# rlawhdrhs/Vision-Transformer-OpenCL

Hardware: AMD Instinct MI355X
Metric: images/sec ViT-B/16 224² fp32 @batch256; % MFMA roofline; top-1 match (higher is better)
Workload: dtype f32; 1 GPU; ViT-B/16 224x224 fp32 forward, batch 256 per GPU, synthetic weights and images (BASELINE.json configs[1]); batch_per_gpu=256, global_batch=256, parallelism=dp1, lanes_per_gpu=1, prune_last_layer=False, ln_fold=True, device=AMD Radeon Graphics, arch=gfx950:sramecc+:xnack-, compute_units=256, clock_mhz=2400

## Files before the change

### include/vit_hip_kernels.h

```cpp
#ifndef VIT_HIP_KERNELS_H
#define VIT_HIP_KERNELS_H

#include <stddef.h>

#ifdef __cplusplus
extern "C" {
#endif

typedef void *vithip_stream_t;
typedef void *vithip_event_t;
typedef void *vithip_graph_t;

typedef struct {
    char name[256];
    char arch[64];
    int compute_units;
    int clock_mhz;
    int wavefront;
    int lds_per_block;
    unsigned long long hbm_bytes;
} vithip_device_info;

const char *vithip_error_string(int code);
int vithip_device_count(int *count);
int vithip_set_device(int device);
int vithip_get_device_info(int device, vithip_device_info *info);
int vithip_malloc(void **ptr, size_t bytes);
int vithip_free(void *ptr);
int vithip_host_alloc(void **ptr, size_t bytes);
int vithip_host_free(void *ptr);
int vithip_memcpy_h2d(void *dst, const void *src, size_t bytes, vithip_stream_t stream);
int vithip_memcpy_d2h(void *dst, const void *src, size_t bytes, vithip_stream_t stream);
int vithip_memcpy_d2d(void *dst, const void *src, size_t bytes, vithip_stream_t stream);
int vithip_memcpy_peer(void *dst, int dst_device, const void *src, int src_device, size_t bytes, vithip_stream_t stream);
int vithip_memset(void *dst, int value, size_t bytes, vithip_stream_t stream);
int vithip_stream_create(vithip_stream_t *stream);
int vithip_stream_destroy(vithip_stream_t stream);
int vithip_stream_sync(vithip_stream_t stream);
int vithip_device_sync(void);
int vithip_event_create(vithip_event_t *event);
int vithip_event_destroy(vithip_event_t event);
int vithip_event_record(vithip_event_t event, vithip_stream_t stream);
int vithip_event_sync(vithip_event_t event);
int vithip_event_elapsed_ms(float *ms, vithip_event_t start, vithip_event_t stop);
int vithip_stream_wait_event(vithip_stream_t stream, vithip_event_t event);
int vithip_graph_begin(vithip_stream_t stream);
int vithip_graph_end(vithip_stream_t stream, vithip_graph_t *graph);
int vithip_graph_launch(vithip_graph_t graph, vithip_stream_t stream);
int vithip_graph_destroy(vithip_graph_t graph);


enum { VITHIP_EPI_BIAS = 0, VITHIP_EPI_BIAS_GELU = 1, VITHIP_EPI_BIAS_RESIDUAL = 2 };

typedef struct {
    const float *A; int lda;
    const float *W; int ldw;
    const float *bias;
    const float *residual; int ldr;
    float *C; int ldc;
    int M, N, K;
    int epilogue;
    int tile, group_m;
    void *workspace;
    int handover_test;
    const float *ln_rows, *ln_colsum;
    float *stats_out, *stats_partials;
    int arith;
} vithip_gemm_args;
int vithip_gemm_f32(vithip_stream_t stream, const vithip_gemm_args *args);
int vithip_gemm_f32_stats_in_epilogue(const vithip_gemm_args *args);
int vithip_ln_fold_weights_f32(vithip_stream_t stream, const float *W, const float *bias, const float *gamma, const float *beta,
                               float *Wf, float *colsum, float *bias_f, int N, int K);
int vithip_ln_fold_weights_f32_centered(vithip_stream_t stream, const float *W, const float *bias, const float *gamma,
                                        const float *beta, float *Wc, float *residual_colsum, float *bias_f, int N, int K);
int vithip_rowstats_f32(vithip_stream_t stream, const float *x, size_t ldx, float *rows_out, int rows, int dim);
int vithip_rowstats_finalize_f32(vithip_stream_t stream, const float *partials, int rows, int dim, float *rows_out);
size_t vithip_gemm_f32_workspace_bytes(void);
int vithip_gemm_f32_workspace_create(void **workspace);
int vithip_gemm_f32_workspace_destroy(void *workspace);
int vithip_gemm_f32_workspace_stats(void *workspace, int *taken, int *recomputed);
void *vithip_gemm_f32_workspace_device_ptr(void *workspace);
enum { VITHIP_BF16_EPI_BF16 = 0, VITHIP_BF16_EPI_BF16_GELU = 1, VITHIP_BF16_EPI_F32_RESIDUAL = 2,
       VITHIP_BF16_EPI_F32_EMBED = 3  };
typedef struct {
    const unsigned short *A; int lda;
    const unsigned short *W; int ldw;
    const float *bias;
    const float *residual; int ldr;
    void *C; int ldc;
    int M, N, K;
    int epilogue;
    int variant;
    const float *ln_rows, *ln_colsum;
    unsigned short *x16; int ldx16;
    float *row_partials;
} vithip_gemm_bf16_args;
int vithip_gemm_bf16(vithip_stream_t stream, const vithip_gemm_bf16_args *args);
int vithip_ln_fold_weights(vithip_stream_t stream, const float *W, const float *bias, const float *gamma, const float *beta,
                           unsigned short *Wf, float *colsum, float *bias_f, int N, int K);
#define VITHIP_QSCALE 0.18033688011112042f
int vithip_ln_fold_weights_scaled(vithip_stream_t stream, const float *W, const float *bias, const float *gamma, const float *beta,
                                  unsigned short *Wf, float *colsum, float *bias_f, int N, int K, int scale_rows, float scale);
int vithip_rowstats_bf16(vithip_stream_t stream, const float *x, size_t ldx, unsigned short *x16, size_t ldx16,
                         float *rows_out, int rows, int dim);
int vithip_ln_strips(int N);
int vithip_rowstats_finalize(vithip_stream_t stream, const float *partials, int strips, int rows, int dim, float *rows_out);
int vithip_gather_rows_f32(vithip_stream_t stream, const float *src, size_t src_stride, float *dst, size_t dst_stride, int rows,
                           int width);
int vithip_layernorm_f32_bf16out(vithip_stream_t stream, const float *x, size_t ldx, unsigned short *y, size_t ldy,
                                 const float *gamma, const float *beta, int rows, int dim);
int vithip_attention_bf16io(vithip_stream_t stream, const unsigned short *qkv, unsigned short *out,
                            int n_images, int tokens, int heads);
int vithip_attention_bf16io_f32math(vithip_stream_t stream, const unsigned short *qkv, unsigned short *out,
                                    int n_images, int tokens, int heads);
int vithip_attention_f32_rows(vithip_stream_t stream, const float *qkv, float *out, int n_images, int tokens, int heads,
                              int q_rows);
int vithip_attention_bf16io_rows(vithip_stream_t stream, const unsigned short *qkv, unsigned short *out, int n_images,
                                 int tokens, int heads, int q_rows);
int vithip_attention_bf16io_qscaled(vithip_stream_t stream, const unsigned short *qkv, unsigned short *out, int n_images,
                                    int tokens, int heads, int q_rows);
int vithip_patch_embed_bf16(vithip_stream_t stream, const float *images, const unsigned short *conv_w16,
                            const float *conv_b, const float *cls, const float *pos, float *x,
                            unsigned short *patches16, int n_images, int img_size, int patch_size, int in_chans,
                            int embed_dim);
int vithip_patch_embed_bf16_implicit(vithip_stream_t stream, const float *images, const unsigned short *conv_w16,
                                     const float *conv_b, const float *cls, const float *pos, float *x,
                                     int n_images, int img_size, int patch_size, int in_chans, int embed_dim);
int vithip_f32_to_bf16(vithip_stream_t stream, const float *src, unsigned short *dst, size_t count);

int vithip_patch_embed_f32(vithip_stream_t stream, const float *images, const float *conv_w,
                           const float *conv_b, const float *cls, const float *pos, float *x,
                           int n_images, int img_size, int patch_size, int in_chans, int embed_dim);

int vithip_layernorm_f32(vithip_stream_t stream, const float *x, size_t ldx, float *y, size_t ldy,
                         const float *gamma, const float *beta, int rows, int dim);

int vithip_attention_f32(vithip_stream_t stream, const float *qkv, float *out,
                         int n_images, int tokens, int heads);

int vithip_softmax_top1_f32(vithip_stream_t stream, const float *logits, int ld_logits,
                            float *probs, int ld_probs, int *top1_label, float *top1_prob,
                            int rows, int classes);

int vithip_images_u8_to_f32(vithip_stream_t stream, const unsigned char *src, float *dst, int n, int img_size, int chans,
                            const float *mean, const float *std);

#ifdef __cplusplus
}
#endif
#endif
```

### vision-transformer-opencl_amd/binding.py

```python
from __future__ import annotations

import ctypes as C
import os
from typing import Optional, Sequence

import numpy as np

from .synth import ModelConfig

HERE = os.path.dirname(os.path.abspath(__file__))
LIB_PATH = os.environ.get("VIT_HIP_LIBRARY") or os.path.join(HERE, "libvit_mi355x.so")

f32p = C.POINTER(C.c_float)
i32p = C.POINTER(C.c_int)

STAGES = ("embed", "ln", "qkv", "attn", "outproj", "fc1", "fc2", "head", "softmax")
IMAGENET_MEAN = (0.485, 0.456, 0.406)
IMAGENET_STD = (0.229, 0.224, 0.225)
EPI_BIAS, EPI_BIAS_GELU, EPI_BIAS_RESIDUAL = 0, 1, 2
ARITH_F32, ARITH_SPLIT3 = 0, 1


class VitError(RuntimeError):
    pass


class CConfig(C.Structure):
    _fields_ = [(k, C.c_int) for k in ("img_size", "patch_size", "in_chans", "num_classes",
                                       "embed_dim", "depth", "num_heads", "hidden_dim")]

    @classmethod
    def of(cls, cfg: ModelConfig) -> "CConfig":
        return cls(cfg.img_size, cfg.patch_size, cfg.in_chans, cfg.num_classes, cfg.embed_dim,
                   cfg.depth, cfg.num_heads, cfg.hidden_dim)


class CNetwork(C.Structure):
    _fields_ = [("data", f32p), ("size", C.c_size_t)]


class CImageData(C.Structure):
    _fields_ = [("n", C.c_int), ("c", C.c_int), ("h", C.c_int), ("w", C.c_int), ("data", f32p)]


class COptions(C.Structure):
    _fields_ = [("device", C.c_int), ("max_batch", C.c_int), ("profile", C.c_int), ("lanes", C.c_int),
                ("dtype", C.c_int), ("prune_last_layer", C.c_int), ("use_graph", C.c_int), ("gemm_tile", C.c_int), ("ln_fold", C.c_int),
                ("gemm_handover_test", C.c_int), ("host_first_piece", C.c_int), ("fp32_split", C.c_int)]


class CStageTimes(C.Structure):
    _fields_ = [("ms", C.c_double * len(STAGES)), ("launches", C.c_long * len(STAGES)), ("images", C.c_long)]


class CDeviceInfo(C.Structure):
    _fields_ = [("name", C.c_char * 256), ("arch", C.c_char * 64), ("compute_units", C.c_int),
                ("clock_mhz", C.c_int), ("wavefront", C.c_int), ("lds_per_block", C.c_int),
                ("hbm_bytes", C.c_ulonglong)]


class CGemmArgs(C.Structure):
    _fields_ = [("A", C.c_void_p), ("lda", C.c_int), ("W", C.c_void_p), ("ldw", C.c_int),
                ("bias", C.c_void_p), ("residual", C.c_void_p), ("ldr", C.c_int),
                ("C", C.c_void_p), ("ldc", C.c_int), ("M", C.c_int), ("N", C.c_int), ("K", C.c_int),
                ("epilogue", C.c_int), ("tile", C.c_int), ("group_m", C.c_int), ("workspace", C.c_void_p),
                ("handover_test", C.c_int), ("ln_rows", C.c_void_p), ("ln_colsum", C.c_void_p),
                ("stats_out", C.c_void_p), ("stats_partials", C.c_void_p), ("arith", C.c_int)]


_lib: Optional[C.CDLL] = None


DP_LIB_PATH = os.path.join(HERE, "libvit_mi355x_dp.so")
_dp_lib = None


def dp_lib() -> C.CDLL:
    global _dp_lib
    if _dp_lib is None:
        if not os.path.exists(DP_LIB_PATH):
            raise VitError(f"{DP_LIB_PATH} is missing: run `make -C {HERE}`")
        L = C.CDLL(DP_LIB_PATH)
        L.vit_dp_create.argtypes = [C.POINTER(C.c_void_p), C.POINTER(C.c_int), C.c_int]
        L.vit_dp_destroy.argtypes = [C.c_void_p]
        L.vit_dp_destroy.restype = None
        L.vit_dp_size.argtypes = [C.c_void_p]
        L.vit_dp_device.argtypes = [C.c_void_p, C.c_int]
        L.vit_dp_last_error.argtypes = [C.c_void_p]
        L.vit_dp_last_error.restype = C.c_char_p
        L.vit_dp_gather_top1.argtypes = [C.c_void_p, C.POINTER(C.c_void_p), C.POINTER(C.c_void_p), C.c_size_t, C.POINTER(C.c_void_p)]
        _dp_lib = L
    return _dp_lib


class DpGroup:

    def __init__(self, devices):
        self.devices = [int(d) for d in devices]
        self._h = C.c_void_p()
        arr = (C.c_int * len(self.devices))(*self.devices)
        rc = dp_lib().vit_dp_create(C.byref(self._h), arr, len(self.devices))
        if rc != 0:
            raise VitError(f"vit_dp_create({self.devices}) failed: {rc}")

    def gather_top1(self, send_ptrs, recv_ptrs, records: int, streams=None) -> None:
        n = len(self.devices)
        send = (C.c_void_p * n)(*send_ptrs)
        recv = (C.c_void_p * n)(*recv_ptrs)
        st = (C.c_void_p * n)(*streams) if streams is not None else None
        rc = dp_lib().vit_dp_gather_top1(self._h, send, recv, records, st)
        if rc != 0:
            raise VitError(f"vit_dp_gather_top1: {dp_lib().vit_dp_last_error(self._h).decode()} ({rc})")

    def close(self) -> None:
        if self._h:
            dp_lib().vit_dp_destroy(self._h)
            self._h = C.c_void_p()


def lib() -> C.CDLL:
    global _lib
    if _lib is None:
        if not os.path.exists(LIB_PATH):
            raise VitError(f"{LIB_PATH} is missing: the HIP extension has not been built "
                           "(run `python -c 'import __graft_entry__ as g; g.build()'` or `make -C "
                           f"{HERE}`); there is no CPU fallback")
        L = C.CDLL(LIB_PATH)
        L.vithip_error_string.restype = C.c_char_p
        L.vit_engine_last_error.restype = C.c_char_p
        L.vit_engine_last_error.argtypes = [C.c_void_p]
        L.vit_engine_create.argtypes = [C.POINTER(C.c_void_p), C.POINTER(CConfig), C.POINTER(COptions)]
        L.vit_engine_destroy.argtypes = [C.c_void_p]
        L.vit_engine_load_weights.argtypes = [C.c_void_p, C.POINTER(CNetwork), C.c_int]
        L.vit_engine_forward_device.argtypes = [C.c_void_p, C.c_void_p, C.c_int, C.c_void_p, C.c_void_p,
                                                C.c_void_p, C.c_void_p]
        L.vit_engine_forward_host.argtypes = [C.c_void_p, C.POINTER(f32p), C.c_int, C.POINTER(f32p)]
        L.vit_engine_forward_device_u8.argtypes = [C.c_void_p, C.c_void_p, C.c_int, f32p, f32p, C.c_void_p, C.c_void_p,
                                                   C.c_void_p, C.c_void_p]
        L.vit_engine_forward_host_u8.argtypes = [C.c_void_p, C.POINTER(C.c_void_p), C.c_int, f32p, f32p, C.POINTER(f32p)]
        L.vithip_images_u8_to_f32.argtypes = [C.c_void_p, C.c_void_p, C.c_void_p, C.c_int, C.c_int, C.c_int, f32p, f32p]
        L.vit_engine_read_logits.argtypes = [C.c_void_p, f32p, C.c_int]
        L.vit_engine_sync.argtypes = [C.c_void_p]
        L.vit_engine_get_stage_times.argtypes = [C.c_void_p, C.POINTER(CStageTimes)]
        L.vit_engine_reset_stage_times.argtypes = [C.c_void_p]
        L.vit_engine_set_profile.argtypes = [C.c_void_p, C.c_int]
        L.vit_config_weight_size.restype = C.c_size_t
        L.vit_config_weight_size.argtypes = [C.POINTER(CConfig), C.c_int]
        L.vit_config_macs_per_image.restype = C.c_ulonglong
        L.vit_config_macs_per_image.argtypes = [C.POINTER(CConfig)]
        L.vit_config_macs_per_image_pruned.restype = C.c_ulonglong
        L.vit_config_macs_per_image_pruned.argtypes = [C.POINTER(CConfig)]
        L.vit_config_b16.restype = CConfig
        L.load_image_data.restype = C.POINTER(CImageData)
        L.load_image_data.argtypes = [C.c_char_p]
        L.free_image_data.argtypes = [C.POINTER(CImageData)]
        L.load_weights.argtypes = [C.c_char_p, C.POINTER(CNetwork), C.c_int]
        L.free_weights.argtypes = [C.POINTER(CNetwork), C.c_int]
        L.vit_round_weights.argtypes = [f32p, C.c_size_t]
        L.vit_compare_results.argtypes = [C.c_char_p, C.c_char_p, C.c_int, C.c_float]
        L.vit_synth_uniform.argtypes = [C.c_ulonglong, C.c_int, C.c_size_t, C.c_float, C.c_float, f32p]
        L.vit_synth_weights.argtypes = [C.POINTER(CConfig), C.c_ulonglong, C.POINTER(CNetwork), C.c_int]
        L.vit_synth_images.restype = C.POINTER(CImageData)
        L.vit_synth_images.argtypes = [C.POINTER(CConfig), C.c_int, C.c_ulonglong]
        L.vit_argmax.argtypes = [f32p, C.c_int]
        L.ViT_hip.argtypes = [C.POINTER(CImageData), C.POINTER(CNetwork), C.POINTER(f32p)]
        L.ViT_opencl.argtypes = [C.POINTER(CImageData), C.POINTER(CNetwork), C.POINTER(f32p)]
        for fn in ("vithip_malloc", "vithip_host_alloc"):
            getattr(L, fn).argtypes = [C.POINTER(C.c_void_p), C.c_size_t]
        L.vithip_free.argtypes = [C.c_void_p]
        for fn in ("vithip_memcpy_h2d", "vithip_memcpy_d2h", "vithip_memcpy_d2d"):
            getattr(L, fn).argtypes = [C.c_void_p, C.c_void_p, C.c_size_t, C.c_void_p]
        L.vithip_gemm_f32.argtypes = [C.c_void_p, C.POINTER(CGemmArgs)]
        L.vithip_patch_embed_f32.argtypes = [C.c_void_p] + [C.c_void_p] * 6 + [C.c_int] * 5
        L.vithip_layernorm_f32.argtypes = [C.c_void_p, C.c_void_p, C.c_size_t, C.c_void_p, C.c_size_t,
                                           C.c_void_p, C.c_void_p, C.c_int, C.c_int]
        L.vithip_attention_f32.argtypes = [C.c_void_p, C.c_void_p, C.c_void_p, C.c_int, C.c_int, C.c_int]
        L.vithip_softmax_top1_f32.argtypes = [C.c_void_p, C.c_void_p, C.c_int, C.c_void_p, C.c_int, C.c_void_p,
                                              C.c_void_p, C.c_int, C.c_int]
        L.vithip_event_create.argtypes = [C.POINTER(C.c_void_p)]
        L.vithip_event_record.argtypes = [C.c_void_p, C.c_void_p]
        L.vithip_event_sync.argtypes = [C.c_void_p]
        L.vithip_event_destroy.argtypes = [C.c_void_p]
        L.vithip_event_elapsed_ms.argtypes = [C.POINTER(C.c_float), C.c_void_p, C.c_void_p]
        L.vithip_stream_sync.argtypes = [C.c_void_p]
        L.vithip_get_device_info.argtypes = [C.c_int, C.POINTER(CDeviceInfo)]
        _lib = L
    return _lib


def hip_check(rc: int, what: str = "HIP call") -> None:
    if rc != 0:
        raise VitError(f"{what}: HIP error {rc} ({lib().vithip_error_string(rc).decode()})")


def _as_f32(a) -> np.ndarray:
    return np.ascontiguousarray(a, dtype=np.float32)


def networks_from(weights: Sequence[np.ndarray]):
    arr = (CNetwork * len(weights))()
    keep = []
    for i, w in enumerate(weights):
        if w is None:
            arr[i].data = None
            arr[i].size = 0
        else:
            w = _as_f32(w)
            keep.append(w)
            arr[i].data = w.ctypes.data_as(f32p)
            arr[i].size = w.size
    return arr, keep


class DeviceArray:

    def __init__(self, shape, dtype=np.float32):
        self.shape = tuple(int(s) for s in np.atleast_1d(shape))
        self.dtype = np.dtype(dtype)
        self.nbytes = int(np.prod(self.shape)) * self.dtype.itemsize
        p = C.c_void_p()
        hip_check(lib().vithip_malloc(C.byref(p), max(self.nbytes, 16)), "vithip_malloc")
        self.ptr = p.value

    @classmethod
    def from_numpy(cls, a: np.ndarray) -> "DeviceArray":
        a = np.ascontiguousarray(a)
        d = cls(a.shape, a.dtype)
        hip_check(lib().vithip_memcpy_h2d(d.ptr, a.ctypes.data, a.nbytes, None), "h2d")
        hip_check(lib().vithip_device_sync(), "sync")
        return d

    def numpy(self) -> np.ndarray:
        out = np.empty(self.shape, self.dtype)
        hip_check(lib().vithip_device_sync(), "sync")
        hip_check(lib().vithip_memcpy_d2h(out.ctypes.data, self.ptr, self.nbytes, None), "d2h")
        hip_check(lib().vithip_device_sync(), "sync")
        return out

    def free(self) -> None:
        if self.ptr:
            lib().vithip_free(self.ptr)
            self.ptr = None

    def __del__(self):
        try:
            self.free()
        except Exception:
            pass


def gemm(A, W, bias, residual=None, epilogue=EPI_BIAS, tile: int = 0, group_m: int = 0, workspace: bool = False,
         handover_test: int = 0, stats: Optional[dict] = None, ln=None, row_stats: Optional[dict] = None,
         arith: int = ARITH_F32) -> np.ndarray:
    A, W, bias = _as_f32(A), _as_f32(W), _as_f32(bias)
    M, K = A.shape
    N = W.shape[0]
    dA, dW, db = DeviceArray.from_numpy(A), DeviceArray.from_numpy(W), DeviceArray.from_numpy(bias)
    dC = DeviceArray((M, N))
    dR = DeviceArray.from_numpy(_as_f32(residual)) if residual is not None else None
    ws = gemm_workspace() if workspace else None
    dRows = DeviceArray.from_numpy(_as_f32(ln[0])) if ln is not None else None
    dCs = DeviceArray.from_numpy(_as_f32(ln[1])) if ln is not None and ln[1] is not None else None
    dSt = DeviceArray((M, 2)) if row_stats is not None else None
    dPart = DeviceArray((max(N // 64, 1), M, 2)) if row_stats is not None and row_stats.get("scratch", True) else None
    args = CGemmArgs(dA.ptr, K, dW.ptr, K, db.ptr, dR.ptr if dR else None, N, dC.ptr, N, M, N, K, epilogue, tile, group_m, ws,
                     handover_test, dRows.ptr if dRows else None, dCs.ptr if dCs else None, dSt.ptr if dSt else None,
                     dPart.ptr if dPart else None, arith)
    if row_stats is not None:
        row_stats["in_epilogue"] = int(lib().vithip_gemm_f32_stats_in_epilogue(C.byref(args)))
    hip_check(lib().vithip_gemm_f32(None, C.byref(args)), "vithip_gemm_f32")
    out = dC.numpy()
    if row_stats is not None:
        row_stats["rows"] = dSt.numpy()
    if ws:
        if stats is not None:
            stats.update(gemm_workspace_stats(ws))
        lib().vithip_gemm_f32_workspace_destroy(C.c_void_p(ws))
    return out


def gemm_workspace() -> int:
    p = C.c_void_p()
    hip_check(lib().vithip_gemm_f32_workspace_create(C.byref(p)), "vithip_gemm_f32_workspace_create")
    return p.value


def gemm_workspace_stats(ws: int) -> dict:
    L = lib()
    hip_check(L.vithip_device_sync(), "vithip_device_sync")
    t, r = C.c_int(), C.c_int()
    L.vithip_gemm_f32_workspace_stats.argtypes = [C.c_void_p, C.POINTER(C.c_int), C.POINTER(C.c_int)]
    hip_check(L.vithip_gemm_f32_workspace_stats(ws, C.byref(t), C.byref(r)), "vithip_gemm_f32_workspace_stats")
    return {"taken": t.value, "recomputed": r.value}


def gemm_workspace_flags(ws: int, count: int = 1016) -> np.ndarray:
    L = lib()
    L.vithip_gemm_f32_workspace_device_ptr.restype = C.c_void_p
    L.vithip_gemm_f32_workspace_device_ptr.argtypes = [C.c_void_p]
    flags = np.empty(count, np.int32)
    hip_check(L.vithip_device_sync(), "sync")
    hip_check(L.vithip_memcpy_d2h(flags.ctypes.data, L.vithip_gemm_f32_workspace_device_ptr(ws), flags.nbytes, None), "d2h")
    hip_check(L.vithip_device_sync(), "sync")
    return flags


def gemm_workspace_set_flags(ws: int, values) -> None:
    L = lib()
    L.vithip_gemm_f32_workspace_device_ptr.restype = C.c_void_p
    L.vithip_gemm_f32_workspace_device_ptr.argtypes = [C.c_void_p]
    v = np.ascontiguousarray(values, np.int32)
    hip_check(L.vithip_device_sync(), "sync")
    hip_check(L.vithip_memcpy_h2d(L.vithip_gemm_f32_workspace_device_ptr(ws), v.ctypes.data, v.nbytes, None), "h2d")
    hip_check(L.vithip_device_sync(), "sync")


class CGemmBf16Args(C.Structure):
    _fields_ = [("A", C.c_void_p), ("lda", C.c_int), ("W", C.c_void_p), ("ldw", C.c_int), ("bias", C.c_void_p),
                ("residual", C.c_void_p), ("ldr", C.c_int), ("C", C.c_void_p), ("ldc", C.c_int),
                ("M", C.c_int), ("N", C.c_int), ("K", C.c_int), ("epilogue", C.c_int),
                ("variant", C.c_int),
                ("ln_rows", C.c_void_p), ("ln_colsum", C.c_void_p), ("x16", C.c_void_p), ("ldx16", C.c_int),
                ("row_partials", C.c_void_p)]


BF16_EPI_BF16, BF16_EPI_BF16_GELU, BF16_EPI_F32_RESIDUAL = 0, 1, 2


def to_bf16_bits(x: np.ndarray) -> np.ndarray:
    u = np.ascontiguousarray(x, np.float32).view(np.uint32).astype(np.uint64)
    return ((u + 0x7FFF + ((u >> 16) & 1)) >> 16).astype(np.uint16)


def from_bf16_bits(b: np.ndarray) -> np.ndarray:
    return (b.astype(np.uint32) << 16).view(np.float32)


def f32_to_bf16_device(x: np.ndarray) -> np.ndarray:
    x = _as_f32(x)
    L = lib()
    L.vithip_f32_to_bf16.argtypes = [C.c_void_p, C.c_void_p, C.c_void_p, C.c_size_t]
    dx = DeviceArray.from_numpy(x)
    dy = DeviceArray(x.shape, np.uint16)
    hip_check(L.vithip_f32_to_bf16(None, dx.ptr, dy.ptr, x.size), "vithip_f32_to_bf16")
    return dy.numpy()


def gemm_bf16(A_bits, W_bits, bias, residual=None, epilogue=BF16_EPI_BF16, variant: int = 0, ln_rows=None, ln_colsum=None,
              ln_producer: bool = False):
    L = lib()
    L.vithip_gemm_bf16.argtypes = [C.c_void_p, C.POINTER(CGemmBf16Args)]
    M, K = A_bits.shape
    N = W_bits.shape[0]
    dA, dW = DeviceArray.from_numpy(np.ascontiguousarray(A_bits, np.uint16)), DeviceArray.from_numpy(np.ascontiguousarray(W_bits, np.uint16))
    db = DeviceArray.from_numpy(_as_f32(bias))
    out_f32 = epilogue == BF16_EPI_F32_RESIDUAL
    dC = DeviceArray((M, N), np.float32 if out_f32 else np.uint16)
    dR = DeviceArray.from_numpy(_as_f32(residual)) if residual is not None else None
    dRows = DeviceArray.from_numpy(_as_f32(ln_rows)) if ln_rows is not None else None
    dCs = DeviceArray.from_numpy(_as_f32(ln_colsum)) if ln_colsum is not None else None
    strips = ln_strips(N)
    dX16 = DeviceArray((M, N), np.uint16) if ln_producer else None
    dPart = DeviceArray((strips, M, 2), np.float32) if ln_producer else None
    args = CGemmBf16Args(dA.ptr, K, dW.ptr, K, db.ptr, dR.ptr if dR else None, N, dC.ptr, N, M, N, K, epilogue,
                         variant, dRows.ptr if dRows else None, dCs.ptr if dCs else None,
                         dX16.ptr if dX16 else None, N, dPart.ptr if dPart else None)
    hip_check(L.vithip_gemm_bf16(None, C.byref(args)), "vithip_gemm_bf16")
    if ln_producer:
        return dC.numpy(), dX16.numpy(), dPart.numpy()
    return dC.numpy()


def ln_strips(N: int) -> int:
    return int(lib().vithip_ln_strips(int(N)))


def ln_fold_weights(W, bias, gamma, beta):
    W = _as_f32(W)
    N, K = W.shape
    L = lib()
    L.vithip_ln_fold_weights.argtypes = [C.c_void_p] * 8 + [C.c_int, C.c_int]
    dW, db, dg, dbe = (DeviceArray.from_numpy(_as_f32(a)) for a in (W, bias, gamma, beta))
    dWf, dcs, dbf = DeviceArray((N, K), np.uint16), DeviceArray((N,), np.float32), DeviceArray((N,), np.float32)
    hip_check(L.vithip_ln_fold_weights(None, dW.ptr, db.ptr, dg.ptr, dbe.ptr, dWf.ptr, dcs.ptr, dbf.ptr, N, K), "vithip_ln_fold_weights")
    return dWf.numpy(), dcs.numpy(), dbf.numpy()


def rowstats_bf16(x):
    x = _as_f32(x)
    rows, dim = x.shape
    L = lib()
    L.vithip_rowstats_bf16.argtypes = [C.c_void_p, C.c_void_p, C.c_size_t, C.c_void_p, C.c_size_t, C.c_void_p, C.c_int, C.c_int]
    dx, d16, dr = DeviceArray.from_numpy(x), DeviceArray((rows, dim), np.uint16), DeviceArray((rows, 2), np.float32)
    hip_check(L.vithip_rowstats_bf16(None, dx.ptr, dim, d16.ptr, dim, dr.ptr, rows, dim), "vithip_rowstats_bf16")
    return d16.numpy(), dr.numpy()


def rowstats_finalize(partials, dim: int):
    partials = _as_f32(partials)
    strips, rows, _ = partials.shape
    L = lib()
    L.vithip_rowstats_finalize.argtypes = [C.c_void_p, C.c_void_p, C.c_int, C.c_int, C.c_int, C.c_void_p]
    dp, dr = DeviceArray.from_numpy(partials), DeviceArray((rows, 2), np.float32)
    hip_check(L.vithip_rowstats_finalize(None, dp.ptr, strips, rows, dim, dr.ptr), "vithip_rowstats_finalize")
    return dr.numpy()


def layernorm_bf16out(x, gamma, beta) -> np.ndarray:
    x = _as_f32(x)
    rows, dim = x.shape
    L = lib()
    L.vithip_layernorm_f32_bf16out.argtypes = [C.c_void_p, C.c_void_p, C.c_size_t, C.c_void_p, C.c_size_t,
                                               C.c_void_p, C.c_void_p, C.c_int, C.c_int]
    dx, dg, db = DeviceArray.from_numpy(x), DeviceArray.from_numpy(_as_f32(gamma)), DeviceArray.from_numpy(_as_f32(beta))
    dy = DeviceArray((rows, dim), np.uint16)
    hip_check(L.vithip_layernorm_f32_bf16out(None, dx.ptr, dim, dy.ptr, dim, dg.ptr, db.ptr, rows, dim),
              "vithip_layernorm_f32_bf16out")
    return dy.numpy()


QSCALE = 0.18033688011112042


def attention_bf16io(qkv_bits, n_images: int, tokens: int, heads: int, f32math: bool = False, q_scaled: bool = False,
                     q_rows: Optional[int] = None) -> np.ndarray:
    D = heads * 64
    dq = DeviceArray.from_numpy(np.ascontiguousarray(qkv_bits, np.uint16))
    do = DeviceArray((n_images * tokens, D), np.uint16)
    if q_scaled:
        fn = lib().vithip_attention_bf16io_qscaled
        fn.argtypes = [C.c_void_p, C.c_void_p, C.c_void_p, C.c_int, C.c_int, C.c_int, C.c_int]
        hip_check(fn(None, dq.ptr, do.ptr, n_images, tokens, heads, q_rows or tokens), "vithip_attention_bf16io_qscaled")
        return do.numpy()
    fn = getattr(lib(), "vithip_attention_bf16io_f32math" if f32math else "vithip_attention_bf16io")
    fn.argtypes = [C.c_void_p, C.c_void_p, C.c_void_p, C.c_int, C.c_int, C.c_int]
    hip_check(fn(None, dq.ptr, do.ptr, n_images, tokens, heads), "vithip_attention_bf16io")
    return do.numpy()


def layernorm(x, gamma, beta) -> np.ndarray:
    x = _as_f32(x)
    rows, dim = x.shape
    dx, dg, db = DeviceArray.from_numpy(x), DeviceArray.from_numpy(_as_f32(gamma)), DeviceArray.from_numpy(_as_f32(beta))
    dy = DeviceArray((rows, dim))
    hip_check(lib().vithip_layernorm_f32(None, dx.ptr, dim, dy.ptr, dim, dg.ptr, db.ptr, rows, dim), "vithip_layernorm_f32")
    return dy.numpy()


def ln_fold_weights_f32(W, bias, gamma, beta):
    W, bias, gamma, beta = _as_f32(W), _as_f32(bias), _as_f32(gamma), _as_f32(beta)
    N, K = W.shape
    dW, db, dg, dbe = (DeviceArray.from_numpy(a) for a in (W, bias, gamma, beta))
    dWf, dcs, dbf = DeviceArray((N, K)), DeviceArray((N,)), DeviceArray((N,))
    lib().vithip_ln_fold_weights_f32.argtypes = [C.c_void_p] * 8 + [C.c_int, C.c_int]
    hip_check(lib().vithip_ln_fold_weights_f32(None, dW.ptr, db.ptr, dg.ptr, dbe.ptr, dWf.ptr, dcs.ptr, dbf.ptr, N, K),
              "vithip_ln_fold_weights_f32")
    return dWf.numpy(), dcs.numpy(), dbf.numpy()


def ln_fold_weights_f32_centered(W, bias, gamma, beta):
    W, bias, gamma, beta = _as_f32(W), _as_f32(bias), _as_f32(gamma), _as_f32(beta)
    N, K = W.shape
    dW, db, dg, dbe = (DeviceArray.from_numpy(a) for a in (W, bias, gamma, beta))
    dWf, dcs, dbf = DeviceArray((N, K)), DeviceArray((N,)), DeviceArray((N,))
    lib().vithip_ln_fold_weights_f32_centered.argtypes = [C.c_void_p] * 8 + [C.c_int, C.c_int]
    hip_check(lib().vithip_ln_fold_weights_f32_centered(None, dW.ptr, db.ptr, dg.ptr, dbe.ptr, dWf.ptr, dcs.ptr, dbf.ptr, N, K),
              "vithip_ln_fold_weights_f32_centered")
    return dWf.numpy(), dcs.numpy(), dbf.numpy()


def rowstats_f32(x) -> np.ndarray:
    x = _as_f32(x)
    rows, dim = x.shape
    L = lib()
    L.vithip_rowstats_f32.argtypes = [C.c_void_p, C.c_void_p, C.c_size_t, C.c_void_p, C.c_int, C.c_int]
    dx, dr = DeviceArray.from_numpy(x), DeviceArray((rows, 2))
    hip_check(L.vithip_rowstats_f32(None, dx.ptr, dim, dr.ptr, rows, dim), "vithip_rowstats_f32")
    return dr.numpy()


def attention(qkv, n_images: int, tokens: int, heads: int) -> np.ndarray:
    qkv = _as_f32(qkv)
    D = heads * 64
    assert qkv.shape == (n_images * tokens, 3 * D)
    dq = DeviceArray.from_numpy(qkv)
    do = DeviceArray((n_images * tokens, D))
    hip_check(lib().vithip_attention_f32(None, dq.ptr, do.ptr, n_images, tokens, heads), "vithip_attention_f32")
    return do.numpy()


def attention_rows(qkv, n_images: int, tokens: int, heads: int, q_rows: int, fill: float = 0.0) -> np.ndarray:
    qkv = _as_f32(qkv)
    D = heads * 64
    L = lib()
    L.vithip_attention_f32_rows.argtypes = [C.c_void_p, C.c_void_p, C.c_void_p, C.c_int, C.c_int, C.c_int, C.c_int]
    dq = DeviceArray.from_numpy(qkv)
    do = DeviceArray.from_numpy(np.full((n_images * tokens, D), fill, np.float32))
    hip_check(L.vithip_attention_f32_rows(None, dq.ptr, do.ptr, n_images, tokens, heads, q_rows), "vithip_attention_f32_rows")
    return do.numpy()


def patch_embed(cfg: ModelConfig, images, conv_w, conv_b, cls, pos) -> np.ndarray:
    images = _as_f32(images)
    n = images.shape[0]
    d = [DeviceArray.from_numpy(_as_f32(a)) for a in (images, conv_w, conv_b, cls, pos)]
    dx = DeviceArray((n * cfg.tokens, cfg.embed_dim))
    hip_check(lib().vithip_patch_embed_f32(None, d[0].ptr, d[1].ptr, d[2].ptr, d[3].ptr, d[4].ptr, dx.ptr, n,
                                           cfg.img_size, cfg.patch_size, cfg.in_chans, cfg.embed_dim),
              "vithip_patch_embed_f32")
    return dx.numpy().reshape(n, cfg.tokens, cfg.embed_dim)


def patch_embed_bf16(cfg: ModelConfig, images, conv_w, conv_b, cls, pos, implicit: bool = False) -> np.ndarray:
    images = _as_f32(images)
    n = images.shape[0]
    L = lib()
    if implicit:
        L.vithip_patch_embed_bf16_implicit.argtypes = [C.c_void_p] * 7 + [C.c_int] * 5
        d = [DeviceArray.from_numpy(_as_f32(a)) for a in (images, conv_b, cls, pos)]
        dw = DeviceArray.from_numpy(to_bf16_bits(_as_f32(conv_w).reshape(cfg.embed_dim, -1)))
        dx = DeviceArray((n * cfg.tokens, cfg.embed_dim))
        hip_check(L.vithip_patch_embed_bf16_implicit(None, d[0].ptr, dw.ptr, d[1].ptr, d[2].ptr, d[3].ptr, dx.ptr, n, cfg.img_size,
                                                     cfg.patch_size, cfg.in_chans, cfg.embed_dim), "vithip_patch_embed_bf16_implicit")
        return dx.numpy().reshape(n, cfg.tokens, cfg.embed_dim)
    L.vithip_patch_embed_bf16.argtypes = [C.c_void_p] * 8 + [C.c_int] * 5
    d = [DeviceArray.from_numpy(_as_f32(a)) for a in (images, conv_b, cls, pos)]
    dw = DeviceArray.from_numpy(to_bf16_bits(_as_f32(conv_w).reshape(cfg.embed_dim, -1)))
    dx = DeviceArray((n * cfg.tokens, cfg.embed_dim))
    dp = DeviceArray((n * cfg.patches, cfg.patch_dim), np.uint16)
    hip_check(L.vithip_patch_embed_bf16(None, d[0].ptr, dw.ptr, d[1].ptr, d[2].ptr, d[3].ptr, dx.ptr, dp.ptr, n,
                                        cfg.img_size, cfg.patch_size, cfg.in_chans, cfg.embed_dim), "vithip_patch_embed_bf16")
    return dx.numpy().reshape(n, cfg.tokens, cfg.embed_dim)


def softmax_top1(logits):
    logits = _as_f32(logits)
    rows, classes = logits.shape
    dl = DeviceArray.from_numpy(logits)
    dp = DeviceArray((rows, classes))
    dlab = DeviceArray((rows,), np.int32)
    dpr = DeviceArray((rows,))
    hip_check(lib().vithip_softmax_top1_f32(None, dl.ptr, classes, dp.ptr, classes, dlab.ptr, dpr.ptr, rows, classes),
              "vithip_softmax_top1_f32")
    return dp.numpy(), dlab.numpy(), dpr.numpy()


def _norm_consts(mean, std, chans: int):
    out = []
    for v in (mean, std):
        if v is None:
            out.append(None)
            continue
        v = np.ascontiguousarray(v, np.float32).reshape(-1)
        if v.size != chans:
            raise ValueError(f"expected {chans} normalisation constants, got {v.size}")
        out.append((C.c_float * chans)(*v.tolist()))
    return out


def images_u8_to_f32(images, mean=IMAGENET_MEAN, std=IMAGENET_STD) -> np.ndarray:
    images = np.ascontiguousarray(images, np.uint8)
    n, S, S2, chans = images.shape
    assert S == S2
    m, s = _norm_consts(mean, std, chans)
    ds, dd = DeviceArray.from_numpy(images), DeviceArray((n, chans, S, S))
    hip_check(lib().vithip_images_u8_to_f32(None, ds.ptr, dd.ptr, n, S, chans, m, s), "vithip_images_u8_to_f32")
    return dd.numpy()


def device_info(device: int = 0) -> dict:
    info = CDeviceInfo()
    hip_check(lib().vithip_get_device_info(device, C.byref(info)), "vithip_get_device_info")
    return {"name": info.name.decode(), "arch": info.arch.decode(), "compute_units": info.compute_units,
            "clock_mhz": info.clock_mhz, "wavefront": info.wavefront, "lds_per_block": info.lds_per_block,
            "hbm_bytes": int(info.hbm_bytes)}


class Engine:

    def __init__(self, cfg: ModelConfig, max_batch: int = 256, device: int = 0, profile: bool = False,
                 lanes: int = 1, dtype: str = "f32", prune_last_layer: bool = False, use_graph: bool = False,
# ... 305 lines not shown
```

### vision-transformer-opencl_amd/csrc/vit_gemm.hip

```cpp
#include <new>

#include "vit_gemm_common.hpp"
#ifdef VIT_PROBES
#include "vit_probes.h"
#endif

namespace vitgemm {
int launch_persistent(hipStream_t stream, GemmParams &p, int epilogue, int group_m, int arith = ARITH_F32);
int launch_persistent_stamped(hipStream_t stream, GemmParams &p, int epilogue, int group_m);
int launch_persistent_switchoff(hipStream_t stream, GemmParams &p, int epilogue, int group_m, int dbg);
int persistent_piece_steps(int M, int N, int K, int slots, int wgs, int kstep);
}

namespace {

using namespace vitgemm;

#ifdef VIT_PROBES
int g_gemm_tile = 0;
int g_gemm_group = 0;
unsigned long long *g_gemm_dbg = nullptr;
#endif

template <int BM, int BN, int WM, int WN, int EPI, int AMODE, int DBG = 0, int BK = 32, bool PIPE = false, int ARITH = ARITH_F32>
// ... 219 lines not shown
                }
            }
            cur ^= 1;
        }
    } else {
        load_global(0);
        store_lds(0);
        if constexpr (DBG != 0) store_lds(1);
        __syncthreads();


        if constexpr (DBG == 5) st_clk1 = __builtin_amdgcn_s_memtime();
        if constexpr (DBG >= 10) {
#pragma unroll
            for (int q = 0; q < DBG - 10; ++q) asm volatile("s_nop 0");
        }
        int cur = 0;
        for (int kt = 0; kt < nk; ++kt) {
            const bool more = kt + 1 < nk;
            if constexpr (DBG == 0 || DBG == 3 || DBG == 5) {
                if (more) load_global((kt + 1) * BK);
            }

            const float *As = As0 + cur * BM * LDS_LD + a_frag_off;
            const float *Bs = Bs0 + cur * BN * LDS_LD + b_frag_off;
#pragma unroll
            for (int c = 0; c < BK / 8; ++c) {
                f32x4 a[TM], b[TN];
#pragma unroll
                for (int i = 0; i < TM; ++i) a[i] = *reinterpret_cast<const f32x4 *>(As + i * 32 * LDS_LD + c * 8);
#pragma unroll
                for (int j = 0; j < TN; ++j) b[j] = *reinterpret_cast<const f32x4 *>(Bs + j * 32 * LDS_LD + c * 8);
#pragma unroll
                for (int s = 0; s < 4; ++s)
#pragma unroll
                    for (int i = 0; i < TM; ++i)
#pragma unroll
                        for (int j = 0; j < TN; ++j)
                            acc[i][j] = __builtin_amdgcn_mfma_f32_32x32x2f32(a[i][s], b[j][s], acc[i][j], 0, 0, 0);
            }

            if constexpr (DBG == 0 || DBG == 2 || DBG == 5) {
                if (more) store_lds(cur ^ 1);
            } else if constexpr (DBG == 3) {
#pragma unroll
                for (int i = 0; i < A_CHUNKS; ++i) asm volatile("" ::"v"(a_stage[i]));
#pragma unroll
                for (int i = 0; i < B_CHUNKS; ++i) asm volatile("" ::"v"(b_stage[i]));
            }
            if constexpr (DBG != 4) __syncthreads();
            cur ^= 1;
        }

    }

    if constexpr (DBG == 5) st_clk2 = __builtin_amdgcn_s_memtime();
    epilogue_store<BM, BN, WM, WN, EPI, AMODE>(p, acc, bias_r, m0, n0, wm, wn, r, h, fold);
    if constexpr (DBG == 5) {
        __builtin_amdgcn_s_waitcnt(0);
        const unsigned long long c3 = __builtin_amdgcn_s_memtime(), r3 = __builtin_amdgcn_s_memrealtime();
        if (tid == 0) {
            unsigned long long *d = p.dbg + (size_t)blockIdx.x * 8;
            d[0] = st_clk0; d[1] = st_clk1; d[2] = st_clk2; d[3] = c3; d[4] = st_rt0; d[5] = r3;
            d[6] = __builtin_amdgcn_s_getreg((3 << 11) | 20);
            d[7] = (unsigned long long)tile;
        }
    }
}

__global__ void cls_rows_kernel(const float *cls, const float *pos, float *x, int n_images, int tokens, int dim) {
    const int idx = blockIdx.x * blockDim.x + threadIdx.x;
    if (idx >= n_images * dim) return;
    const int im = idx / dim, d = idx - im * dim;
    x[(size_t)im * tokens * dim + d] = cls[d] + pos[d];
}

template <int BM, int BN, int WM, int WN, int AMODE, int BK = 32, bool PIPE = false, int ARITH = ARITH_F32>
int launch_tile(hipStream_t stream, GemmParams &p, int epilogue) {
    p.tiles_m = (p.M + BM - 1) / BM;
    p.tiles_n = (p.N + BN - 1) / BN;
    const dim3 grid(p.tiles_m * p.tiles_n), block(256);
    if constexpr (AMODE == A_PATCHES) {
        hipLaunchKernelGGL((gemm_f32_nt_kernel<BM, BN, WM, WN, VITHIP_EPI_BIAS, A_PATCHES, 0, BK, PIPE>), grid, block, 0, stream, p);
    } else {
        switch (epilogue) {
            case VITHIP_EPI_BIAS:
                hipLaunchKernelGGL((gemm_f32_nt_kernel<BM, BN, WM, WN, VITHIP_EPI_BIAS, A_DENSE, 0, BK, PIPE, ARITH>), grid, block, 0, stream, p);
                break;
            case VITHIP_EPI_BIAS_GELU:
                hipLaunchKernelGGL((gemm_f32_nt_kernel<BM, BN, WM, WN, VITHIP_EPI_BIAS_GELU, A_DENSE, 0, BK, PIPE, ARITH>), grid, block, 0, stream, p);
                break;
            case VITHIP_EPI_BIAS_RESIDUAL:
                hipLaunchKernelGGL((gemm_f32_nt_kernel<BM, BN, WM, WN, VITHIP_EPI_BIAS_RESIDUAL, A_DENSE, 0, BK, PIPE, ARITH>), grid, block, 0, stream, p);
                break;
            case EPI_BIAS_LN:
                hipLaunchKernelGGL((gemm_f32_nt_kernel<BM, BN, WM, WN, EPI_BIAS_LN, A_DENSE, 0, BK, PIPE, ARITH>), grid, block, 0, stream, p);
                break;
            case EPI_BIAS_GELU_LN:
                hipLaunchKernelGGL((gemm_f32_nt_kernel<BM, BN, WM, WN, EPI_BIAS_GELU_LN, A_DENSE, 0, BK, PIPE, ARITH>), grid, block, 0, stream, p);
                break;
            default:
                return static_cast<int>(hipErrorInvalidValue);
        }
    }
    return static_cast<int>(hipGetLastError());
}

#ifdef VIT_PROBES
template <int DBG, int EPI = VITHIP_EPI_BIAS, bool PIPE = false>
int launch_probe(hipStream_t stream, GemmParams &p) {
    p.tiles_m = (p.M + 127) / 128;
    p.tiles_n = (p.N + 127) / 128;
    hipLaunchKernelGGL((gemm_f32_nt_kernel<128, 128, 64, 64, EPI, A_DENSE, DBG, 32, PIPE>),
                       dim3(p.tiles_m * p.tiles_n), dim3(256), 0, stream, p);
    return static_cast<int>(hipGetLastError());
}
#endif

template <int AMODE, int ARITH = ARITH_F32>
int dispatch(hipStream_t stream, GemmParams &p, int epilogue, int tile, int group_m) {
    constexpr bool SPLIT = ARITH == ARITH_SPLIT3;
    constexpr int BK = SPLIT ? SPLIT_BK : 32;
    static_assert(!SPLIT || AMODE == A_DENSE, "the patch embedding stays on fp32 MFMA");
    const int cols128 = (p.N + 127) / 128;
    p.group_m = group_m > 0 ? group_m : (cols128 <= 8 ? 1 : 4);
#ifdef VIT_PROBES
    if (g_gemm_tile) tile = g_gemm_tile;
    if (g_gemm_group) p.group_m = g_gemm_group;
    if constexpr (AMODE == A_DENSE && !SPLIT) {
        switch (tile) {
            case 101: return launch_probe<1>(stream, p);
            case 102: return launch_probe<2>(stream, p);
            case 103: return launch_probe<3>(stream, p);
            case 104: return launch_probe<4>(stream, p);
            case 105: p.dbg = g_gemm_dbg; return g_gemm_dbg ? launch_probe<5>(stream, p) : static_cast<int>(hipErrorInvalidValue);
            case 129: p.dbg = g_gemm_dbg; return g_gemm_dbg ? vitgemm::launch_persistent_stamped(stream, p, epilogue, p.group_m) : static_cast<int>(hipErrorInvalidValue);
            case 125: p.dbg = g_gemm_dbg; return g_gemm_dbg ? launch_probe<5, VITHIP_EPI_BIAS, true>(stream, p) : static_cast<int>(hipErrorInvalidValue);
            case 126: p.dbg = g_gemm_dbg; return g_gemm_dbg ? launch_probe<5, VITHIP_EPI_BIAS_GELU, true>(stream, p) : static_cast<int>(hipErrorInvalidValue);
            case 131: case 132: case 133: case 134: case 135: case 136:
                return vitgemm::launch_persistent_switchoff(stream, p, epilogue, p.group_m, tile - 130);
            default: break;
        }
    }
#endif
    if constexpr (AMODE == A_PATCHES) {
        const bool pipe_ok = (32 % p.patch == 0 || p.patch % 32 == 0) && (p.patch * p.patch) % 32 == 0 &&
                             (size_t)(p.M / p.patches + 1) * p.chans * p.img * p.img * 4 < 0x7fffffffull;
#ifdef VIT_PROBES
        if (tile == 1) return launch_tile<128, 128, 64, 64, A_PATCHES>(stream, p, epilogue);
        if (tile == 2) return launch_tile<256, 128, 128, 64, A_PATCHES>(stream, p, epilogue);
        if (tile == 10) return launch_tile<128, 128, 64, 64, A_PATCHES, 32, true>(stream, p, epilogue);
        if (tile == 3) return launch_tile<128, 64, 64, 32, A_PATCHES>(stream, p, epilogue);
#endif
        if (!pipe_ok) return launch_tile<128, 64, 64, 32, A_PATCHES>(stream, p, epilogue);
        return launch_tile<128, 64, 64, 32, A_PATCHES, 32, true>(stream, p, epilogue);
    }
    switch (tile) {
        case 9: return vitgemm::launch_persistent(stream, p, epilogue, p.group_m, ARITH);
        case 6: case 7: case 8: case 12:
            if constexpr (SPLIT) return static_cast<int>(hipErrorInvalidValue);
            else if (tile == 6) return launch_tile<128, 128, 64, 64, AMODE, 16, true>(stream, p, epilogue);
            else if (tile == 7) return launch_tile<256, 128, 128, 64, AMODE, 32, true>(stream, p, epilogue);
            else if (tile == 8) return launch_tile<128, 64, 64, 32, AMODE, 32, true>(stream, p, epilogue);
            else if (p.K % 128) return static_cast<int>(hipErrorInvalidValue);
            else return vitgemm::launch_gemm_f32_latency(stream, p, epilogue);
        case 10: return launch_tile<128, 128, 64, 64, AMODE, BK, true, ARITH>(stream, p, epilogue);
        case 11: return launch_tile<64, 64, 32, 32, AMODE, BK, true, ARITH>(stream, p, epilogue);
        default: {
            const long tiles = (long)((p.M + 127) / 128) * ((p.N + 127) / 128);
            if (!SPLIT && p.K % 128 == 0 && (long)((p.M + 63) / 64) * ((p.N + 63) / 64) < 160)
                return vitgemm::launch_gemm_f32_latency(stream, p, epilogue);
            if ((long)((p.M + 127) / 128) * ((p.N + 63) / 64) < 256)
                return launch_tile<64, 64, 32, 32, AMODE, BK, true, ARITH>(stream, p, epilogue);
            if (epilogue == VITHIP_EPI_BIAS_RESIDUAL) {
                if (tiles < 1024) return launch_tile<64, 64, 32, 32, AMODE, BK, true, ARITH>(stream, p, epilogue);
                if ((p.row_partials && p.N % 128 == 0) || (p.sk_ws && vitgemm::persistent_piece_steps(p.M, p.N, p.K, p.sk_slots, 0, BK) > 0))
                    return vitgemm::launch_persistent(stream, p, epilogue, p.group_m, ARITH);
                return launch_tile<128, 128, 64, 64, AMODE, BK, true, ARITH>(stream, p, epilogue);
            }
            if (tiles < 1280) return launch_tile<64, 64, 32, 32, AMODE, BK, true, ARITH>(stream, p, epilogue);
            return vitgemm::launch_persistent(stream, p, epilogue, p.group_m, ARITH);
        }
    }
}

bool aligned16(const void *ptr) { return (reinterpret_cast<size_t>(ptr) & 15) == 0; }

}

extern "C" {

#ifdef VIT_PROBES
int vithip_gemm_set_tile(int tile) {
    if ((tile < 0 || tile > 12) && (tile < 101 || tile > 136)) return static_cast<int>(hipErrorInvalidValue);
    g_gemm_tile = tile;
    return 0;
}

int vithip_gemm_set_debug_buffer(void *buf) {
    g_gemm_dbg = static_cast<unsigned long long *>(buf);
    return 0;
}

int vithip_gemm_set_group(int group_m) {
    if (group_m < 0 || group_m > 1024) return static_cast<int>(hipErrorInvalidValue);
    g_gemm_group = group_m;
    return 0;
}
#endif

struct GemmWorkspace {
    void *dev;
    int slots;
    int device;
    int gen;
};
static size_t workspace_dev_bytes(int slots) { return 4096 + (size_t)slots * 128 * 128 * 4; }

size_t vithip_gemm_f32_workspace_bytes(void) {
    int dev = 0, cus = 0;
    if (hipGetDevice(&dev) != hipSuccess || hipDeviceGetAttribute(&cus, hipDeviceAttributeMultiprocessorCount, dev) != hipSuccess) return 0;
    return workspace_dev_bytes(2 * cus);
}

int vithip_gemm_f32_workspace_create(void **ws) {
    if (!ws) return static_cast<int>(hipErrorInvalidValue);
    *ws = nullptr;
    int dev = 0, cus = 0;
    hipError_t e = hipGetDevice(&dev);
    if (e == hipSuccess) e = hipDeviceGetAttribute(&cus, hipDeviceAttributeMultiprocessorCount, dev);
    if (e != hipSuccess) return static_cast<int>(e);
    GemmWorkspace *w = new (std::nothrow) GemmWorkspace{nullptr, 2 * cus, dev, 0};
    if (!w) return static_cast<int>(hipErrorOutOfMemory);
    e = hipExtMallocWithFlags(&w->dev, workspace_dev_bytes(w->slots), hipDeviceMallocUncached);
    if (e == hipSuccess) e = hipMemset(w->dev, 0, 4096);
    if (e == hipSuccess) e = hipDeviceSynchronize();
    if (e != hipSuccess) {
        if (w->dev) (void)hipFree(w->dev);
        delete w;
        return static_cast<int>(e);
    }
    *ws = w;
    return 0;
}
int vithip_gemm_f32_workspace_destroy(void *ws) {
    if (!ws) return 0;
    GemmWorkspace *w = static_cast<GemmWorkspace *>(ws);
    const hipError_t e = hipFree(w->dev);
    delete w;
    return static_cast<int>(e);
}
int vithip_gemm_f32_workspace_stats(void *ws, int *taken, int *recomputed) {
    if (!ws) return static_cast<int>(hipErrorInvalidValue);
    GemmWorkspace *w = static_cast<GemmWorkspace *>(ws);
    int c[2] = {0, 0};
    char *at = static_cast<char *>(w->dev) + 1016 * sizeof(int);
    hipError_t e = hipMemcpy(c, at, sizeof(c), hipMemcpyDeviceToHost);
    if (e == hipSuccess && (c[0] || c[1])) e = hipMemset(at, 0, sizeof(c));
    if (taken) *taken = c[0];
    if (recomputed) *recomputed = c[1];
    return static_cast<int>(e);
}
void *vithip_gemm_f32_workspace_device_ptr(void *ws) { return ws ? static_cast<GemmWorkspace *>(ws)->dev : nullptr; }

int vithip_gemm_f32_stats_in_epilogue(const vithip_gemm_args *a) {
    if (!a || !a->stats_out || !a->stats_partials || a->epilogue != VITHIP_EPI_BIAS_RESIDUAL || a->M <= 0 || a->N <= 0 || a->N % 128 ||
        a->N > 2048)
        return 0;
    const long tiles = (long)((a->M + 127) / 128) * (a->N / 128);
    return (a->tile == 9 || (a->tile == 0 && tiles >= 1024)) ? 1 : 0;
}

int vithip_gemm_f32(vithip_stream_t stream, const vithip_gemm_args *a) {
    if (!a || !a->A || !a->W || !a->bias || !a->C) return static_cast<int>(hipErrorInvalidValue);
    if (a->M <= 0 || a->N <= 0 || a->K <= 0 || a->K % KALIGN != 0) return static_cast<int>(hipErrorInvalidValue);
    if (a->lda % 4 || a->ldw % 4 || a->lda < a->K || a->ldw < a->K || a->ldc < a->N)
        return static_cast<int>(hipErrorInvalidValue);
    if (!aligned16(a->A) || !aligned16(a->W)) return static_cast<int>(hipErrorInvalidValue);
    if ((size_t)a->M * a->lda * 4 >= 0x7fffffffull || (size_t)a->N * a->ldw * 4 >= 0x7fffffffull)
        return static_cast<int>(hipErrorInvalidValue);
    if (a->epilogue == VITHIP_EPI_BIAS_RESIDUAL && (!a->residual || a->ldr < a->N))
        return static_cast<int>(hipErrorInvalidValue);
    if ((size_t)a->M * a->ldc * 4 >= 0x7fffffffull ||
        (a->epilogue == VITHIP_EPI_BIAS_RESIDUAL && (size_t)a->M * a->ldr * 4 >= 0x7fffffffull))
        return static_cast<int>(hipErrorInvalidValue);
    GemmParams p{};
    p.A = a->A; p.W = a->W; p.bias = a->bias; p.R = a->residual; p.C = a->C;
    p.lda = a->lda; p.ldw = a->ldw; p.ldr = a->ldr; p.ldc = a->ldc;
    p.M = a->M; p.N = a->N; p.K = a->K;
    if (a->workspace) {
        GemmWorkspace *w = static_cast<GemmWorkspace *>(a->workspace);
        int dev = -1;
        if (hipGetDevice(&dev) != hipSuccess || dev != w->device) return static_cast<int>(hipErrorInvalidDevice);
        p.sk_ws = w->dev;
        p.sk_slots = w->slots;
        p.sk_late = a->handover_test == 1;
        w->gen = w->gen >= (1 << 28) ? 1 : w->gen + 1;
        p.sk_gen = w->gen;
    }
    if (a->handover_test < 0 || a->handover_test > 1) return static_cast<int>(hipErrorInvalidValue);
    if (a->tile < 0 || (a->tile > 0 && a->tile < 6) || a->tile > 12 || a->group_m < 0 || a->group_m > 1024) return static_cast<int>(hipErrorInvalidValue);
    if (a->arith != ARITH_F32 && (a->arith != ARITH_SPLIT3 || (a->tile != 0 && a->tile != 9 && a->tile != 10 && a->tile != 11)))
        return static_cast<int>(hipErrorInvalidValue);
    int epilogue = a->epilogue;
    if (a->ln_rows || a->ln_colsum) {
        if (!a->ln_rows || (epilogue != VITHIP_EPI_BIAS && epilogue != VITHIP_EPI_BIAS_GELU) ||
            (reinterpret_cast<size_t>(a->ln_rows) & 7))
            return static_cast<int>(hipErrorInvalidValue);
        p.ln_rows = a->ln_rows;
        p.ln_colsum = a->ln_colsum;
        epilogue = epilogue == VITHIP_EPI_BIAS ? vitgemm::EPI_BIAS_LN : vitgemm::EPI_BIAS_GELU_LN;
    }
    if (a->stats_out) {
        if (epilogue != VITHIP_EPI_BIAS_RESIDUAL || a->N % 64 || a->N > 2048 || (reinterpret_cast<size_t>(a->stats_out) & 7) ||
            (reinterpret_cast<size_t>(a->stats_partials) & 7))
            return static_cast<int>(hipErrorInvalidValue);
        if (vithip_gemm_f32_stats_in_epilogue(a)) p.row_partials = a->stats_partials;
    }
    const int rc = a->arith == ARITH_SPLIT3 ? dispatch<A_DENSE, ARITH_SPLIT3>(static_cast<hipStream_t>(stream), p, epilogue, a->tile, a->group_m)
                                            : dispatch<A_DENSE>(static_cast<hipStream_t>(stream), p, epilogue, a->tile, a->group_m);
    if (rc != 0 || !a->stats_out) return rc;
    if (p.stats_in_epilogue) return vithip_rowstats_finalize_f32(stream, a->stats_partials, a->M, a->N, a->stats_out);
    return vithip_rowstats_f32(stream, a->C, (size_t)a->ldc, a->stats_out, a->M, a->N);
}

int vithip_patch_embed_f32(vithip_stream_t stream, const float *images, const float *conv_w,
                           const float *conv_b, const float *cls, const float *pos, float *x,
                           int n_images, int img_size, int patch_size, int in_chans, int embed_dim) {
    if (!images || !conv_w || !conv_b || !cls || !pos || !x || n_images <= 0)
        return static_cast<int>(hipErrorInvalidValue);
    if (patch_size % 4 || img_size % patch_size) return static_cast<int>(hipErrorInvalidValue);
    const int K = in_chans * patch_size * patch_size;
    if (K % KALIGN || img_size % 4) return static_cast<int>(hipErrorInvalidValue);
    if (!aligned16(images) || !aligned16(conv_w)) return static_cast<int>(hipErrorInvalidValue);
    const int G = img_size / patch_size;
    GemmParams p{};
    p.A = images; p.W = conv_w; p.bias = conv_b; p.C = x; p.pos = pos;
    p.lda = 0; p.ldw = K; p.ldc = embed_dim;
    p.M = n_images * G * G; p.N = embed_dim; p.K = K;
    p.patches = G * G; p.grid = G; p.patch = patch_size; p.img = img_size; p.chans = in_chans;
    hipStream_t s = static_cast<hipStream_t>(stream);
    const int total = n_images * embed_dim;
    hipLaunchKernelGGL(cls_rows_kernel, dim3((total + 255) / 256), dim3(256), 0, s, cls, pos, x,
                       n_images, G * G + 1, embed_dim);
    int e = static_cast<int>(hipGetLastError());
    if (e) return e;
    return dispatch<A_PATCHES>(s, p, VITHIP_EPI_BIAS, 0, 0);
}

}
```

### vision-transformer-opencl_amd/csrc/vit_gemm_common.hpp

```cpp
#pragma once
#include <hip/hip_runtime.h>

#include <type_traits>

#include "vit_hip_kernels.h"

namespace vitgemm {


typedef float f32x16 __attribute__((ext_vector_type(16)));
typedef float f32x4 __attribute__((ext_vector_type(4)));
typedef float f32x2 __attribute__((ext_vector_type(2)));
typedef unsigned u32x4 __attribute__((ext_vector_type(4)));

constexpr int KALIGN = 32;

enum { A_DENSE = 0, A_PATCHES = 1 };
enum { EPI_BIAS_LN = 3, EPI_BIAS_GELU_LN = 4, EPI_RESIDUAL_STATS = 5 };

struct GemmParams {
    const float *A;
    const float *W;
    const float *bias;
    const float *R;
    float *C;
    int lda, ldw, ldr, ldc;
    int M, N, K;
    int tiles_m, tiles_n;
    int group_m;
    const float *pos;
    unsigned long long *dbg;
    int patches;
    int grid;
    int patch;
    int img;
    int chans;
    void *sk_ws;
    int sk_slots;
    int sk_x;
    int sk_late;
    int sk_gen;
    const float *ln_rows;
    const float *ln_colsum;
    float *row_partials;
    int stats_in_epilogue;
};

__device__ __forceinline__ float erf_fp32(float x) {
    const float t = fminf(fabsf(x), 4.0f);
    float q = -3.144179208902642e-05f;
    q = fmaf(q, t, 3.0881378916092217e-04f);
    q = fmaf(q, t, -1.0324339382350445e-03f);
    q = fmaf(q, t, -5.368884885683656e-04f);
    q = fmaf(q, t, 1.95839274674654e-02f);
    q = fmaf(q, t, -1.0291960090398788e-01f);
    q = fmaf(q, t, -6.36597752571106e-01f);
    q = fmaf(q, t, -1.128380298614502f);
    const float e = __builtin_amdgcn_exp2f(q * t * 1.4426950408889634f);
    return copysignf(1.0f - e, x);
}

__device__ __forceinline__ float gelu_erf(float x) {
    return 0.5f * x * (1.0f + erf_fp32(x * 0.70710678118654752440f));
}

__device__ __forceinline__ void gelu_erf_x8(float (&y)[8]) {
    typedef float v2 __attribute__((ext_vector_type(2)));
    v2 yy[4], u[4], t[4], q[4];
#pragma unroll
    for (int v = 0; v < 4; ++v) {
        yy[v] = v2{y[2 * v], y[2 * v + 1]};
        u[v] = yy[v] * v2{0.70710678118654752440f, 0.70710678118654752440f};
        t[v] = v2{fminf(fabsf(u[v][0]), 4.0f), fminf(fabsf(u[v][1]), 4.0f)};
        q[v] = __builtin_elementwise_fma(v2{-3.144179208902642e-05f, -3.144179208902642e-05f}, t[v],
                                         v2{3.0881378916092217e-04f, 3.0881378916092217e-04f});
    }
    __builtin_amdgcn_sched_barrier(0);
    constexpr float c[6] = {-1.0324339382350445e-03f, -5.368884885683656e-04f, 1.95839274674654e-02f,
                            -1.0291960090398788e-01f, -6.36597752571106e-01f, -1.128380298614502f};
#pragma unroll
    for (int k = 0; k < 6; ++k) {
#pragma unroll
        for (int v = 0; v < 4; ++v) q[v] = __builtin_elementwise_fma(q[v], t[v], v2{c[k], c[k]});
        __builtin_amdgcn_sched_barrier(0);
    }
#pragma unroll
    for (int v = 0; v < 4; ++v) q[v] = q[v] * t[v] * v2{1.4426950408889634f, 1.4426950408889634f};
    __builtin_amdgcn_sched_barrier(0);
#pragma unroll
    for (int v = 0; v < 4; ++v) q[v] = v2{__builtin_amdgcn_exp2f(q[v][0]), __builtin_amdgcn_exp2f(q[v][1])};
    __builtin_amdgcn_sched_barrier(0);
#pragma unroll
    for (int v = 0; v < 4; ++v) {
        const v2 e = v2{1.0f, 1.0f} - q[v];
        const v2 sgn = v2{copysignf(e[0], u[v][0]), copysignf(e[1], u[v][1])};
        const v2 r = v2{0.5f, 0.5f} * yy[v] * (v2{1.0f, 1.0f} + sgn);
        y[2 * v] = r[0];
        y[2 * v + 1] = r[1];
    }
}

__device__ __forceinline__ f32x2 gelu_bf16_x2(f32x2 y) {
    constexpr float kClamp = 5.656854249492381f;
    const f32x2 t = f32x2{fminf(__builtin_fabsf(y.x), kClamp), fminf(__builtin_fabsf(y.y), kClamp)};
    constexpr float c[7] = {-1.000037431716919f,   -1.1505244970321655f,   -0.4605136811733246f,  -0.05179140716791153f,
                            0.007414536084979773f, -0.0006474481779150665f, 2.524326555430889e-05f};
    f32x2 q = f32x2{c[6], c[6]};
#pragma unroll
    for (int k = 5; k >= 0; --k) q = __builtin_elementwise_fma(q, t, f32x2{c[k], c[k]});
    const f32x2 e = f32x2{__builtin_amdgcn_exp2f(q.x), __builtin_amdgcn_exp2f(q.y)};
    return __builtin_elementwise_fma(-t, e, __builtin_elementwise_max(y, f32x2{0.f, 0.f}));
}

template <int NP>
__device__ __forceinline__ void gelu_bf16_lockstep(f32x2 (&y)[NP]) {
    constexpr float kClamp = 5.656854249492381f;
    constexpr float c[7] = {-1.000037431716919f,   -1.1505244970321655f,   -0.4605136811733246f,  -0.05179140716791153f,
                            0.007414536084979773f, -0.0006474481779150665f, 2.524326555430889e-05f};
    f32x2 t[NP], q[NP];
#pragma unroll
    for (int v = 0; v < NP; ++v) {
        t[v] = f32x2{fminf(__builtin_fabsf(y[v].x), kClamp), fminf(__builtin_fabsf(y[v].y), kClamp)};
        q[v] = __builtin_elementwise_fma(f32x2{c[6], c[6]}, t[v], f32x2{c[5], c[5]});
    }
    __builtin_amdgcn_sched_barrier(0);
#pragma unroll
    for (int k = 4; k >= 0; --k) {
#pragma unroll
        for (int v = 0; v < NP; ++v) q[v] = __builtin_elementwise_fma(q[v], t[v], f32x2{c[k], c[k]});
        __builtin_amdgcn_sched_barrier(0);
    }
#pragma unroll
    for (int v = 0; v < NP; ++v) q[v] = f32x2{__builtin_amdgcn_exp2f(q[v].x), __builtin_amdgcn_exp2f(q[v].y)};
    __builtin_amdgcn_sched_barrier(0);
#pragma unroll
    for (int v = 0; v < NP; ++v) y[v] = __builtin_elementwise_fma(-t[v], q[v], __builtin_elementwise_max(y[v], f32x2{0.f, 0.f}));
}

__device__ __forceinline__ int xcd_remap(int bid, int nwg) {
    const int q = nwg >> 3, rem = nwg & 7;
    const int xcd = bid & 7, idx = bid >> 3;
    const int base = xcd < rem ? xcd * (q + 1) : rem * (q + 1) + (xcd - rem) * q;
    return base + idx;
}

__device__ __forceinline__ void tile_coords(int tile, int tiles_m, int tiles_n, int group_m, int &tm, int &tn) {
    const int per_group = group_m * tiles_n;
    const int g = tile / per_group, in_g = tile - g * per_group;
    const int first = g * group_m;
    const int rows = tiles_m - first < group_m ? tiles_m - first : group_m;
    tn = in_g / rows;
    tm = first + (in_g - tn * rows);
}


enum { ARITH_F32 = 0, ARITH_SPLIT3 = 1 };
typedef __bf16 bf16x8 __attribute__((ext_vector_type(8)));
typedef __bf16 bf16x4 __attribute__((ext_vector_type(4)));
typedef unsigned u32x2 __attribute__((ext_vector_type(2)));
constexpr int SPLIT_BK = 16;
constexpr int SPLIT_LD = 28;
constexpr int SPLIT_TERM_A[6] = {0, 2, 1, 0, 1, 0};
constexpr int SPLIT_TERM_W[6] = {2, 0, 1, 1, 0, 0};

__device__ __forceinline__ float bf16_to_f32(__bf16 v) {
    return __builtin_bit_cast(float, (unsigned)__builtin_bit_cast(unsigned short, v) << 16);
}
__device__ __forceinline__ void split3_store(float *row, int kc, f32x4 x) {
#pragma unroll
    for (int piece = 0; piece < 3; ++piece) {
        bf16x4 b;
#pragma unroll
        for (int e = 0; e < 4; ++e) b[e] = (__bf16)x[e];
        *reinterpret_cast<u32x2 *>(row + piece * 8 + kc / 2) = __builtin_bit_cast(u32x2, b);
        if (piece < 2) {
#pragma unroll
            for (int e = 0; e < 4; ++e) x[e] = x[e] - bf16_to_f32(b[e]);
        }
    }
}
template <int TM, int TN, int NS, typename Restage>
__device__ __forceinline__ void split3_step(f32x16 (&acc)[TM][TN], const float *As, const float *Bs, Restage &&restage) {
    bf16x8 a[TM][3], b[TN][3];
#pragma unroll
    for (int o = 0; o < 3; ++o) {
        const int pa = SPLIT_TERM_A[o], pb = SPLIT_TERM_W[o];
#pragma unroll
        for (int i = 0; i < TM; ++i) a[i][pa] = *reinterpret_cast<const bf16x8 *>(As + i * 32 * SPLIT_LD + pa * 8);
#pragma unroll
        for (int j = 0; j < TN; ++j) b[j][pb] = *reinterpret_cast<const bf16x8 *>(Bs + j * 32 * SPLIT_LD + pb * 8);
    }
    __builtin_amdgcn_sched_barrier(0);
    constexpr int NM = 6 * TM * TN, NR = NM / 2 > 0 ? NM / 2 : 1;
#pragma unroll
    for (int idx = 0; idx < NM; ++idx) {
        const int t = idx / (TM * TN), i = (idx / TN) % TM, j = idx % TN;
        acc[i][j] = __builtin_amdgcn_mfma_f32_32x32x16_bf16(a[i][SPLIT_TERM_A[t]], b[j][SPLIT_TERM_W[t]], acc[i][j], 0, 0, 0);
        if (idx < NR) {
            const int slot_before = (idx * NS) / NR, slot_after = ((idx + 1) * NS) / NR;
            if (slot_after > slot_before) {
                __builtin_amdgcn_sched_barrier(0);
#pragma unroll
                for (int q = slot_before; q < slot_after; ++q) restage(q);
                __builtin_amdgcn_sched_barrier(0);
            }
        }
    }
}

template <int TN, int TM = 1>
struct FoldOperands {
    float colsum[TN];
    const f32x2 *rows;
    float rstd[TM][16], mean[TM];
    bool preloaded;
};
template <int TN, int TM>
__device__ __forceinline__ void fold_preload(FoldOperands<TN, TM> &fold, const float *ln_rows, int M, int m_tile, int r, int h) {
#pragma unroll
    for (int i = 0; i < TM; ++i) {
        const int mr = m_tile + i * 32 + r;
        fold.mean[i] = ln_rows[2 * (size_t)(mr < M ? mr : M - 1) + 1];
#pragma unroll
        for (int v = 0; v < 16; ++v) {
            const int m = m_tile + i * 32 + 4 * h + (v & 3) + 8 * (v >> 2);
            fold.rstd[i][v] = ln_rows[2 * (size_t)(m < M ? m : M - 1)];
        }
    }
    fold.preloaded = true;
}
__device__ __forceinline__ float fold_center(float acc, float mean, float colsum) { return __builtin_fmaf(-mean, colsum, acc); }
__device__ __forceinline__ float fold_scale(float centered, float rstd, float bias) { return __builtin_fmaf(rstd, centered, bias); }

#ifndef FOLD_HOIST
#define FOLD_HOIST 1
#endif
template <int BM, int BN, int WM, int WN, int EPI, int AMODE>
__device__ __forceinline__ void epilogue_store(const GemmParams &p, const f32x16 (&acc)[WM / 32][WN / 32],
                                               const float (&bias_r)[WN / 32], int m0, int n0, int wm, int wn,
                                               int r, int h, const FoldOperands<WN / 32, WM / 32> &fold = FoldOperands<WN / 32, WM / 32>{}) {
    constexpr int TM = WM / 32, TN = WN / 32;
    constexpr bool FOLD = EPI == EPI_BIAS_LN || EPI == EPI_BIAS_GELU_LN;
    constexpr bool GELU = EPI == VITHIP_EPI_BIAS_GELU || EPI == EPI_BIAS_GELU_LN;
    constexpr int ST_NT = 2;
    const bool interior = (m0 + BM <= p.M) && (n0 + BN <= p.N);
    if (interior) {
        if constexpr (FOLD) {
            const __amdgpu_buffer_rsrc_t c_rsrc = __builtin_amdgcn_make_buffer_rsrc(p.C, 0, 0x7fffffff, 0x00020000);
            const bool center = p.ln_colsum != nullptr;
            auto rstd_of_block = [&](int i, float (&dst)[16]) __attribute__((always_inline)) {
#pragma unroll
                for (int g = 0; g < 4; ++g) {
                    const int lr = wm * WM + i * 32 + 4 * h + 8 * g;
#pragma unroll
                    for (int e = 0; e < 4; ++e) dst[4 * g + e] = fold.preloaded ? fold.rstd[i][4 * g + e] : fold.rows[lr + e].x;
                }
            };
            auto scale_and_store = [&](int i, const f32x16 (&src)[TN], const float (&row_rstd)[16]) __attribute__((always_inline)) {
                const int mb = m0 + wm * WM + i * 32 + 4 * h;
#pragma unroll
                for (int j = 0; j < TN; ++j) {
                    const int n = n0 + wn * WN + j * 32 + r;
                    const int c_off = (mb * p.ldc + n) * 4, c_row = p.ldc * 4;
#pragma unroll
                    for (int half = 0; half < 2; ++half) {
                        float y[8];
#pragma unroll
                        for (int q = 0; q < 8; ++q) y[q] = fold_scale(src[j][half * 8 + q], row_rstd[half * 8 + q], bias_r[j]);
                        if constexpr (GELU) gelu_erf_x8(y);
#pragma unroll
                        for (int q = 0; q < 8; ++q) {
                            const int v = half * 8 + q;
                            __builtin_amdgcn_raw_buffer_store_b32(__builtin_bit_cast(unsigned, y[q]), c_rsrc, c_off, ((v & 3) + 8 * (v >> 2)) * c_row, ST_NT);
                        }
                    }
                }
            };
            if (center) {
                float b_op[TN];
#pragma unroll
                for (int j = 0; j < TN; ++j) b_op[j] = h == 0 ? fold.colsum[j] : 0.0f;
#pragma unroll
                for (int i = 0; i < TM; ++i) {
                    const float mean = fold.preloaded ? fold.mean[i] : fold.rows[wm * WM + i * 32 + r].y;
                    const float a_op = h == 0 ? -mean : 0.0f;
                    f32x16 centered[TN];
#pragma unroll
                    for (int j = 0; j < TN; ++j) centered[j] = __builtin_amdgcn_mfma_f32_32x32x2f32(a_op, b_op[j], acc[i][j], 0, 0, 0);
                    float row_rstd[16];
                    rstd_of_block(i, row_rstd);
                    scale_and_store(i, centered, row_rstd);
                }
            } else {
                float row_rstd[TM][16];
#pragma unroll
                for (int i = 0; i < (FOLD_HOIST ? TM : 0); ++i) rstd_of_block(i, row_rstd[i]);
#pragma unroll
                for (int i = 0; i < TM; ++i) {
                    if (!FOLD_HOIST) rstd_of_block(i, row_rstd[i]);
                    scale_and_store(i, acc[i], row_rstd[i]);
                }
            }
            return;
        }
#pragma unroll
        for (int j = 0; j < TN; ++j) {
            const int n = n0 + wn * WN + j * 32 + r;
#pragma unroll
            for (int i = 0; i < TM; ++i) {
                const int mb = m0 + wm * WM + i * 32 + 4 * h;
                if constexpr (AMODE == A_PATCHES) {
                    float add[16];
                    size_t orow[16];
#pragma unroll
                    for (int v = 0; v < 16; ++v) {
                        const int m = mb + (v & 3) + 8 * (v >> 2);
                        const int im = m / p.patches, pp = m - im * p.patches;
                        add[v] = p.pos[(size_t)(pp + 1) * p.N + n];
                        orow[v] = (size_t)m + im + 1;
                    }
#pragma unroll
                    for (int v = 0; v < 16; ++v) p.C[orow[v] * p.ldc + n] = acc[i][j][v] + bias_r[j] + add[v];
                } else {
                    const __amdgpu_buffer_rsrc_t c_rsrc = __builtin_amdgcn_make_buffer_rsrc(p.C, 0, 0x7fffffff, 0x00020000);
                    const int c_off = (mb * p.ldc + n) * 4, c_row = p.ldc * 4;
                    if constexpr (EPI == VITHIP_EPI_BIAS_RESIDUAL) {
                        const __amdgpu_buffer_rsrc_t r_rsrc = __builtin_amdgcn_make_buffer_rsrc(const_cast<float *>(p.R), 0, 0x7fffffff, 0x00020000);
                        const int r_off = (mb * p.ldr + n) * 4, r_row = p.ldr * 4;
#pragma unroll
                        for (int half = 0; half < 2; ++half) {
                            float res[8];
#pragma unroll
                            for (int q = 0; q < 8; ++q) {
                                const int v = half * 8 + q;
                                res[q] = __builtin_bit_cast(float, __builtin_amdgcn_raw_buffer_load_b32(r_rsrc, r_off, ((v & 3) + 8 * (v >> 2)) * r_row, 0));
                            }
#pragma unroll
                            for (int q = 0; q < 8; ++q) {
                                const int v = half * 8 + q;
                                __builtin_amdgcn_raw_buffer_store_b32(__builtin_bit_cast(unsigned, acc[i][j][v] + bias_r[j] + res[q]), c_rsrc, c_off,
                                                                      ((v & 3) + 8 * (v >> 2)) * c_row, 0);
                            }
                        }
                    } else {
#pragma unroll
                        for (int half = 0; half < 2; ++half) {
                            float y[8];
#pragma unroll
                            for (int q = 0; q < 8; ++q) y[q] = acc[i][j][half * 8 + q] + bias_r[j];
                            if constexpr (GELU) gelu_erf_x8(y);
#pragma unroll
                            for (int q = 0; q < 8; ++q) {
                                const int v = half * 8 + q;
                                __builtin_amdgcn_raw_buffer_store_b32(__builtin_bit_cast(unsigned, y[q]), c_rsrc, c_off, ((v & 3) + 8 * (v >> 2)) * c_row, ST_NT);
                            }
                        }
                    }
                }
            }
        }
    } else {
#pragma unroll
        for (int j = 0; j < TN; ++j) {
            const int n = n0 + wn * WN + j * 32 + r;
            const bool n_ok = n < p.N;
#pragma unroll
            for (int i = 0; i < TM; ++i) {
#pragma unroll
                for (int v = 0; v < 16; ++v) {
                    const int m = m0 + wm * WM + i * 32 + (v & 3) + 8 * (v >> 2) + 4 * h;
                    if (n_ok && m < p.M) {
                        float y;
                        if constexpr (FOLD) {
                            const f32x2 row = fold.rows[m - m0];
                            y = fold_scale(fold_center(acc[i][j][v], row.y, fold.colsum[j]), row.x, bias_r[j]);
                        }
                        else y = acc[i][j][v] + bias_r[j];
                        if constexpr (AMODE == A_PATCHES) {
                            const int im = m / p.patches, pp = m - im * p.patches;
                            y += p.pos[(size_t)(pp + 1) * p.N + n];
                            p.C[((size_t)m + im + 1) * p.ldc + n] = y;
                        } else {
                            if constexpr (GELU) y = gelu_erf(y);
                            if constexpr (EPI == VITHIP_EPI_BIAS_RESIDUAL) y += p.R[(size_t)m * p.ldr + n];
                            p.C[(size_t)m * p.ldc + n] = y;
                        }
                    }
                }
            }
        }
    }
}

struct Bf16Params {
    const unsigned short *A;
    const unsigned short *W;
    const float *bias;
    const float *R;
    void *C;
    int lda, ldw, ldr, ldc;
    int M, N, K;
    int tiles_m, tiles_n, group_m;
    unsigned long long *dbg;
    int patches;
    const float *ln_rows;
    const float *ln_colsum;
    unsigned short *x16;
    int ldx16;
    float *partials;
};
int launch_gemm_bf16_pp(hipStream_t stream, const Bf16Params &p, int epilogue, int cus);
int launch_gemm_bf16_w4(hipStream_t stream, const Bf16Params &p, int epilogue, int cus);
int launch_gemm_f32_latency(hipStream_t stream, GemmParams &p, int epilogue);
int launch_patch_embed_bf16(hipStream_t s, const float *images, const unsigned short *conv_w16, const float *conv_b,
                            const float *cls, const float *pos, float *x, int n_images, int img_size, int patch_size,
                            int in_chans, int embed_dim);

__device__ __forceinline__ float reduce_scatter16(const float (&a)[16], int r) {
    float b[8], c[4], d[2], e;
    {
        const bool up = (r & 16) != 0;
#pragma unroll
        for (int k = 0; k < 8; ++k) b[k] = (up ? a[k + 8] : a[k]) + __shfl_xor(up ? a[k] : a[k + 8], 16);
    }
    {
        const bool up = (r & 8) != 0;
#pragma unroll
        for (int k = 0; k < 4; ++k) c[k] = (up ? b[k + 4] : b[k]) + __shfl_xor(up ? b[k] : b[k + 4], 8);
    }
    {
        const bool up = (r & 4) != 0;
#pragma unroll
        for (int k = 0; k < 2; ++k) d[k] = (up ? c[k + 2] : c[k]) + __shfl_xor(up ? c[k] : c[k + 2], 4);
    }
    {
        const bool up = (r & 2) != 0;
        e = (up ? d[1] : d[0]) + __shfl_xor(up ? d[0] : d[1], 2);
    }
    return e + __shfl_xor(e, 1);
}

template <int BM, int BN, int WM, int WN>
__device__ __forceinline__ void epilogue_store_residual_stats(const GemmParams &p, const f32x16 (&acc)[WM / 32][WN / 32],
                                                              const float (&bias_r)[WN / 32], int m0, int n0, int wm, int wn,
                                                              int r, int h) {
    static_assert(WN == 64, "one 64-column strip per wave");
    constexpr int TM = WM / 32;
    const bool interior = m0 + BM <= p.M;
    const int strip = (n0 + wn * WN) >> 6;
    const __amdgpu_buffer_rsrc_t c_rsrc = __builtin_amdgcn_make_buffer_rsrc(p.C, 0, 0x7fffffff, 0x00020000);
    const __amdgpu_buffer_rsrc_t r_rsrc = __builtin_amdgcn_make_buffer_rsrc(const_cast<float *>(p.R), 0, 0x7fffffff, 0x00020000);
#pragma unroll
    for (int i = 0; i < TM; ++i) {
        const int mb = m0 + wm * WM + i * 32 + 4 * h;
        float y[2][16];
#pragma unroll
        for (int j = 0; j < 2; ++j) {
            const int n = n0 + wn * WN + j * 32 + r;
            const int c_off = (mb * p.ldc + n) * 4, c_row = p.ldc * 4, r_off = (mb * p.ldr + n) * 4, r_row = p.ldr * 4;
            if (interior) {
#pragma unroll
                for (int half = 0; half < 2; ++half) {
                    float res[8];
#pragma unroll
                    for (int q = 0; q < 8; ++q) {
                        const int v = half * 8 + q;
                        res[q] = __builtin_bit_cast(float, __builtin_amdgcn_raw_buffer_load_b32(r_rsrc, r_off, ((v & 3) + 8 * (v >> 2)) * r_row, 0));
                    }
#pragma unroll
                    for (int q = 0; q < 8; ++q) {
                        const int v = half * 8 + q;
                        y[j][v] = acc[i][j][v] + bias_r[j] + res[q];
                        __builtin_amdgcn_raw_buffer_store_b32(__builtin_bit_cast(unsigned, y[j][v]), c_rsrc, c_off, ((v & 3) + 8 * (v >> 2)) * c_row, 0);
                    }
                }
            } else {
#pragma unroll
                for (int v = 0; v < 16; ++v) {
                    const int m = mb + (v & 3) + 8 * (v >> 2);
                    y[j][v] = 0.0f;
                    if (m < p.M) {
                        y[j][v] = acc[i][j][v] + bias_r[j] + p.R[(size_t)m * p.ldr + n];
                        p.C[(size_t)m * p.ldc + n] = y[j][v];
                    }
                }
            }
        }
        float u[16], w[16];
        {
#pragma clang fp contract(off)
#pragma unroll
            for (int v = 0; v < 16; ++v) {
                u[v] = y[0][v] + y[1][v];
                const float sq0 = y[0][v] * y[0][v];
                w[v] = __builtin_fmaf(y[1][v], y[1][v], sq0);
            }
        }
        const float us = reduce_scatter16(u, r), ws = reduce_scatter16(w, r);
        const int v = (r >> 1) & 15;
        const int m = mb + (v & 3) + 8 * (v >> 2);
        if (!(r & 1) && m < p.M) *reinterpret_cast<f32x2 *>(p.row_partials + ((size_t)strip * p.M + m) * 2) = f32x2{us, ws};
    }
}

}
```

### vision-transformer-opencl_amd/csrc/vit_gemm_persistent.hip

```cpp
#include "vit_gemm_common.hpp"

namespace vitgemm {

constexpr int PBK = 32;
constexpr int PLD = PBK + 4;
constexpr int SK_HEADER_BYTES = 4096, SK_MAX_OWNERS = 1000, SK_STAT_TAKEN = 1016, SK_STAT_RECOMPUTED = 1017;

template <int BM, int BN, int WM, int WN, int EPI, bool STAMP = false, bool SK = false, int DBG = 0, int ARITH = ARITH_F32>
__global__ __launch_bounds__(256, 2) void gemm_f32_nt_persistent_kernel(const GemmParams p) {
    constexpr bool SPLIT = ARITH == ARITH_SPLIT3;
    static_assert(!SPLIT || DBG == 0, "switch-off builds are fp32 only");
    constexpr int PBK = SPLIT ? SPLIT_BK : vitgemm::PBK;
    constexpr int PLD = SPLIT ? SPLIT_LD : vitgemm::PLD;
    constexpr int ROWS_PER_PASS = 256 / (PBK / 4);
    constexpr int WGN = BN / WN;
    constexpr int TM = WM / 32, TN = WN / 32;
    constexpr int A_CHUNKS = BM * (PBK / 4) / 256;
    constexpr int B_CHUNKS = BN * (PBK / 4) / 256;
    constexpr int NC = PBK / 8;
    constexpr int NS = A_CHUNKS + B_CHUNKS;
    constexpr int NM = 4 * TM * TN;
    static_assert((BM / WM) * WGN == 4, "4 waves per workgroup");

    __shared__ __attribute__((aligned(16))) float lds[2 * (BM + BN) * PLD];
    __shared__ int sk_decision;
    constexpr bool FOLD = EPI == EPI_BIAS_LN || EPI == EPI_BIAS_GELU_LN;
    __shared__ __attribute__((aligned(16))) f32x2 fold_rows_lds[FOLD ? 2 * BM : 2];
    static_assert(!FOLD || BM == 128, "one 16-byte lane copy of 64 lanes = 128 rows");
    float *const As0 = lds;
    float *const Bs0 = lds + 2 * BM * PLD;

    const int tid = threadIdx.x;
    const int lane = tid & 63, wave = tid >> 6;
    const int r = lane & 31, h = lane >> 5;
    const int wm = wave / WGN, wn = wave % WGN;

    unsigned long long st0 = 0, st_rt0 = 0, st_loop0 = 0, st_epi = 0;
    if constexpr (STAMP) {
        st0 = __builtin_amdgcn_s_memtime();
        st_rt0 = __builtin_amdgcn_s_memrealtime();
    }

    const int total = p.tiles_m * p.tiles_n;
    const int nwg = gridDim.x;
    const int first = xcd_remap(blockIdx.x, nwg);
    if (first >= total) return;
    const int nk = p.K / PBK;

    const int full = total / nwg, R = total - full * nwg;
    const int x = SK ? p.sk_x : 0;
    const int H = nwg - R;
    const bool owner = first < R;
    const int npre = (x > 0 && !owner && R > 0) ? (R - (first - R) + H - 1) / H : 0;
    const int pstart = (SK && p.sk_late) ? full : 0, fstart = (SK && p.sk_late) ? 0 : npre;
    const int nseg = npre + full + (owner ? 1 : 0);
    bool took = false;
    struct Seg { int tile, k0, k1, in, out; };
    auto get_seg = [&](int i) -> Seg {
        Seg g;
        if (i >= pstart && i < pstart + npre) {
            const int o = (first - R) + (i - pstart) * H;
            g.tile = full * nwg + o; g.k0 = 0; g.k1 = x; g.in = -1; g.out = o;
        } else if (i < npre + full) {
            g.tile = first + (i - fstart) * nwg; g.k0 = 0; g.k1 = nk; g.in = -1; g.out = -1;
        } else {
            g.tile = first + full * nwg; g.k0 = took ? x : 0; g.k1 = nk; g.in = took ? first : -1; g.out = -1;
        }
        return g;
    };

    const int ld_row = tid / (PBK / 4);
    const int ld_kc = (tid % (PBK / 4)) * 4;
    const __amdgpu_buffer_rsrc_t a_rsrc = __builtin_amdgcn_make_buffer_rsrc(const_cast<float *>(p.A), 0, 0x7fffffff, 0x00020000);
    const __amdgpu_buffer_rsrc_t w_rsrc = __builtin_amdgcn_make_buffer_rsrc(const_cast<float *>(p.W), 0, 0x7fffffff, 0x00020000);
    int a_src[A_CHUNKS];
    int b_src[B_CHUNKS];
    f32x4 a_stage[A_CHUNKS], b_stage[B_CHUNKS];

    auto set_sources = [&](int tile) {
        int tm, tn;
        tile_coords(tile, p.tiles_m, p.tiles_n, p.group_m, tm, tn);
#pragma unroll
        for (int i = 0; i < A_CHUNKS; ++i) {
            int m = tm * BM + ld_row + i * ROWS_PER_PASS;
            m = m < p.M ? m : p.M - 1;
            a_src[i] = (m * p.lda + ld_kc) * 4;
        }
#pragma unroll
        for (int i = 0; i < B_CHUNKS; ++i) {
            int n = tn * BN + ld_row + i * ROWS_PER_PASS;
            n = n < p.N ? n : p.N - 1;
            b_src[i] = (n * p.ldw + ld_kc) * 4;
        }
    };
    auto load_bias = [&](int n0, float (&dst)[TN]) {
#pragma unroll
        for (int j = 0; j < TN; ++j) {
            const int n = n0 + wn * WN + j * 32 + r;
            dst[j] = n < p.N ? p.bias[n] : 0.0f;
        }
    };

    int *const sk_flags = reinterpret_cast<int *>(p.sk_ws);
    const int SK_PARKED = (p.sk_gen << 2) | 1, SK_WITHDRAWN = (p.sk_gen << 2) | 2;
    int steps = 0;
    auto decide = [&]() {
        if (tid == 0) {
            int *const f = sk_flags + first;
            int v = __hip_atomic_load(f, __ATOMIC_RELAXED, __HIP_MEMORY_SCOPE_AGENT);
            while (v != SK_PARKED) {
                int expected = v;
                if (__hip_atomic_compare_exchange_strong(f, &expected, SK_WITHDRAWN, __ATOMIC_RELAXED, __ATOMIC_RELAXED, __HIP_MEMORY_SCOPE_AGENT)) {
                    v = SK_WITHDRAWN;
                    break;
                }
                v = expected;
            }
            if (v == SK_PARKED) __hip_atomic_store(f, 0, __ATOMIC_RELAXED, __HIP_MEMORY_SCOPE_AGENT);
            __hip_atomic_fetch_add(sk_flags + (v == SK_PARKED ? SK_STAT_TAKEN : SK_STAT_RECOMPUTED), 1, __ATOMIC_RELAXED, __HIP_MEMORY_SCOPE_AGENT);
            sk_decision = v == SK_PARKED;
        }
        __syncthreads();
        took = __builtin_amdgcn_readfirstlane(sk_decision) != 0;
        if (took) steps -= x;
    };

    int seg_l = 0, k_l, kend_l;
    {
        const Seg g = get_seg(0);
        set_sources(g.tile);
        k_l = g.k0;
        kend_l = g.k1;
    }
    auto advance_load_cursor = [&]() {
        if (++k_l == kend_l) {
            if (++seg_l < nseg) {
                if (SK && owner && x > 0 && seg_l == nseg - 1) decide();
                const Seg g = get_seg(seg_l);
                set_sources(g.tile);
                k_l = g.k0;
                kend_l = g.k1;
            } else {
                k_l = kend_l - 1;
            }
        }
    };
    auto load_step = [&]() {
        const int k0 = k_l * PBK;
#pragma unroll
        for (int i = 0; i < A_CHUNKS; ++i) a_stage[i] = __builtin_bit_cast(f32x4, __builtin_amdgcn_raw_buffer_load_b128(a_rsrc, a_src[i], k0 * 4, 0));
#pragma unroll
        for (int i = 0; i < B_CHUNKS; ++i) b_stage[i] = __builtin_bit_cast(f32x4, __builtin_amdgcn_raw_buffer_load_b128(w_rsrc, b_src[i], k0 * 4, 0));
    };
    auto stage_write = [&](float *row, f32x4 v) __attribute__((always_inline)) {
        if constexpr (SPLIT) split3_store(row, ld_kc, v);
        else *reinterpret_cast<f32x4 *>(row + ld_kc) = v;
    };
    auto store_step = [&](int buf) {
        float *As = As0 + buf * BM * PLD, *Bs = Bs0 + buf * BN * PLD;
#pragma unroll
        for (int i = 0; i < A_CHUNKS; ++i) stage_write(As + (ld_row + i * ROWS_PER_PASS) * PLD, a_stage[i]);
#pragma unroll
        for (int i = 0; i < B_CHUNKS; ++i) stage_write(Bs + (ld_row + i * ROWS_PER_PASS) * PLD, b_stage[i]);
    };
    auto restage_slot = [&](int q, int buf, int k0) {
        if (q < A_CHUNKS) {
            float *As = As0 + buf * BM * PLD;
            if (DBG != 5 && DBG != 6) stage_write(As + (ld_row + q * ROWS_PER_PASS) * PLD, a_stage[q]);
            if (DBG != 2 && DBG != 6) a_stage[q] = __builtin_bit_cast(f32x4, __builtin_amdgcn_raw_buffer_load_b128(a_rsrc, a_src[q], k0 * 4, 0));
        } else {
            const int qb = q - A_CHUNKS;
            float *Bs = Bs0 + buf * BN * PLD;
            if (DBG != 5 && DBG != 6) stage_write(Bs + (ld_row + qb * ROWS_PER_PASS) * PLD, b_stage[qb]);
            if (DBG != 2 && DBG != 6) b_stage[qb] = __builtin_bit_cast(f32x4, __builtin_amdgcn_raw_buffer_load_b128(w_rsrc, b_src[qb], k0 * 4, 0));
        }
    };

    const int a_frag_off = (wm * WM + r) * PLD + h * 4;
    const int b_frag_off = (wn * WN + r) * PLD + h * 4;
    f32x4 af[2][TM], bf[2][TN];
    auto read_frags = [&](int buf, int c, int set) {
        if constexpr (SPLIT) return;
        const float *As = As0 + buf * BM * PLD + a_frag_off + c * 8;
        const float *Bs = Bs0 + buf * BN * PLD + b_frag_off + c * 8;
#pragma unroll
        for (int i = 0; i < TM; ++i) af[set][i] = *reinterpret_cast<const f32x4 *>(As + i * 32 * PLD);
#pragma unroll
        for (int j = 0; j < TN; ++j) bf[set][j] = *reinterpret_cast<const f32x4 *>(Bs + j * 32 * PLD);
    };

    f32x16 acc[TM][TN];
    constexpr int SC_SYS = 0x11;
    auto slot_rsrc = [&](int o) {
        return __builtin_amdgcn_make_buffer_rsrc(reinterpret_cast<char *>(p.sk_ws) + SK_HEADER_BYTES + (size_t)o * (BM * BN * 4), 0, BM * BN * 4, 0x00020000);
    };
    auto park = [&](int o) {
        const __amdgpu_buffer_rsrc_t rs = slot_rsrc(o);
#pragma unroll
        for (int i = 0; i < TM; ++i)
#pragma unroll
            for (int j = 0; j < TN; ++j)
#pragma unroll
                for (int q4 = 0; q4 < 4; ++q4) {
                    f32x4 v;
#pragma unroll
                    for (int e = 0; e < 4; ++e) v[e] = acc[i][j][4 * q4 + e];
                    __builtin_amdgcn_raw_buffer_store_b128(__builtin_bit_cast(u32x4, v), rs, tid * 16,
                                                           ((i * TN + j) * 4 + q4) * 4096, SC_SYS);
                }
        asm volatile("s_waitcnt vmcnt(0)" ::: "memory");
        __syncthreads();
        if (tid == 0) {
            int cur = __hip_atomic_load(sk_flags + o, __ATOMIC_RELAXED, __HIP_MEMORY_SCOPE_AGENT);
            for (;;) {
                if (cur == SK_WITHDRAWN) {
                    __hip_atomic_store(sk_flags + o, 0, __ATOMIC_RELAXED, __HIP_MEMORY_SCOPE_AGENT);
                    break;
                }
                int expected = cur;
                if (__hip_atomic_compare_exchange_strong(sk_flags + o, &expected, SK_PARKED, __ATOMIC_RELAXED, __ATOMIC_RELAXED, __HIP_MEMORY_SCOPE_AGENT)) break;
                cur = expected;
            }
        }
    };
    auto unpark = [&](int o) {
        const __amdgpu_buffer_rsrc_t rs = slot_rsrc(o);
#pragma unroll
        for (int i = 0; i < TM; ++i)
#pragma unroll
            for (int j = 0; j < TN; ++j)
#pragma unroll
                for (int q4 = 0; q4 < 4; ++q4) {
                    const f32x4 v = __builtin_bit_cast(f32x4, __builtin_amdgcn_raw_buffer_load_b128(rs, tid * 16, ((i * TN + j) * 4 + q4) * 4096, SC_SYS));
#pragma unroll
                    for (int e = 0; e < 4; ++e) acc[i][j][4 * q4 + e] = v[e];
                }
        __builtin_amdgcn_s_waitcnt(0x0F70);
    };

    int seg_c = 0, k_c, kend_c, m0, n0, out_c;
    [[maybe_unused]] int seg_k0 = 0;
    float bias_r[TN];
    FoldOperands<TN, TM> fold{};
    [[maybe_unused]] int fold_buf = 0;
    auto begin_segment = [&](int i) {
        const Seg g = get_seg(i);
        int tm, tn;
        tile_coords(g.tile, p.tiles_m, p.tiles_n, p.group_m, tm, tn);
        m0 = tm * BM;
        n0 = tn * BN;
        k_c = g.k0;
        seg_k0 = g.k0;
        kend_c = g.k1;
        out_c = g.out;
        if (g.out < 0) load_bias(n0, bias_r);
        if constexpr (FOLD) {
            if (g.out < 0) {
#pragma unroll
                for (int j = 0; j < TN; ++j) {
                    const int n = n0 + wn * WN + j * 32 + r;
                    fold.colsum[j] = (p.ln_colsum && n < p.N) ? p.ln_colsum[n] : 0.0f;
                }
                if (wave == 0) {
                    const int left = p.M - m0 < BM ? p.M - m0 : BM;
                    const __amdgpu_buffer_rsrc_t rr = __builtin_amdgcn_make_buffer_rsrc(const_cast<float *>(p.ln_rows) + (size_t)m0 * 2, 0, left * 8, 0x00020000);
                    const unsigned dst = (unsigned)(size_t)(fold_rows_lds + fold_buf * BM);
                    asm volatile("s_mov_b32 m0, %0\n\ts_nop 0\n\tbuffer_load_dwordx4 %1, %2, 0 offen lds" ::"s"(dst), "v"(lane * 16), "s"(rr) : "memory", "m0");
                }
                fold.rows = fold_rows_lds + fold_buf * BM;
                fold_buf ^= 1;
            }
        }
        if (SK && g.in >= 0) {
            unpark(g.in);
        } else {
#pragma unroll
            for (int ii = 0; ii < TM; ++ii)
#pragma unroll
                for (int jj = 0; jj < TN; ++jj)
#pragma unroll
                    for (int v = 0; v < 16; ++v) acc[ii][jj][v] = 0.0f;
        }
    };
    begin_segment(0);

    for (int i = 0; i < nseg; ++i) {
        const Seg g = get_seg(i);
        steps += g.k1 - g.k0;
    }
    load_step();
    advance_load_cursor();
    store_step(0);
    load_step();
    advance_load_cursor();
    __syncthreads();
    read_frags(0, 0, 0);
    if (DBG == 4) read_frags(0, 1, 1);
    (void)af; (void)bf;

    if constexpr (STAMP) st_loop0 = __builtin_amdgcn_s_memtime();
    int cur = 0;
    for (int g = 0; g < steps; ++g) {
        const int k_ahead = k_l * PBK;
        if constexpr (FOLD) {
            if (k_c + 1 == kend_c && out_c < 0) {
                constexpr int FOLD_WAIT = 2 * NS, FOLD_MIN_STEPS = 4;
                static_assert(FOLD_WAIT <= 63, "vmcnt is a 6-bit count on gfx950");
                static_assert((FOLD_MIN_STEPS - 1) * NS >= FOLD_WAIT + NS, "the copy must be older than the loads the wait leaves in flight");
                if (kend_c - seg_k0 >= FOLD_MIN_STEPS) asm volatile("s_waitcnt vmcnt(%0)" ::"n"(FOLD_WAIT) : "memory");
                else asm volatile("s_waitcnt vmcnt(0)" ::: "memory");
            }
        }
        if constexpr (SPLIT) {
            split3_step<TM, TN, NS>(acc, As0 + cur * BM * PLD + a_frag_off, Bs0 + cur * BN * PLD + b_frag_off,
                                    [&](int q) __attribute__((always_inline)) { restage_slot(q, cur ^ 1, k_ahead); });
            advance_load_cursor();
            __syncthreads();
        } else
#pragma unroll
        for (int c = 0; c < NC; ++c) {
            if (c + 1 < NC && DBG != 4) read_frags(cur, c + 1, (c + 1) & 1);
            if (c == NC - 1) {
                if (DBG != 3) __syncthreads();
                if (DBG != 4) read_frags(cur ^ 1, 0, NC & 1);
            }
            __builtin_amdgcn_sched_barrier(0);
#pragma unroll
            for (int idx = 0; idx < NM; ++idx) {
                const int s2 = idx / (TM * TN), i = (idx / TN) % TM, j = idx % TN;
                acc[i][j] = __builtin_amdgcn_mfma_f32_32x32x2f32(af[c & 1][i][s2], bf[c & 1][j][s2], acc[i][j], 0, 0, 0);
                if (c == 0) {
                    const int slot_before = (idx * NS) / NM, slot_after = ((idx + 1) * NS) / NM;
                    if (slot_after > slot_before) {
                        __builtin_amdgcn_sched_barrier(0);
#pragma unroll
                        for (int q = slot_before; q < slot_after; ++q) restage_slot(q, cur ^ 1, k_ahead);
                        __builtin_amdgcn_sched_barrier(0);
                    }
                }
            }
            if (c == 0) advance_load_cursor();
        }
        cur ^= 1;

        if (++k_c == kend_c) {
            unsigned long long e0 = 0;
            if constexpr (STAMP) e0 = __builtin_amdgcn_s_memtime();
            if (SK && out_c >= 0) park(out_c);
            else if (DBG != 1 || p.M < 0) {
                if constexpr (EPI == EPI_RESIDUAL_STATS) epilogue_store_residual_stats<BM, BN, WM, WN>(p, acc, bias_r, m0, n0, wm, wn, r, h);
                else epilogue_store<BM, BN, WM, WN, EPI, A_DENSE>(p, acc, bias_r, m0, n0, wm, wn, r, h, fold);
            }
            if constexpr (STAMP) st_epi += __builtin_amdgcn_s_memtime() - e0;
            if (++seg_c < nseg) begin_segment(seg_c);
        }
    }
    if constexpr (STAMP) {
        const unsigned long long c3 = __builtin_amdgcn_s_memtime(), r3 = __builtin_amdgcn_s_memrealtime();
        if (tid == 0) {
            unsigned long long *d = p.dbg + (size_t)blockIdx.x * 8;
            d[0] = st0; d[1] = st_loop0; d[2] = st_epi; d[3] = c3; d[4] = st_rt0; d[5] = r3;
            d[6] = (unsigned long long)nseg; d[7] = (unsigned long long)steps;
        }
    }
}

static int persistent_wgs() {
    int dev = 0, cus = 0;
    if (hipGetDevice(&dev) != hipSuccess || hipDeviceGetAttribute(&cus, hipDeviceAttributeMultiprocessorCount, dev) != hipSuccess) return 0;
    return 2 * cus;
}

int persistent_piece_steps(int M, int N, int K, int slots, int wgs, int kstep) {
    if (wgs <= 0) wgs = persistent_wgs();
    if (wgs <= 0) return 0;
    const int total = ((M + 127) / 128) * ((N + 127) / 128);
    const int nwg = total < wgs ? total : wgs;
    const int full = total / nwg, R = total - full * nwg, nk = K / PBK;
    if (full < 1 || R <= 0 || R >= nwg || R > slots || R > SK_MAX_OWNERS) return 0;
    const int c = (R + (nwg - R) - 1) / (nwg - R);
    const int x = nk / (c + 1);
    return (x >= 4 && nk - c * x >= 8) ? x * (PBK / kstep) : 0;
}

template <int BM, int BN, int WM, int WN, int ARITH = ARITH_F32>
int launch_persistent_tile(hipStream_t stream, GemmParams &p, int epilogue, int group_m) {
    const int wgs = persistent_wgs();
    if (wgs <= 0) return static_cast<int>(hipErrorInvalidDevice);
    p.tiles_m = (p.M + BM - 1) / BM;
    p.tiles_n = (p.N + BN - 1) / BN;
    p.group_m = group_m;
    const int total = p.tiles_m * p.tiles_n;
    const dim3 grid(total < wgs ? total : wgs), block(256);
    p.sk_x = (p.sk_ws && BM == 128 && BN == 128) ? persistent_piece_steps(p.M, p.N, p.K, p.sk_slots, wgs, ARITH == ARITH_SPLIT3 ? SPLIT_BK : PBK) : 0;
    if (p.sk_x > 0) {
        switch (epilogue) {
            case VITHIP_EPI_BIAS:
                hipLaunchKernelGGL((gemm_f32_nt_persistent_kernel<BM, BN, WM, WN, VITHIP_EPI_BIAS, false, true, 0, ARITH>), grid, block, 0, stream, p);
                break;
            case VITHIP_EPI_BIAS_GELU:
                hipLaunchKernelGGL((gemm_f32_nt_persistent_kernel<BM, BN, WM, WN, VITHIP_EPI_BIAS_GELU, false, true, 0, ARITH>), grid, block, 0, stream, p);
                break;
            case VITHIP_EPI_BIAS_RESIDUAL:
                hipLaunchKernelGGL((gemm_f32_nt_persistent_kernel<BM, BN, WM, WN, VITHIP_EPI_BIAS_RESIDUAL, false, true, 0, ARITH>), grid, block, 0, stream, p);
                break;
            case EPI_BIAS_LN:
                hipLaunchKernelGGL((gemm_f32_nt_persistent_kernel<BM, BN, WM, WN, EPI_BIAS_LN, false, true, 0, ARITH>), grid, block, 0, stream, p);
                break;
            case EPI_BIAS_GELU_LN:
                hipLaunchKernelGGL((gemm_f32_nt_persistent_kernel<BM, BN, WM, WN, EPI_BIAS_GELU_LN, false, true, 0, ARITH>), grid, block, 0, stream, p);
                break;
            case EPI_RESIDUAL_STATS:
                hipLaunchKernelGGL((gemm_f32_nt_persistent_kernel<BM, BN, WM, WN, EPI_RESIDUAL_STATS, false, true, 0, ARITH>), grid, block, 0, stream, p);
                break;
            default:
                return static_cast<int>(hipErrorInvalidValue);
        }
        return static_cast<int>(hipGetLastError());
    }
    switch (epilogue) {
        case VITHIP_EPI_BIAS:
            hipLaunchKernelGGL((gemm_f32_nt_persistent_kernel<BM, BN, WM, WN, VITHIP_EPI_BIAS, false, false, 0, ARITH>), grid, block, 0, stream, p);
            break;
        case VITHIP_EPI_BIAS_GELU:
            hipLaunchKernelGGL((gemm_f32_nt_persistent_kernel<BM, BN, WM, WN, VITHIP_EPI_BIAS_GELU, false, false, 0, ARITH>), grid, block, 0, stream, p);
            break;
        case VITHIP_EPI_BIAS_RESIDUAL:
            hipLaunchKernelGGL((gemm_f32_nt_persistent_kernel<BM, BN, WM, WN, VITHIP_EPI_BIAS_RESIDUAL, false, false, 0, ARITH>), grid, block, 0, stream, p);
            break;
        case EPI_BIAS_LN:
            hipLaunchKernelGGL((gemm_f32_nt_persistent_kernel<BM, BN, WM, WN, EPI_BIAS_LN, false, false, 0, ARITH>), grid, block, 0, stream, p);
            break;
        case EPI_BIAS_GELU_LN:
            hipLaunchKernelGGL((gemm_f32_nt_persistent_kernel<BM, BN, WM, WN, EPI_BIAS_GELU_LN, false, false, 0, ARITH>), grid, block, 0, stream, p);
            break;
        case EPI_RESIDUAL_STATS:
            hipLaunchKernelGGL((gemm_f32_nt_persistent_kernel<BM, BN, WM, WN, EPI_RESIDUAL_STATS, false, false, 0, ARITH>), grid, block, 0, stream, p);
            break;
        default:
            return static_cast<int>(hipErrorInvalidValue);
    }
    return static_cast<int>(hipGetLastError());
}

#ifdef VIT_PROBES
int launch_persistent_stamped(hipStream_t stream, GemmParams &p, int epilogue, int group_m) {
    const int wgs = persistent_wgs();
    if (wgs <= 0) return static_cast<int>(hipErrorInvalidDevice);
    p.tiles_m = (p.M + 127) / 128;
    p.tiles_n = (p.N + 127) / 128;
    p.group_m = group_m;
    const int total = p.tiles_m * p.tiles_n;
    const dim3 grid(total < wgs ? total : wgs), block(256);
    if (epilogue == VITHIP_EPI_BIAS_GELU)
        hipLaunchKernelGGL((gemm_f32_nt_persistent_kernel<128, 128, 64, 64, VITHIP_EPI_BIAS_GELU, true>), grid, block, 0, stream, p);
    else if (epilogue == EPI_BIAS_GELU_LN)
        hipLaunchKernelGGL((gemm_f32_nt_persistent_kernel<128, 128, 64, 64, EPI_BIAS_GELU_LN, true>), grid, block, 0, stream, p);
    else if (epilogue == EPI_BIAS_LN)
        hipLaunchKernelGGL((gemm_f32_nt_persistent_kernel<128, 128, 64, 64, EPI_BIAS_LN, true>), grid, block, 0, stream, p);
    else
        hipLaunchKernelGGL((gemm_f32_nt_persistent_kernel<128, 128, 64, 64, VITHIP_EPI_BIAS, true>), grid, block, 0, stream, p);
    return static_cast<int>(hipGetLastError());
}


template <int DBG>
static int launch_switchoff_dbg(hipStream_t stream, const GemmParams &p, int epilogue, dim3 grid) {
    switch (epilogue) {
        case VITHIP_EPI_BIAS: hipLaunchKernelGGL((gemm_f32_nt_persistent_kernel<128, 128, 64, 64, VITHIP_EPI_BIAS, false, false, DBG>), grid, dim3(256), 0, stream, p); break;
        case VITHIP_EPI_BIAS_GELU: hipLaunchKernelGGL((gemm_f32_nt_persistent_kernel<128, 128, 64, 64, VITHIP_EPI_BIAS_GELU, false, false, DBG>), grid, dim3(256), 0, stream, p); break;
        case VITHIP_EPI_BIAS_RESIDUAL: hipLaunchKernelGGL((gemm_f32_nt_persistent_kernel<128, 128, 64, 64, VITHIP_EPI_BIAS_RESIDUAL, false, false, DBG>), grid, dim3(256), 0, stream, p); break;
        default: return static_cast<int>(hipErrorInvalidValue);
    }
    return static_cast<int>(hipGetLastError());
}
int launch_persistent_switchoff(hipStream_t stream, GemmParams &p, int epilogue, int group_m, int dbg) {
    const int wgs = persistent_wgs();
    if (wgs <= 0) return static_cast<int>(hipErrorInvalidDevice);
    p.tiles_m = (p.M + 127) / 128;
    p.tiles_n = (p.N + 127) / 128;
    p.group_m = group_m;
    p.sk_x = 0;
    const int total = p.tiles_m * p.tiles_n;
    const dim3 grid(total < wgs ? total : wgs);
    switch (dbg) {
        case 1: return launch_switchoff_dbg<1>(stream, p, epilogue, grid);
        case 2: return launch_switchoff_dbg<2>(stream, p, epilogue, grid);
        case 3: return launch_switchoff_dbg<3>(stream, p, epilogue, grid);
        case 4: return launch_switchoff_dbg<4>(stream, p, epilogue, grid);
        case 5: return launch_switchoff_dbg<5>(stream, p, epilogue, grid);
        case 6: return launch_switchoff_dbg<6>(stream, p, epilogue, grid);
        default: return static_cast<int>(hipErrorInvalidValue);
    }
}
#endif

int launch_persistent(hipStream_t stream, GemmParams &p, int epilogue, int group_m, int arith) {
    if (epilogue == VITHIP_EPI_BIAS_RESIDUAL && p.row_partials && p.N % 128 == 0) {
        epilogue = EPI_RESIDUAL_STATS;
        p.stats_in_epilogue = 1;
    }
    if (arith == ARITH_SPLIT3) return launch_persistent_tile<128, 128, 64, 64, ARITH_SPLIT3>(stream, p, epilogue, group_m);
    return launch_persistent_tile<128, 128, 64, 64>(stream, p, epilogue, group_m);
}

}
```

### vision-transformer-opencl_amd/host/vit_engine.c

```c
#include "vit_engine.h"

#include <limits.h>
#include <math.h>
#include <stdarg.h>
#include <stdio.h>
#include <stdlib.h>
#include <omp.h>
#include <string.h>

#include "vit_hip_kernels.h"
#include "vit_io.h"

#define VIT_MAX_LANES 4
#define MAX_EVENTS 4096
#define VIT_MAX_U8_CHANS 4

typedef struct {
    int u8;
    float mean[VIT_MAX_U8_CHANS], std[VIT_MAX_U8_CHANS];
} vit_input;

struct vit_engine {
    vit_config cfg;
    vit_engine_options opt;
    int tokens;
    int n_weights;
    char err[512];

    vithip_stream_t stream;
    vithip_stream_t aux_stream[VIT_MAX_LANES - 1];
    vithip_event_t ev_fork, ev_join[VIT_MAX_LANES - 1];
    float *wblob;
    size_t wblob_bytes;
    float **w;
    unsigned short *wblob16;
    int fold;
    int split;
    unsigned short *wfold16;
    float *wfold32;
    float *wfoldf;
    float *ln_rows32;
    float *ln_part32;
    int lane_cap;
    void *gemm_ws[VIT_MAX_LANES];
    long handover_taken, handover_recomputed;
    int n_cus;
    vithip_graph_t graph;
    const void *g_images; vit_input g_in; float *g_probs; int *g_label; float *g_prob; int g_n;
    unsigned short **w16;
    int weights_loaded;

    float *x, *y, *qkv, *hbuf, *z, *logits;
    float *in_stage[2], *out_stage[2];
    float *pin_in[2], *pin_out[2];
    vithip_stream_t copy_stream;
    vithip_event_t ev_h2d[2], ev_done[2];
    unsigned char *in8_stage[2];
    vithip_event_t ev_in_stage;
    int in_stage_pending;
    int last_rows;

    vithip_event_t ev[2 * MAX_EVENTS];
    int ev_stage[MAX_EVENTS];
    int ev_used;
    int ev_ready;
    long pending_images;
    vit_stage_times times;
};


vit_config vit_config_b16(void) {
    vit_config c = {224, 16, 3, 1000, 768, 12, 12, 3072};
    return c;
}

int vit_config_tokens(const vit_config *cfg) {
    int g = cfg->img_size / cfg->patch_size;
    return g * g + 1;
}

size_t vit_config_weight_size(const vit_config *cfg, int index) {
    const size_t D = (size_t)cfg->embed_dim, H = (size_t)cfg->hidden_dim;
    const size_t T = (size_t)vit_config_tokens(cfg);
    const size_t PK = (size_t)cfg->in_chans * cfg->patch_size * cfg->patch_size;
    const int base = 4 + VIT_WEIGHTS_PER_LAYER * cfg->depth;
    if (index < 0 || index >= base + 4) return 0;
    if (index < 4) {
        const size_t s[4] = {D, D * PK, D, T * D};
        return s[index];
    }
    if (index >= base) {
        const size_t s[4] = {D, D, (size_t)cfg->num_classes * D, (size_t)cfg->num_classes};
        return s[index - base];
    }
    {
        const size_t s[12] = {D, D, 3 * D * D, 3 * D, D * D, D, D, D, H * D, H, D * H, D};
        return s[(index - 4) % VIT_WEIGHTS_PER_LAYER];
    }
}

unsigned long long vit_config_macs_per_image(const vit_config *cfg) {
    const unsigned long long T = (unsigned long long)vit_config_tokens(cfg), D = cfg->embed_dim,
                             H = cfg->hidden_dim, hd = D / cfg->num_heads,
                             PK = (unsigned long long)cfg->in_chans * cfg->patch_size * cfg->patch_size;
    const unsigned long long layer = T * D * 3 * D + 2 * cfg->num_heads * T * T * hd + T * D * D + 2 * T * D * H;
    return (T - 1) * PK * D + cfg->depth * layer + D * cfg->num_classes;
}

unsigned long long vit_config_macs_per_image_pruned(const vit_config *cfg) {
    const unsigned long long T = (unsigned long long)vit_config_tokens(cfg), D = cfg->embed_dim, H = cfg->hidden_dim,
                             hd = D / cfg->num_heads;
    const unsigned long long saved = (T - 1) * (D * D + 2 * cfg->num_heads * T * hd + D * D + 2 * D * H);
    return vit_config_macs_per_image(cfg) - saved;
}

void vit_engine_default_options(vit_engine_options *opt) {
    opt->device = 0;
    opt->max_batch = 256;
    opt->profile = 0;
    opt->lanes = 1;
    opt->dtype = VIT_DTYPE_F32;
    opt->prune_last_layer = 0;
    opt->use_graph = 0;
    opt->gemm_tile = 0;
    opt->ln_fold = 0;
    opt->gemm_handover_test = 0;
    opt->host_first_piece = 0;
    opt->fp32_split = 0;
}

static int fail(vit_engine *e, int code, const char *fmt, ...) {
    va_list ap;
    va_start(ap, fmt);
    vsnprintf(e->err, sizeof(e->err), fmt, ap);
    va_end(ap);
    return code;
}

#define HIP_TRY(e, call)                                                                     \
    do {                                                                                     \
        int rc_ = (call);                                                                    \
        if (rc_ != 0)                                                                        \
            return fail((e), VIT_ERR_HIP, "[%s:%d] HIP error %d (%s) in %s", __FILE__, __LINE__, \
                        rc_, vithip_error_string(rc_), #call);                               \
    } while (0)

const char *vit_engine_last_error(const vit_engine *e) { return e ? e->err : "null engine"; }
const vit_config *vit_engine_config(const vit_engine *e) { return &e->cfg; }

#define WEIGHT_TAIL_PAD (1u << 20)

static int check_config(vit_engine *e) {
    const vit_config *c = &e->cfg;
    if (c->img_size <= 0 || c->patch_size <= 0 || c->in_chans <= 0 || c->num_classes <= 0 ||
        c->embed_dim <= 0 || c->depth <= 0 || c->num_heads <= 0 || c->hidden_dim <= 0)
        return fail(e, VIT_ERR_ARG, "vit_config: all dimensions must be positive");
    if (c->img_size % c->patch_size) return fail(e, VIT_ERR_ARG, "img_size must be a multiple of patch_size");
    if (c->embed_dim % c->num_heads || c->embed_dim / c->num_heads != 64)
        return fail(e, VIT_ERR_ARG, "HIP attention kernel needs head_dim == 64 (got %d/%d)", c->embed_dim, c->num_heads);
    if (c->embed_dim % 32 || c->hidden_dim % 32)
        return fail(e, VIT_ERR_ARG, "embed_dim and hidden_dim must be multiples of 32");
    if (c->patch_size % 4 || c->img_size % 4 || (c->in_chans * c->patch_size * c->patch_size) % 32)
        return fail(e, VIT_ERR_ARG, "patch geometry unsupported (patch%%4, img%%4, C*P*P%%32 must be 0)");
    if (c->embed_dim > 2048) return fail(e, VIT_ERR_ARG, "embed_dim > 2048 unsupported by the LayerNorm kernel");
    return VIT_OK;
}

static int ensure_gemm_workspaces(vit_engine *e) {
    if (e->opt.dtype != VIT_DTYPE_F32) return VIT_OK;
    for (int j = 0; j < e->opt.lanes && j < VIT_MAX_LANES; ++j)
        if (!e->gemm_ws[j]) HIP_TRY(e, vithip_gemm_f32_workspace_create(&e->gemm_ws[j]));
    return VIT_OK;
}

int vit_engine_create(vit_engine **out, const vit_config *cfg, const vit_engine_options *opt) {
    static vit_engine scratch;
    if (!out) return VIT_ERR_ARG;
    *out = NULL;
    vit_engine *e = (vit_engine *)calloc(1, sizeof(*e));
    if (!e) return fail(&scratch, VIT_ERR_NOMEM, "out of host memory");
    *out = e;
    e->cfg = cfg ? *cfg : vit_config_b16();
    if (opt) e->opt = *opt; else vit_engine_default_options(&e->opt);
    if (e->opt.max_batch <= 0) e->opt.max_batch = 256;
    if (e->opt.lanes < 1) e->opt.lanes = 1;
    int rc = check_config(e);
    if (rc) return rc;
    e->tokens = vit_config_tokens(&e->cfg);
    e->n_weights = VIT_WEIGHT_COUNT(e->cfg.depth);
    {
        const size_t T_ = (size_t)e->tokens, per[3] = {T_ * (size_t)e->cfg.hidden_dim, T_ * (size_t)e->cfg.embed_dim,
                                                         (size_t)e->cfg.in_chans * e->cfg.img_size * e->cfg.img_size};
        size_t worst = per[0] > per[1] ? per[0] : per[1];
        if (per[2] > worst) worst = per[2];
        const size_t cap = ((size_t)0x7fffffff - 4096) / (worst * sizeof(float));
        if (cap < 1) return fail(e, VIT_ERR_ARG, "model too large: one image needs %zu bytes of fp32 rows, the fp32 kernels "
                                                 "address < 2 GiB per launch", worst * sizeof(float));
        e->lane_cap = cap > (size_t)INT_MAX ? INT_MAX : (int)cap;
    }

    int ndev = 0;
    HIP_TRY(e, vithip_device_count(&ndev));
    if (e->opt.device < 0 || e->opt.device >= ndev)
        return fail(e, VIT_ERR_ARG, "device %d not available (%d HIP devices)", e->opt.device, ndev);
    HIP_TRY(e, vithip_set_device(e->opt.device));
    {
        vithip_device_info di;
        HIP_TRY(e, vithip_get_device_info(e->opt.device, &di));
        e->n_cus = di.compute_units;
    }
    HIP_TRY(e, vithip_stream_create(&e->stream));
    for (int j = 0; j < VIT_MAX_LANES - 1; ++j) {
        HIP_TRY(e, vithip_stream_create(&e->aux_stream[j]));
        HIP_TRY(e, vithip_event_create(&e->ev_join[j]));
    }
    HIP_TRY(e, vithip_event_create(&e->ev_fork));

    const size_t B = (size_t)e->opt.max_batch, T = (size_t)e->tokens, D = (size_t)e->cfg.embed_dim,
                 H = (size_t)e->cfg.hidden_dim, NC = (size_t)e->cfg.num_classes;
    const size_t img = (size_t)e->cfg.in_chans * e->cfg.img_size * e->cfg.img_size;
    HIP_TRY(e, vithip_malloc((void **)&e->x, B * T * D * sizeof(float)));
    HIP_TRY(e, vithip_malloc((void **)&e->y, B * T * D * sizeof(float)));
    HIP_TRY(e, vithip_malloc((void **)&e->qkv, B * T * 3 * D * sizeof(float)));
    HIP_TRY(e, vithip_malloc((void **)&e->hbuf, B * T * H * sizeof(float)));
    HIP_TRY(e, vithip_malloc((void **)&e->z, B * D * sizeof(float)));
    HIP_TRY(e, vithip_malloc((void **)&e->logits, B * NC * sizeof(float)));
    if (e->opt.lanes > VIT_MAX_LANES) e->opt.lanes = VIT_MAX_LANES;
    {
        int rc_ws = ensure_gemm_workspaces(e);
        if (rc_ws) return rc_ws;
    }
    if (e->opt.dtype == VIT_DTYPE_BF16 && e->opt.ln_fold >= 0) {
        const int ok = e->cfg.embed_dim >= 128 && e->cfg.hidden_dim >= 128 && e->cfg.embed_dim % 64 == 0 && e->cfg.hidden_dim % 64 == 0;
        if (!ok && e->opt.ln_fold > 0) return fail(e, VIT_ERR_ARG, "ln_fold needs embed_dim and hidden_dim >= 128 and multiples of 64");
        e->fold = ok;
        if (e->fold) {
            const size_t L = (size_t)e->cfg.depth;
            HIP_TRY(e, vithip_malloc((void **)&e->wfold16, L * (3 * D * D + H * D) * sizeof(unsigned short) + WEIGHT_TAIL_PAD));
            HIP_TRY(e, vithip_memset((char *)e->wfold16 + L * (3 * D * D + H * D) * sizeof(unsigned short), 0, WEIGHT_TAIL_PAD, e->stream));
            HIP_TRY(e, vithip_malloc((void **)&e->wfoldf, L * (6 * D + 2 * H) * sizeof(float)));
        }
    }
    e->split = e->opt.dtype == VIT_DTYPE_F32 && e->opt.fp32_split >= 0;
    if (e->opt.dtype == VIT_DTYPE_F32 && e->opt.ln_fold >= 0) {
        const int ok = e->cfg.embed_dim % 64 == 0 && e->cfg.embed_dim <= 2048;
        if (!ok && e->opt.ln_fold > 0) return fail(e, VIT_ERR_ARG, "ln_fold (fp32) needs embed_dim to be a multiple of 64, at most 2048");
        e->fold = ok;
        if (e->fold) {
            const size_t L = (size_t)e->cfg.depth;
            HIP_TRY(e, vithip_malloc((void **)&e->wfold32, L * (3 * D * D + H * D) * sizeof(float) + WEIGHT_TAIL_PAD));
            HIP_TRY(e, vithip_memset((char *)e->wfold32 + L * (3 * D * D + H * D) * sizeof(float), 0, WEIGHT_TAIL_PAD, e->stream));
            HIP_TRY(e, vithip_malloc((void **)&e->wfoldf, L * (6 * D + 2 * H) * sizeof(float)));
            HIP_TRY(e, vithip_malloc((void **)&e->ln_rows32, (B * T + B) * 2 * sizeof(float)));
            HIP_TRY(e, vithip_malloc((void **)&e->ln_part32, (D / 64) * B * T * 2 * sizeof(float)));
        }
    }
    HIP_TRY(e, vithip_stream_create(&e->copy_stream));
    for (int b = 0; b < 2; ++b) {
        HIP_TRY(e, vithip_malloc((void **)&e->in_stage[b], B * img * sizeof(float)));
        HIP_TRY(e, vithip_malloc((void **)&e->out_stage[b], B * NC * sizeof(float)));
        HIP_TRY(e, vithip_host_alloc((void **)&e->pin_in[b], B * img * sizeof(float)));
        HIP_TRY(e, vithip_host_alloc((void **)&e->pin_out[b], B * NC * sizeof(float)));
        HIP_TRY(e, vithip_event_create(&e->ev_h2d[b]));
        HIP_TRY(e, vithip_event_create(&e->ev_done[b]));
    }

    e->w = (float **)calloc((size_t)e->n_weights, sizeof(float *));
    e->w16 = (unsigned short **)calloc((size_t)e->n_weights, sizeof(unsigned short *));
    if (!e->w || !e->w16) return fail(e, VIT_ERR_NOMEM, "out of host memory");
    if (e->opt.dtype != VIT_DTYPE_F32 && e->opt.dtype != VIT_DTYPE_BF16)
        return fail(e, VIT_ERR_ARG, "dtype must be VIT_DTYPE_F32 or VIT_DTYPE_BF16");
    if (e->opt.dtype == VIT_DTYPE_BF16 && (e->cfg.embed_dim % 64 || e->cfg.hidden_dim % 64))
        return fail(e, VIT_ERR_ARG, "bf16 path needs embed_dim and hidden_dim to be multiples of 64");
    if (e->opt.profile) return vit_engine_set_profile(e, 1);
    return VIT_OK;
}

void vit_engine_destroy(vit_engine *e) {
    if (!e) return;
    vithip_set_device(e->opt.device);
    if (e->stream) vithip_stream_sync(e->stream);
    if (e->ev_ready)
        for (int i = 0; i < 2 * MAX_EVENTS; ++i) vithip_event_destroy(e->ev[i]);
    if (e->graph) vithip_graph_destroy(e->graph);
    vithip_free(e->x); vithip_free(e->y); vithip_free(e->qkv); vithip_free(e->hbuf);
    vithip_free(e->z); vithip_free(e->logits);
    for (int j = 0; j < VIT_MAX_LANES; ++j) vithip_gemm_f32_workspace_destroy(e->gemm_ws[j]);
    if (e->copy_stream) { vithip_stream_sync(e->copy_stream); vithip_stream_destroy(e->copy_stream); }
    if (e->ev_in_stage) vithip_event_destroy(e->ev_in_stage);
    for (int b = 0; b < 2; ++b) {
        vithip_free(e->in_stage[b]); vithip_free(e->out_stage[b]); vithip_free(e->in8_stage[b]);
        if (e->pin_in[b]) vithip_host_free(e->pin_in[b]);
        if (e->pin_out[b]) vithip_host_free(e->pin_out[b]);
        if (e->ev_h2d[b]) vithip_event_destroy(e->ev_h2d[b]);
        if (e->ev_done[b]) vithip_event_destroy(e->ev_done[b]);
    }
    vithip_free(e->wblob);
    vithip_free(e->wfold16);
    vithip_free(e->wfold32);
    vithip_free(e->ln_rows32);
    vithip_free(e->ln_part32);
    vithip_free(e->wfoldf);
    free(e->w16);
    for (int j = 0; j < VIT_MAX_LANES - 1; ++j) {
        if (e->aux_stream[j]) { vithip_stream_sync(e->aux_stream[j]); vithip_stream_destroy(e->aux_stream[j]); }
        if (e->ev_join[j]) vithip_event_destroy(e->ev_join[j]);
    }
    if (e->ev_fork) vithip_event_destroy(e->ev_fork);
    if (e->stream) vithip_stream_destroy(e->stream);
    free(e->w);
    free(e);
}

int vit_engine_set_lanes(vit_engine *e, int lanes) {
    if (!e) return VIT_ERR_ARG;
    if (lanes < 1 || lanes > VIT_MAX_LANES) return fail(e, VIT_ERR_ARG, "lanes must be 1..%d", VIT_MAX_LANES);
    e->opt.lanes = lanes;
    HIP_TRY(e, vithip_set_device(e->opt.device));
    return ensure_gemm_workspaces(e);
}

int vit_engine_set_profile(vit_engine *e, int on) {
    if (on && !e->ev_ready) {
        for (int i = 0; i < 2 * MAX_EVENTS; ++i) HIP_TRY(e, vithip_event_create(&e->ev[i]));
        e->ev_ready = 1;
    }
    e->opt.profile = on ? 1 : 0;
    return VIT_OK;
}


static void drop_graph(vit_engine *e) {
    if (e->graph) { vithip_graph_destroy(e->graph); e->graph = NULL; }
    e->g_n = 0; e->g_images = NULL; e->g_probs = NULL; e->g_label = NULL; e->g_prob = NULL;
    memset(&e->g_in, 0, sizeof(e->g_in));
}

static int alloc_weight_blob(vit_engine *e, const size_t *off, size_t f32_floats, size_t gemm_floats) {
    const int bf16 = e->opt.dtype == VIT_DTYPE_BF16;
    const size_t bytes = f32_floats * sizeof(float) + (bf16 ? gemm_floats * sizeof(unsigned short) : 0);
    HIP_TRY(e, vithip_set_device(e->opt.device));
    if (e->stream) HIP_TRY(e, vithip_stream_sync(e->stream));
    drop_graph(e);
    e->weights_loaded = 0;
    if (e->wblob && e->wblob_bytes != bytes) { vithip_free(e->wblob); e->wblob = NULL; }
    if (!e->wblob) {
        HIP_TRY(e, vithip_malloc((void **)&e->wblob, bytes + WEIGHT_TAIL_PAD));
        HIP_TRY(e, vithip_memset((char *)e->wblob + bytes, 0, WEIGHT_TAIL_PAD, e->stream));
    }
    e->wblob_bytes = bytes;
    e->wblob16 = bf16 ? (unsigned short *)(e->wblob + f32_floats) : NULL;
    for (int i = 0; i < e->n_weights; ++i) {
        e->w[i] = e->wblob + off[i];
        e->w16[i] = (bf16 && off[i] < gemm_floats) ? e->wblob16 + off[i] : NULL;
    }
    return VIT_OK;
}

static int fold_ln_weights(vit_engine *e) {
    if (!e->fold) return VIT_OK;
    const size_t D = (size_t)e->cfg.embed_dim, H = (size_t)e->cfg.hidden_dim;
    for (int l = 0; l < e->cfg.depth; ++l) {
        float **lw = e->w + 4 + VIT_WEIGHTS_PER_LAYER * l;
        float *ff = e->wfoldf + (size_t)l * (6 * D + 2 * H);
        if (e->opt.dtype == VIT_DTYPE_F32) {
            float *f32 = e->wfold32 + (size_t)l * (3 * D * D + H * D);
            HIP_TRY(e, vithip_ln_fold_weights_f32_centered(e->stream, lw[2], lw[3], lw[0], lw[1], f32, ff, ff + 3 * D, (int)(3 * D), (int)D));
            HIP_TRY(e, vithip_ln_fold_weights_f32_centered(e->stream, lw[8], lw[9], lw[6], lw[7], f32 + 3 * D * D, ff + 6 * D, ff + 6 * D + H, (int)H, (int)D));
            continue;
        }
        unsigned short *f16 = e->wfold16 + (size_t)l * (3 * D * D + H * D);
        HIP_TRY(e, vithip_ln_fold_weights_scaled(e->stream, lw[2], lw[3], lw[0], lw[1], f16, ff, ff + 3 * D, (int)(3 * D), (int)D, (int)D, VITHIP_QSCALE));
        HIP_TRY(e, vithip_ln_fold_weights(e->stream, lw[8], lw[9], lw[6], lw[7], f16 + 3 * D * D, ff + 6 * D, ff + 6 * D + H, (int)H, (int)D));
    }
    return VIT_OK;
}

int vit_engine_load_weight_image(vit_engine *e, const vit_weight_image *img) {
    if (!e || !img || !img->f32) return e ? fail(e, VIT_ERR_ARG, "null weight image") : VIT_ERR_ARG;
    if (memcmp(&img->cfg, &e->cfg, sizeof(vit_config)) != 0 || img->count != e->n_weights)
        return fail(e, VIT_ERR_WEIGHTS, "weight image was built for another model configuration");
    int rc = alloc_weight_blob(e, img->off, img->f32_floats, img->gemm_floats);
    if (rc) return rc;
    const int bf16 = e->opt.dtype == VIT_DTYPE_BF16;
    const size_t up = img->f32_floats * sizeof(float) + ((bf16 && img->bf16_elems) ? img->bf16_elems * sizeof(unsigned short) : 0);
    HIP_TRY(e, vithip_memcpy_h2d(e->wblob, img->f32, up, e->stream));
    if (bf16 && !img->bf16_elems)
        HIP_TRY(e, vithip_f32_to_bf16(e->stream, e->wblob, e->wblob16, img->gemm_floats));
    if ((rc = fold_ln_weights(e))) return rc;
    HIP_TRY(e, vithip_stream_sync(e->stream));
    e->weights_loaded = 1;
    return VIT_OK;
}

int vit_engine_load_weights(vit_engine *e, const Network *weights, int count) {
    if (!e || !weights) return e ? fail(e, VIT_ERR_ARG, "null weights") : VIT_ERR_ARG;
    if (count != e->n_weights)
        return fail(e, VIT_ERR_WEIGHTS, "expected %d weight tensors for depth %d, got %d", e->n_weights, e->cfg.depth, count);
    for (int i = 0; i < count; ++i) {
        const size_t want = vit_config_weight_size(&e->cfg, i);
        if (!weights[i].data)
            return fail(e, VIT_ERR_WEIGHTS, "weight %d is missing (Network[%d].data == NULL; expected %zu floats)", i, i, want);
        if (weights[i].size != want)
            return fail(e, VIT_ERR_WEIGHTS, "weight %d has %zu floats, expected %zu", i, weights[i].size, want);
    }
    vit_weight_image img;
    if (vit_weight_image_build(&img, &e->cfg, weights, count, 0) != 0) return fail(e, VIT_ERR_NOMEM, "out of host memory packing the weights");
    const int rc = vit_engine_load_weight_image(e, &img);
    vit_weight_image_free(&img);
    return rc;
}

int vit_engine_copy_weights(vit_engine *dst, vit_engine *src) {
    if (!dst || !src) return VIT_ERR_ARG;
    if (!src->weights_loaded) return fail(dst, VIT_ERR_STATE, "copy_weights: the source engine has no weights");
    if (memcmp(&dst->cfg, &src->cfg, sizeof(vit_config)) != 0 || dst->opt.dtype != src->opt.dtype)
        return fail(dst, VIT_ERR_ARG, "copy_weights: engines differ in model configuration or dtype");
    size_t *off = (size_t *)malloc(sizeof(size_t) * (size_t)dst->n_weights);
    if (!off) return fail(dst, VIT_ERR_NOMEM, "out of host memory");
    size_t gemm_floats = 0;
    const size_t f32_floats = vit_weight_layout(&dst->cfg, off, NULL, &gemm_floats);
    int rc = alloc_weight_blob(dst, off, f32_floats, gemm_floats);
    free(off);
    if (rc) return rc;
    HIP_TRY(dst, vithip_memcpy_peer(dst->wblob, dst->opt.device, src->wblob, src->opt.device, dst->wblob_bytes, dst->stream));
    if ((rc = fold_ln_weights(dst))) return rc;
    HIP_TRY(dst, vithip_stream_sync(dst->stream));
    dst->weights_loaded = 1;
    return VIT_OK;
}

int vit_engine_read_weight_image(vit_engine *e, vit_weight_image *img) {
    if (!e || !img) return VIT_ERR_ARG;
    if (!e->weights_loaded) return fail(e, VIT_ERR_STATE, "read_weight_image: no weights loaded");
    Network *tmp = (Network *)calloc((size_t)e->n_weights, sizeof(Network));
    if (!tmp) return fail(e, VIT_ERR_NOMEM, "out of host memory");
    size_t *off = (size_t *)malloc(sizeof(size_t) * (size_t)e->n_weights), *size = (size_t *)malloc(sizeof(size_t) * (size_t)e->n_weights);
    size_t gemm_floats = 0;
    const size_t f32_floats = (off && size) ? vit_weight_layout(&e->cfg, off, size, &gemm_floats) : 0;
    float *host = f32_floats ? (float *)malloc(e->wblob_bytes) : NULL;
    int rc = host ? VIT_OK : fail(e, VIT_ERR_NOMEM, "out of host memory");
    if (!rc) {
        rc = vithip_set_device(e->opt.device) || vithip_memcpy_d2h(host, e->wblob, e->wblob_bytes, e->stream) ||
             vithip_stream_sync(e->stream);
        if (rc) rc = fail(e, VIT_ERR_HIP, "read_weight_image: device-to-host copy failed");
    }
    if (!rc) {
        for (int i = 0; i < e->n_weights; ++i) { tmp[i].data = host + off[i]; tmp[i].size = size[i]; }
        const int bf16 = e->opt.dtype == VIT_DTYPE_BF16;
        if (vit_weight_image_build(img, &e->cfg, tmp, e->n_weights, bf16) != 0) rc = fail(e, VIT_ERR_NOMEM, "out of host memory");
        if (!rc && bf16) memcpy(img->bf16, host + f32_floats, gemm_floats * sizeof(unsigned short));
    }
    free(host); free(off); free(size); free(tmp);
    return rc;
}


static int stage_begin(vit_engine *e, vithip_stream_t s, int stage) {
    if (!e->opt.profile || e->ev_used >= MAX_EVENTS) return 0;
    e->ev_stage[e->ev_used] = stage;
    return vithip_event_record(e->ev[2 * e->ev_used], s);
}
static int stage_end(vit_engine *e, vithip_stream_t s) {
    if (!e->opt.profile || e->ev_used >= MAX_EVENTS) return 0;
    int rc = vithip_event_record(e->ev[2 * e->ev_used + 1], s);
    e->ev_used++;
    return rc;
}

typedef struct {
    int stage, bf16;
    const void *A; int lda;
    const void *W; const float *bias;
    void *C; int ldc;
    int M, N, K;
    int role;
    const float *ln_rows, *ln_colsum;
    float *stats_rows, *stats_part;
    unsigned short *x16;
} gemm_desc;

static int gemm(vit_engine *e, vithip_stream_t s, const gemm_desc *g, int *stats_ready) {
    const float *res = g->role == VITHIP_EPI_BIAS_RESIDUAL ? (const float *)g->C : NULL;
    const int ldr = g->ln_rows ? 0 : g->ldc;
    int ready;
    HIP_TRY(e, stage_begin(e, s, g->stage));
    if (g->bf16) {
        static const int epi16[] = {[VITHIP_EPI_BIAS] = VITHIP_BF16_EPI_BF16, [VITHIP_EPI_BIAS_GELU] = VITHIP_BF16_EPI_BF16_GELU,
                                    [VITHIP_EPI_BIAS_RESIDUAL] = VITHIP_BF16_EPI_F32_RESIDUAL};
        vithip_gemm_bf16_args a;
        memset(&a, 0, sizeof(a));
        a.A = g->A; a.lda = g->lda; a.W = g->W; a.ldw = g->K; a.bias = g->bias; a.residual = res; a.ldr = ldr;
        a.C = g->C; a.ldc = g->ldc; a.M = g->M; a.N = g->N; a.K = g->K; a.epilogue = epi16[g->role];
        a.ln_rows = g->ln_rows; a.ln_colsum = g->ln_colsum;
        if ((ready = g->stats_rows != NULL)) { a.x16 = g->x16; a.ldx16 = g->ldc; a.row_partials = g->stats_part; }
        HIP_TRY(e, vithip_gemm_bf16(s, &a));
    } else {
        vithip_gemm_args a;
        memset(&a, 0, sizeof(a));
        a.workspace = e->gemm_ws[0];
        for (int j = 0; j < VIT_MAX_LANES - 1; ++j)
            if (s == e->aux_stream[j]) a.workspace = e->gemm_ws[j + 1];
        a.handover_test = e->opt.gemm_handover_test; a.tile = e->opt.gemm_tile;
        a.arith = e->split && g->stage != VIT_STAGE_HEAD;
        a.A = g->A; a.lda = g->lda; a.W = g->W; a.ldw = g->K; a.bias = g->bias; a.residual = res; a.ldr = ldr;
        a.C = g->C; a.ldc = g->ldc; a.M = g->M; a.N = g->N; a.K = g->K; a.epilogue = g->role;
        a.ln_rows = g->ln_rows; a.ln_colsum = g->ln_colsum;
        a.stats_out = g->stats_rows; a.stats_partials = g->stats_part;
        if (!(ready = vithip_gemm_f32_stats_in_epilogue(&a))) a.stats_out = a.stats_partials = NULL;
        HIP_TRY(e, vithip_gemm_f32(s, &a));
    }
    HIP_TRY(e, stage_end(e, s));
    if (g->bf16 && ready) {
        HIP_TRY(e, stage_begin(e, s, VIT_STAGE_LN));
        HIP_TRY(e, vithip_rowstats_finalize(s, g->stats_part, vithip_ln_strips(g->N), g->M, g->N, g->stats_rows));
        HIP_TRY(e, stage_end(e, s));
    }
    if (stats_ready) *stats_ready = ready;
    return VIT_OK;
}

static int collect_profile(vit_engine *e) {
    if (e->ev_used == 0) return VIT_OK;
    HIP_TRY(e, vithip_device_sync());
    for (int i = 0; i < e->ev_used; ++i) {
        float ms = 0.f;
        HIP_TRY(e, vithip_event_elapsed_ms(&ms, e->ev[2 * i], e->ev[2 * i + 1]));
        e->times.ms[e->ev_stage[i]] += ms;
        e->times.launches[e->ev_stage[i]]++;
    }
    e->times.images += e->pending_images;
    e->pending_images = 0;
    e->ev_used = 0;
    return VIT_OK;
}

typedef struct {
    vithip_stream_t s;
    int off, n;
    int stats_ready;
    float *x;
    void *y, *qkv, *h;
    void *xa;
    float *tok_pairs, *cls_pairs, *partials;
} vit_lane;

typedef struct {
    vit_engine *e;
    vit_lane lane[VIT_MAX_LANES];
    int L;
    int T, D, H, NC;
} chunk_ctx;

#define RUN(call) do { int rc_ = (call); if (rc_) return rc_; } while (0)

static void *at(const void *p, size_t i, size_t esz) { return (char *)p + i * esz; }

static int stage_embed(chunk_ctx *c, const void *d_images, const vit_input *in, float *f32_stage) {
    vit_engine *e = c->e;
    const vit_config *cfg = &e->cfg;
    float **w = e->w;
    const size_t img = (size_t)cfg->in_chans * cfg->img_size * cfg->img_size;
    const int pk = cfg->in_chans * cfg->patch_size * cfg->patch_size;
    const int embed16 = e->opt.dtype == VIT_DTYPE_BF16 && pk % 64 == 0 && pk >= 128 && cfg->patch_size % 8 == 0 &&
                        (size_t)pk <= 2 * (size_t)c->H;
    for (int j = 0; j < c->L; ++j) {
        const vit_lane *ln = &c->lane[j];
        const float *images = in->u8 ? f32_stage + ln->off * img : (const float *)d_images + ln->off * img;
        if (in->u8) {
            HIP_TRY(e, stage_begin(e, ln->s, VIT_STAGE_EMBED));
            HIP_TRY(e, vithip_images_u8_to_f32(ln->s, (const unsigned char *)d_images + ln->off * img, f32_stage + ln->off * img,
                                               ln->n, cfg->img_size, cfg->in_chans, in->mean, in->std));
            HIP_TRY(e, stage_end(e, ln->s));
        }
        HIP_TRY(e, stage_begin(e, ln->s, VIT_STAGE_EMBED));
        if (embed16)
            HIP_TRY(e, vithip_patch_embed_bf16(ln->s, images, e->w16[1], w[2], w[0], w[3], ln->x,
                                               (unsigned short *)e->hbuf + (size_t)ln->off * (c->T - 1) * pk,
                                               ln->n, cfg->img_size, cfg->patch_size, cfg->in_chans, c->D));
        else
            HIP_TRY(e, vithip_patch_embed_f32(ln->s, images, w[1], w[2], w[0], w[3], ln->x, ln->n,
                                              cfg->img_size, cfg->patch_size, cfg->in_chans, c->D));
        HIP_TRY(e, stage_end(e, ln->s));
    }
    return VIT_OK;
}

static int layernorm(chunk_ctx *c, vithip_stream_t s, const float *x, size_t ldx, void *y, size_t ldy, const float *gamma,
                     const float *beta, int rows) {
    vit_engine *e = c->e;
    HIP_TRY(e, stage_begin(e, s, VIT_STAGE_LN));
    if (e->opt.dtype == VIT_DTYPE_BF16) HIP_TRY(e, vithip_layernorm_f32_bf16out(s, x, ldx, y, ldy, gamma, beta, rows, c->D));
    else HIP_TRY(e, vithip_layernorm_f32(s, x, ldx, y, ldy, gamma, beta, rows, c->D));
    HIP_TRY(e, stage_end(e, s));
    return VIT_OK;
}

static int row_stats(chunk_ctx *c, const vit_lane *ln, size_t ldx, float *pairs, int rows) {
    vit_engine *e = c->e;
    HIP_TRY(e, stage_begin(e, ln->s, VIT_STAGE_LN));
    if (e->opt.dtype == VIT_DTYPE_BF16) HIP_TRY(e, vithip_rowstats_bf16(ln->s, ln->x, ldx, ln->xa, ldx, pairs, rows, c->D));
    else HIP_TRY(e, vithip_rowstats_f32(ln->s, ln->x, ldx, pairs, rows, c->D));
    HIP_TRY(e, stage_end(e, ln->s));
    return VIT_OK;
}

static int encoder_layer(chunk_ctx *c, int l) {
    vit_engine *e = c->e;
    const int T = c->T, D = c->D, H = c->H, heads = e->cfg.num_heads;
    const int bf16 = e->opt.dtype == VIT_DTYPE_BF16, fold = e->fold, feeds_next = l + 1 < e->cfg.depth;
    const int pruned = e->opt.prune_last_layer && T <= 224 && !feeds_next;
    const size_t esz = bf16 ? sizeof(unsigned short) : sizeof(float);
    float **lw = e->w + 4 + VIT_WEIGHTS_PER_LAYER * l;
    unsigned short **lw16 = e->w16 + 4 + VIT_WEIGHTS_PER_LAYER * l;
    const void *w_qkv = bf16 ? (const void *)lw16[2] : lw[2], *w_out = bf16 ? (const void *)lw16[4] : lw[4],
               *w_fc1 = bf16 ? (const void *)lw16[8] : lw[8], *w_fc2 = bf16 ? (const void *)lw16[10] : lw[10];
    const float *b_qkv = lw[3], *b_fc1 = lw[9], *cs_qkv = NULL, *cs_fc1 = NULL;
    if (fold) {
        const size_t wl = (size_t)l * (3 * (size_t)D * D + (size_t)H * D);
        const float *ff = e->wfoldf + (size_t)l * (6 * D + 2 * H);
        w_qkv = bf16 ? (const void *)(e->wfold16 + wl) : (const void *)(e->wfold32 + wl);
        w_fc1 = at(w_qkv, 3 * (size_t)D * D, esz);
        b_qkv = ff + 3 * D; b_fc1 = ff + 6 * D + H;
        if (bf16) { cs_qkv = ff; cs_fc1 = ff + 6 * D; }
    }
    const int r = pruned ? T : 1;
    int rows[VIT_MAX_LANES], ln2_ready[VIT_MAX_LANES];
    float *pairs[VIT_MAX_LANES];
    for (int j = 0; j < c->L; ++j) {
        rows[j] = pruned ? c->lane[j].n : c->lane[j].n * T;
        pairs[j] = pruned ? c->lane[j].cls_pairs : c->lane[j].tok_pairs;
    }

    for (int j = 0; j < c->L; ++j) {
        vit_lane *ln = &c->lane[j];
        if (!fold) RUN(layernorm(c, ln->s, ln->x, D, ln->y, D, lw[0], lw[1], ln->n * T));
        else if (!ln->stats_ready) RUN(row_stats(c, ln, D, ln->tok_pairs, ln->n * T));
    }
    for (int j = 0; j < c->L; ++j) {
        vit_lane *ln = &c->lane[j];
        gemm_desc g = {.stage = VIT_STAGE_QKV, .bf16 = bf16, .A = fold ? ln->xa : ln->y, .lda = D, .W = w_qkv, .bias = b_qkv,
                       .C = ln->qkv, .ldc = 3 * D, .M = ln->n * T, .N = 3 * D, .K = D, .role = VITHIP_EPI_BIAS,
                       .ln_rows = ln->tok_pairs, .ln_colsum = cs_qkv};
        if (pruned) {
            gemm_desc kv = g;
            kv.W = at(w_qkv, (size_t)D * D, esz); kv.bias = b_qkv + D; kv.C = at(ln->qkv, D, esz); kv.N = 2 * D;
            kv.ln_colsum = cs_qkv ? cs_qkv + D : NULL;
            RUN(gemm(e, ln->s, &kv, NULL));
            if (fold) {
                HIP_TRY(e, stage_begin(e, ln->s, VIT_STAGE_LN));
                HIP_TRY(e, vithip_gather_rows_f32(ln->s, ln->tok_pairs, (size_t)2 * T, ln->cls_pairs, 2, ln->n, 2));
                HIP_TRY(e, stage_end(e, ln->s));
            }
            g.lda = r * D; g.ldc = r * 3 * D; g.M = rows[j]; g.N = D; g.ln_rows = pairs[j];
        }
        RUN(gemm(e, ln->s, &g, NULL));
    }
    for (int j = 0; j < c->L; ++j) {
        const vit_lane *ln = &c->lane[j];
        HIP_TRY(e, stage_begin(e, ln->s, VIT_STAGE_ATTN));
        if (!bf16 && pruned) HIP_TRY(e, vithip_attention_f32_rows(ln->s, ln->qkv, ln->y, ln->n, T, heads, 1));
        else if (!bf16) HIP_TRY(e, vithip_attention_f32(ln->s, ln->qkv, ln->y, ln->n, T, heads));
        else if (fold) HIP_TRY(e, vithip_attention_bf16io_qscaled(ln->s, ln->qkv, ln->y, ln->n, T, heads, pruned ? 1 : T));
        else if (pruned) HIP_TRY(e, vithip_attention_bf16io_rows(ln->s, ln->qkv, ln->y, ln->n, T, heads, 1));
        else HIP_TRY(e, vithip_attention_bf16io(ln->s, ln->qkv, ln->y, ln->n, T, heads));
        HIP_TRY(e, stage_end(e, ln->s));
    }
    for (int j = 0; j < c->L; ++j) {
        vit_lane *ln = &c->lane[j];
        gemm_desc g = {.stage = VIT_STAGE_OUTPROJ, .bf16 = bf16, .A = ln->y, .lda = r * D, .W = w_out, .bias = lw[5],
                       .C = ln->x, .ldc = r * D, .M = rows[j], .N = D, .K = D, .role = VITHIP_EPI_BIAS_RESIDUAL};
        if (fold && (bf16 || !pruned)) { g.stats_rows = pairs[j]; g.stats_part = ln->partials; g.x16 = bf16 ? ln->xa : NULL; }
        RUN(gemm(e, ln->s, &g, &ln2_ready[j]));
    }
    for (int j = 0; j < c->L; ++j) {
        const vit_lane *ln = &c->lane[j];
        if (!fold) RUN(layernorm(c, ln->s, ln->x, (size_t)r * D, ln->y, D, lw[6], lw[7], rows[j]));
        else if (!ln2_ready[j]) RUN(row_stats(c, ln, (size_t)r * D, pairs[j], rows[j]));
    }
    for (int j = 0; j < c->L; ++j) {
        const vit_lane *ln = &c->lane[j];
        gemm_desc g = {.stage = VIT_STAGE_FC1, .bf16 = bf16, .A = ln->y, .lda = D, .W = w_fc1, .bias = b_fc1, .C = ln->h, .ldc = H,
                       .M = rows[j], .N = H, .K = D, .role = VITHIP_EPI_BIAS_GELU};
        if (fold) { g.A = ln->xa; g.lda = r * D; g.ln_rows = pairs[j]; g.ln_colsum = cs_fc1; }
        RUN(gemm(e, ln->s, &g, NULL));
    }
    for (int j = 0; j < c->L; ++j) {
        vit_lane *ln = &c->lane[j];
        gemm_desc g = {.stage = VIT_STAGE_FC2, .bf16 = bf16, .A = ln->h, .lda = H, .W = w_fc2, .bias = lw[11], .C = ln->x,
                       .ldc = r * D, .M = rows[j], .N = D, .K = H, .role = VITHIP_EPI_BIAS_RESIDUAL};
        if (fold && feeds_next) { g.stats_rows = ln->tok_pairs; g.stats_part = ln->partials; g.x16 = bf16 ? ln->xa : NULL; }
        RUN(gemm(e, ln->s, &g, &ln->stats_ready));
    }
    return VIT_OK;
}

static int stage_head(chunk_ctx *c, float *d_probs, int *d_label, float *d_prob) {
    vit_engine *e = c->e;
    const int T = c->T, D = c->D, NC = c->NC;
    float **fw = e->w + 4 + VIT_WEIGHTS_PER_LAYER * e->cfg.depth;
    for (int j = 0; j < c->L; ++j) {
        const vit_lane *ln = &c->lane[j];
        HIP_TRY(e, stage_begin(e, ln->s, VIT_STAGE_LN));
        HIP_TRY(e, vithip_layernorm_f32(ln->s, ln->x, (size_t)T * D, e->z + (size_t)ln->off * D, (size_t)D, fw[0], fw[1], ln->n, D));
        HIP_TRY(e, stage_end(e, ln->s));
    }
    for (int j = 0; j < c->L; ++j) {
        const vit_lane *ln = &c->lane[j];
        const gemm_desc g = {.stage = VIT_STAGE_HEAD, .A = e->z + (size_t)ln->off * D, .lda = D, .W = fw[2], .bias = fw[3],
                             .C = e->logits + (size_t)ln->off * NC, .ldc = NC, .M = ln->n, .N = NC, .K = D, .role = VITHIP_EPI_BIAS};
        RUN(gemm(e, ln->s, &g, NULL));
    }
    for (int j = 0; j < c->L; ++j) {
        const vit_lane *ln = &c->lane[j];
        const size_t o = (size_t)ln->off;
        HIP_TRY(e, stage_begin(e, ln->s, VIT_STAGE_SOFTMAX));
        HIP_TRY(e, vithip_softmax_top1_f32(ln->s, e->logits + o * NC, NC, d_probs + o * NC, NC, d_label ? d_label + o : NULL, d_prob ? d_prob + o : NULL, ln->n, NC));
        HIP_TRY(e, stage_end(e, ln->s));
    }
    return VIT_OK;
}

static int forward_chunk(vit_engine *e, vithip_stream_t s, const void *d_images, const vit_input *in, float *f32_stage, int nb,
                         float *d_probs, int *d_label, float *d_prob) {
    const vit_config *cfg = &e->cfg;
    chunk_ctx ctx, *c = &ctx;
    c->e = e;
    c->T = e->tokens; c->D = cfg->embed_dim; c->H = cfg->hidden_dim; c->NC = cfg->num_classes;
    c->L = e->opt.lanes > VIT_MAX_LANES ? VIT_MAX_LANES : e->opt.lanes;
    if (c->L < 1 || nb < 2 * c->L) c->L = 1;
    const int bf16 = e->opt.dtype == VIT_DTYPE_BF16;
    const size_t B = (size_t)e->opt.max_batch, T = (size_t)c->T, D = (size_t)c->D, H = (size_t)c->H;
    const size_t esz = bf16 ? sizeof(unsigned short) : sizeof(float);
    float *pairs = e->ln_rows32, *part = e->ln_part32;
    size_t strips = D / 64;
    unsigned short *x16 = NULL;
    if (bf16) {
        x16 = (unsigned short *)e->y + B * T * D;
        strips = (size_t)vithip_ln_strips((int)D);
        part = (float *)((unsigned short *)e->qkv + B * T * 3 * D);
        pairs = part + strips * B * T * 2;
    }
    for (int j = 0; j < c->L; ++j) {
        vit_lane *ln = &c->lane[j];
        memset(ln, 0, sizeof(*ln));
        ln->off = (int)((long)nb * j / c->L);
        ln->n = (int)((long)nb * (j + 1) / c->L) - ln->off;
        ln->s = j == 0 ? s : e->aux_stream[j - 1];
        const size_t row0 = (size_t)ln->off * T;
        ln->x = e->x + row0 * D;
        ln->y = at(e->y, row0 * D, esz); ln->qkv = at(e->qkv, row0 * 3 * D, esz); ln->h = at(e->hbuf, row0 * H, esz);
        if (e->fold) {
            ln->xa = bf16 ? (void *)(x16 + row0 * D) : (void *)ln->x;
            ln->tok_pairs = pairs + row0 * 2;
            ln->cls_pairs = pairs + (B * T + (size_t)ln->off) * 2;
            ln->partials = part + row0 * strips * 2;
        }
    }

    if (c->L > 1) {
        HIP_TRY(e, vithip_event_record(e->ev_fork, s));
        for (int j = 1; j < c->L; ++j) HIP_TRY(e, vithip_stream_wait_event(c->lane[j].s, e->ev_fork));
    }
    RUN(stage_embed(c, d_images, in, f32_stage));
    for (int l = 0; l < cfg->depth; ++l) RUN(encoder_layer(c, l));
    RUN(stage_head(c, d_probs, d_label, d_prob));
    for (int j = 1; j < c->L; ++j) {
        HIP_TRY(e, vithip_event_record(e->ev_join[j - 1], c->lane[j].s));
        HIP_TRY(e, vithip_stream_wait_event(s, e->ev_join[j - 1]));
    }
    e->last_rows = nb;
    return VIT_OK;
}
#undef RUN

static int chunk_limit(const vit_engine *e) {
    int lanes = e->opt.lanes < 1 ? 1 : (e->opt.lanes > VIT_MAX_LANES ? VIT_MAX_LANES : e->opt.lanes);
    if (e->opt.dtype == VIT_DTYPE_BF16) return e->opt.max_batch;
    const long cap = (long)e->lane_cap * lanes;
    return cap < e->opt.max_batch ? (int)cap : e->opt.max_batch;
}

static int input_u8(vit_engine *e, const char *who, const float *mean, const float *std, vit_input *in) {
    memset(in, 0, sizeof(*in));
    in->u8 = 1;
    if (!mean || !std) return fail(e, VIT_ERR_ARG, "%s: mean and std are required", who);
    if (e->cfg.in_chans > VIT_MAX_U8_CHANS)
        return fail(e, VIT_ERR_ARG, "%s: 8-bit input takes at most %d channels (in_chans = %d)", who, VIT_MAX_U8_CHANS, e->cfg.in_chans);
    for (int c = 0; c < e->cfg.in_chans; ++c) {
        if (!isfinite(mean[c]) || !isfinite(std[c]) || std[c] == 0.0f)
            return fail(e, VIT_ERR_ARG, "%s: channel %d: mean (%g) and std (%g) must be finite, std non-zero", who, c, mean[c], std[c]);
        in->mean[c] = mean[c];
        in->std[c] = std[c];
    }
    return VIT_OK;
}

static int in_stage_taken(vit_engine *e, const vit_input *in, vithip_stream_t s) {
    if (!in->u8) return VIT_OK;
    HIP_TRY(e, vithip_event_record(e->ev_in_stage, s));
    e->in_stage_pending = 1;
    return VIT_OK;
}

static int forward_device_in(vit_engine *e, const void *d_images, const vit_input *in, int n, float *d_probs,
                             int *d_top1_label, float *d_top1_prob, void *stream) {
    if (!e->weights_loaded) return fail(e, VIT_ERR_STATE, "forward before vit_engine_load_weights()");
    vithip_stream_t s = stream ? (vithip_stream_t)stream : e->stream;
    const size_t img = (size_t)e->cfg.in_chans * e->cfg.img_size * e->cfg.img_size * (in->u8 ? 1 : sizeof(float));
    const size_t NC = (size_t)e->cfg.num_classes;
    HIP_TRY(e, vithip_set_device(e->opt.device));
    if (in->u8 && !e->ev_in_stage) HIP_TRY(e, vithip_event_create(&e->ev_in_stage));
    const int chunk = chunk_limit(e);
    const int graphable = e->opt.use_graph && !e->opt.profile && e->opt.lanes == 1 && s != NULL;
    if (graphable && e->graph && e->g_n == n && e->g_images == d_images && !memcmp(&e->g_in, in, sizeof(*in)) &&
        e->g_probs == d_probs && e->g_label == d_top1_label && e->g_prob == d_top1_prob) {
        HIP_TRY(e, vithip_graph_launch(e->graph, s));
        return in_stage_taken(e, in, s);
    }
    if (graphable) {
        if (e->graph) { vithip_graph_destroy(e->graph); e->graph = NULL; }
        HIP_TRY(e, vithip_graph_begin(s));
    }
    for (int done = 0; done < n; done += chunk) {
        const int nb = n - done < chunk ? n - done : chunk;
        int rc = forward_chunk(e, s, (const char *)d_images + (size_t)done * img, in, e->in_stage[0], nb, d_probs + (size_t)done * NC,
                               d_top1_label ? d_top1_label + done : NULL,
                               d_top1_prob ? d_top1_prob + done : NULL);
        if (rc) {
            if (graphable) {
                vithip_graph_t g = NULL;
                if (vithip_graph_end(s, &g) == 0 && g) vithip_graph_destroy(g);
            }
            return rc;
        }
        if (e->opt.profile) e->pending_images += nb;
        if (e->opt.profile && e->ev_used > MAX_EVENTS - 256 && (rc = collect_profile(e))) return rc;
    }
    if (graphable) {
        HIP_TRY(e, vithip_graph_end(s, &e->graph));
        e->g_n = n; e->g_images = d_images; e->g_in = *in; e->g_probs = d_probs; e->g_label = d_top1_label; e->g_prob = d_top1_prob;
        HIP_TRY(e, vithip_graph_launch(e->graph, s));
    }
    return in_stage_taken(e, in, s);
}

int vit_engine_forward_device(vit_engine *e, const float *d_images, int n, float *d_probs,
                              int *d_top1_label, float *d_top1_prob, void *stream) {
    if (!e) return VIT_ERR_ARG;
    if (!d_images || !d_probs || n <= 0) return fail(e, VIT_ERR_ARG, "forward_device: bad arguments (n=%d)", n);
    vit_input in;
    memset(&in, 0, sizeof(in));
    return forward_device_in(e, d_images, &in, n, d_probs, d_top1_label, d_top1_prob, stream);
}

int vit_engine_forward_device_u8(vit_engine *e, const unsigned char *d_images, int n, const float *mean, const float *std,
                                 float *d_probs, int *d_top1_label, float *d_top1_prob, void *stream) {
    if (!e) return VIT_ERR_ARG;
    if (!d_images || !d_probs || n <= 0) return fail(e, VIT_ERR_ARG, "forward_device_u8: bad arguments (n=%d)", n);
    if ((size_t)d_images & 3) return fail(e, VIT_ERR_ARG, "forward_device_u8: d_images must be 4-byte aligned");
    vit_input in;
    const int rc = input_u8(e, "forward_device_u8", mean, std, &in);
    if (rc) return rc;
    return forward_device_in(e, d_images, &in, n, d_probs, d_top1_label, d_top1_prob, stream);
}

int vit_engine_sync(vit_engine *e) {
    if (!e) return VIT_ERR_ARG;
    HIP_TRY(e, vithip_stream_sync(e->stream));
    return VIT_OK;
}

#define GATHER_THREADS_MAX 16
#define SUB_PIECE 64
#define SUB_PIECE_FIRST 16
static int gather_threads(void) {
    int n = omp_get_num_procs();
    return n < 1 ? 1 : (n > GATHER_THREADS_MAX ? GATHER_THREADS_MAX : n);
}
typedef struct {
    const float *const *f32;
    const unsigned char *const *u8;
} host_images;
static const void *host_image(const host_images *im, int i) { return im->u8 ? (const void *)im->u8[i] : (const void *)im->f32[i]; }

static void gather_images(char *dst, const host_images *images, int first, int count, size_t img_bytes) {
    const int nt = gather_threads();
#pragma omp parallel for num_threads(nt) schedule(static) if (count >= 4)
    for (int i = 0; i < count; ++i) memcpy(dst + (size_t)i * img_bytes, host_image(images, first + i), img_bytes);
}
static int stage_piece(vit_engine *e, int slot, void *dst, const host_images *images, int first, int count, size_t img_bytes, int sub) {
    for (int s0 = 0; s0 < count; s0 += sub) {
        const int c = count - s0 < sub ? count - s0 : sub;
        char *pin = (char *)e->pin_in[slot] + (size_t)s0 * img_bytes;
        gather_images(pin, images, first + s0, c, img_bytes);
        HIP_TRY(e, vithip_memcpy_h2d((char *)dst + (size_t)s0 * img_bytes, pin, (size_t)c * img_bytes, e->copy_stream));
    }
    HIP_TRY(e, vithip_event_record(e->ev_h2d[slot], e->copy_stream));
    return VIT_OK;
}

static int forward_host_in(vit_engine *e, const char *who, const host_images *images, const vit_input *in, int n, float *const *probs) {
    if (!e->weights_loaded) return fail(e, VIT_ERR_STATE, "forward before vit_engine_load_weights()");
    const size_t img = (size_t)e->cfg.in_chans * e->cfg.img_size * e->cfg.img_size;
    const size_t img_bytes = img * (in->u8 ? 1 : sizeof(float));
    const size_t NC = (size_t)e->cfg.num_classes;
    for (int i = 0; i < n; ++i)
        if (!host_image(images, i) || !probs[i]) return fail(e, VIT_ERR_ARG, "%s: image or output row %d is NULL", who, i);
    HIP_TRY(e, vithip_set_device(e->opt.device));
    for (int b = 0; b < 2 && in->u8; ++b)
        if (!e->in8_stage[b]) HIP_TRY(e, vithip_malloc((void **)&e->in8_stage[b], (size_t)e->opt.max_batch * img));
    if (e->in_stage_pending) {
        HIP_TRY(e, vithip_stream_wait_event(e->copy_stream, e->ev_in_stage));
        e->in_stage_pending = 0;
    }
    void *up[2];
    for (int b = 0; b < 2; ++b) up[b] = in->u8 ? (void *)e->in8_stage[b] : (void *)e->in_stage[b];
    const int chunk = chunk_limit(e);
    int first_n = n;
    if (e->opt.host_first_piece > 0) first_n = e->opt.host_first_piece;
    else if (e->opt.dtype == VIT_DTYPE_F32 && n >= 128) {
        first_n = (5 * n / 32 + 2) & ~3;
        if (first_n > 64) first_n = 64;
    } else if (n >= 128) first_n = 64;
    else if (n >= 64) first_n = (n + 1) / 2;
    if (first_n > chunk) first_n = chunk;
    if (first_n > n) first_n = n;
    const int np = 1 + (n - first_n + chunk - 1) / chunk;
#define PIECE_LO(i) ((i) == 0 ? 0 : ((i) >= np ? n : first_n + ((i) - 1) * chunk))
#define PIECE_N(i) ((PIECE_LO((i) + 1) < n ? PIECE_LO((i) + 1) : n) - PIECE_LO(i))
    {
        int rc0 = stage_piece(e, 0, up[0], images, 0, PIECE_N(0), img_bytes, np > 1 ? SUB_PIECE_FIRST : SUB_PIECE);
        if (rc0) return rc0;
    }
    for (int k = 0; k < np; ++k) {
        const int b = k & 1, nb = PIECE_N(k);
        HIP_TRY(e, vithip_stream_wait_event(e->stream, e->ev_h2d[b]));
        int rc = forward_chunk(e, e->stream, up[b], in, e->in_stage[b], nb, e->out_stage[b], NULL, NULL);
        if (rc) return rc;
        HIP_TRY(e, vithip_memcpy_d2h(e->pin_out[b], e->out_stage[b], (size_t)nb * NC * sizeof(float), e->stream));
        HIP_TRY(e, vithip_event_record(e->ev_done[b], e->stream));
        if (e->opt.profile) e->pending_images += nb;
        if (k >= 1) {
            HIP_TRY(e, vithip_event_sync(e->ev_done[b ^ 1]));
            const int first = PIECE_LO(k - 1);
            for (int i = 0; i < PIECE_N(k - 1); ++i)
                memcpy(probs[first + i], e->pin_out[b ^ 1] + (size_t)i * NC, NC * sizeof(float));
        }
        if (k + 1 < np) {
            rc = stage_piece(e, b ^ 1, up[b ^ 1], images, PIECE_LO(k + 1), PIECE_N(k + 1), img_bytes, SUB_PIECE);
            if (rc) return rc;
        }
    }
    {
        const int b = (np - 1) & 1, first = PIECE_LO(np - 1);
        HIP_TRY(e, vithip_event_sync(e->ev_done[b]));
        for (int i = 0; i < PIECE_N(np - 1); ++i)
            memcpy(probs[first + i], e->pin_out[b] + (size_t)i * NC, NC * sizeof(float));
    }
#undef PIECE_N
#undef PIECE_LO
    if (e->opt.profile) {
        int rc = collect_profile(e);
        if (rc) return rc;
    }
    return VIT_OK;
}

int vit_engine_forward_host(vit_engine *e, const float *const *images, int n, float *const *probs) {
    if (!e) return VIT_ERR_ARG;
    if (!images || !probs || n <= 0) return fail(e, VIT_ERR_ARG, "forward_host: bad arguments (n=%d)", n);
    const host_images im = {images, NULL};
    vit_input in;
    memset(&in, 0, sizeof(in));
    return forward_host_in(e, "forward_host", &im, &in, n, probs);
}

int vit_engine_forward_host_u8(vit_engine *e, const unsigned char *const *images, int n, const float *mean, const float *std,
                               float *const *probs) {
    if (!e) return VIT_ERR_ARG;
    if (!images || !probs || n <= 0) return fail(e, VIT_ERR_ARG, "forward_host_u8: bad arguments (n=%d)", n);
    const host_images im = {NULL, images};
    vit_input in;
    const int rc = input_u8(e, "forward_host_u8", mean, std, &in);
    if (rc) return rc;
    return forward_host_in(e, "forward_host_u8", &im, &in, n, probs);
}

int vit_engine_handover_stats(vit_engine *e, long *taken, long *recomputed) {
    if (!e) return VIT_ERR_ARG;
    HIP_TRY(e, vithip_set_device(e->opt.device));
    HIP_TRY(e, vithip_device_sync());
    for (int j = 0; j < VIT_MAX_LANES; ++j) {
// ... 35 lines not shown
```

Before: 4777 images/sec.

## Pre-split fp32 weights into a swizzled three-plane bf16 image for the split3 GEMM

At weight load, each layer's GEMM weights are converted once into a blocked image of three bf16 pieces (hi/mid/lo) laid out per 128-row panel and K step. The persistent split3 GEMM kernel gains a WIMG variant that streams those pre-split pieces straight into a swizzled LDS layout, instead of loading fp32 weights and splitting them on every tile. It also uses a new swizzled LDS stride for the A operand to cut bank conflicts. This removes the per-tile weight conversion work and reads 6 bytes per weight instead of 4, at the cost of extra device memory for the images and a new kernel path restricted to 128x128 tiles.

```diff
diff --git a/include/vit_hip_kernels.h b/include/vit_hip_kernels.h
--- a/include/vit_hip_kernels.h
+++ b/include/vit_hip_kernels.h
@@ -66,8 +66,11 @@
     const float *ln_rows, *ln_colsum;
     float *stats_out, *stats_partials;
     int arith;
+    const void *w_split;
 } vithip_gemm_args;
 int vithip_gemm_f32(vithip_stream_t stream, const vithip_gemm_args *args);
+size_t vithip_split3_weights_bytes(int N, int K);
+int vithip_split3_weights_f32(vithip_stream_t stream, const float *W, int ldw, int N, int K, void *out);
 int vithip_gemm_f32_stats_in_epilogue(const vithip_gemm_args *args);
 int vithip_ln_fold_weights_f32(vithip_stream_t stream, const float *W, const float *bias, const float *gamma, const float *beta,
                                float *Wf, float *colsum, float *bias_f, int N, int K);
diff --git a/vision-transformer-opencl_amd/binding.py b/vision-transformer-opencl_amd/binding.py
--- a/vision-transformer-opencl_amd/binding.py
+++ b/vision-transformer-opencl_amd/binding.py
@@ -65,7 +65,7 @@
                 ("C", C.c_void_p), ("ldc", C.c_int), ("M", C.c_int), ("N", C.c_int), ("K", C.c_int),
                 ("epilogue", C.c_int), ("tile", C.c_int), ("group_m", C.c_int), ("workspace", C.c_void_p),
                 ("handover_test", C.c_int), ("ln_rows", C.c_void_p), ("ln_colsum", C.c_void_p),
-                ("stats_out", C.c_void_p), ("stats_partials", C.c_void_p), ("arith", C.c_int)]
+                ("stats_out", C.c_void_p), ("stats_partials", C.c_void_p), ("arith", C.c_int), ("w_split", C.c_void_p)]
 
 
 _lib: Optional[C.CDLL] = None
@@ -171,6 +171,9 @@
         for fn in ("vithip_memcpy_h2d", "vithip_memcpy_d2h", "vithip_memcpy_d2d"):
             getattr(L, fn).argtypes = [C.c_void_p, C.c_void_p, C.c_size_t, C.c_void_p]
         L.vithip_gemm_f32.argtypes = [C.c_void_p, C.POINTER(CGemmArgs)]
+        L.vithip_split3_weights_bytes.argtypes = [C.c_int, C.c_int]
+        L.vithip_split3_weights_bytes.restype = C.c_size_t
+        L.vithip_split3_weights_f32.argtypes = [C.c_void_p, C.c_void_p, C.c_int, C.c_int, C.c_int, C.c_void_p]
         L.vithip_patch_embed_f32.argtypes = [C.c_void_p] + [C.c_void_p] * 6 + [C.c_int] * 5
         L.vithip_layernorm_f32.argtypes = [C.c_void_p, C.c_void_p, C.c_size_t, C.c_void_p, C.c_size_t,
                                            C.c_void_p, C.c_void_p, C.c_int, C.c_int]
@@ -251,7 +254,7 @@
 
 def gemm(A, W, bias, residual=None, epilogue=EPI_BIAS, tile: int = 0, group_m: int = 0, workspace: bool = False,
          handover_test: int = 0, stats: Optional[dict] = None, ln=None, row_stats: Optional[dict] = None,
-         arith: int = ARITH_F32) -> np.ndarray:
+         arith: int = ARITH_F32, w_split: bool = False) -> np.ndarray:
     A, W, bias = _as_f32(A), _as_f32(W), _as_f32(bias)
     M, K = A.shape
     N = W.shape[0]
@@ -266,6 +269,9 @@
     args = CGemmArgs(dA.ptr, K, dW.ptr, K, db.ptr, dR.ptr if dR else None, N, dC.ptr, N, M, N, K, epilogue, tile, group_m, ws,
                      handover_test, dRows.ptr if dRows else None, dCs.ptr if dCs else None, dSt.ptr if dSt else None,
                      dPart.ptr if dPart else None, arith)
+    dImg = split3_weights_device(dW, N, K) if w_split else None
+    if dImg is not None:
+        args.w_split = dImg.ptr
     if row_stats is not None:
         row_stats["in_epilogue"] = int(lib().vithip_gemm_f32_stats_in_epilogue(C.byref(args)))
     hip_check(lib().vithip_gemm_f32(None, C.byref(args)), "vithip_gemm_f32")
@@ -277,6 +283,22 @@
             stats.update(gemm_workspace_stats(ws))
         lib().vithip_gemm_f32_workspace_destroy(C.c_void_p(ws))
     return out
+
+
+def split3_weights_device(dW: "DeviceArray", N: int, K: int, ldw: Optional[int] = None) -> "DeviceArray":
+    nbytes = int(lib().vithip_split3_weights_bytes(N, K))
+    if nbytes == 0:
+        raise VitError(f"vithip_split3_weights_bytes({N}, {K}): bad shape")
+    out = DeviceArray((nbytes,), np.uint8)
+    hip_check(lib().vithip_split3_weights_f32(None, dW.ptr, K if ldw is None else ldw, N, K, out.ptr), "vithip_split3_weights_f32")
+    return out
+
+
+def split3_weights(W) -> np.ndarray:
+    W = _as_f32(W)
+    N, K = W.shape
+    img = split3_weights_device(DeviceArray.from_numpy(W), N, K).numpy()
+    return img.view(np.uint16).reshape((N + 127) // 128, K // 16, 3, 128, 16)
 
 
 def gemm_workspace() -> int:
diff --git a/vision-transformer-opencl_amd/csrc/vit_gemm.hip b/vision-transformer-opencl_amd/csrc/vit_gemm.hip
--- a/vision-transformer-opencl_amd/csrc/vit_gemm.hip
+++ b/vision-transformer-opencl_amd/csrc/vit_gemm.hip
@@ -545,6 +545,8 @@
     if (a->tile < 0 || (a->tile > 0 && a->tile < 6) || a->tile > 12 || a->group_m < 0 || a->group_m > 1024) return static_cast<int>(hipErrorInvalidValue);
     if (a->arith != ARITH_F32 && (a->arith != ARITH_SPLIT3 || (a->tile != 0 && a->tile != 9 && a->tile != 10 && a->tile != 11)))
         return static_cast<int>(hipErrorInvalidValue);
+    if (a->w_split && !aligned16(a->w_split)) return static_cast<int>(hipErrorInvalidValue);
+    p.w_split = a->arith == ARITH_SPLIT3 ? a->w_split : nullptr;
     int epilogue = a->epilogue;
     if (a->ln_rows || a->ln_colsum) {
         if (!a->ln_rows || (epilogue != VITHIP_EPI_BIAS && epilogue != VITHIP_EPI_BIAS_GELU) ||
diff --git a/vision-transformer-opencl_amd/csrc/vit_gemm_common.hpp b/vision-transformer-opencl_amd/csrc/vit_gemm_common.hpp
--- a/vision-transformer-opencl_amd/csrc/vit_gemm_common.hpp
+++ b/vision-transformer-opencl_amd/csrc/vit_gemm_common.hpp
@@ -44,6 +44,7 @@
     const float *ln_colsum;
     float *row_partials;
     int stats_in_epilogue;
+    const void *w_split;
 };
 
 __device__ __forceinline__ float erf_fp32(float x) {
@@ -166,19 +167,30 @@
 __device__ __forceinline__ float bf16_to_f32(__bf16 v) {
     return __builtin_bit_cast(float, (unsigned)__builtin_bit_cast(unsigned short, v) << 16);
 }
+__device__ __forceinline__ u32x2 split3_piece(f32x4 &x, int piece) {
+    bf16x4 b;
+#pragma unroll
+    for (int e = 0; e < 4; ++e) b[e] = (__bf16)x[e];
+    if (piece < 2) {
+#pragma unroll
+        for (int e = 0; e < 4; ++e) x[e] = x[e] - bf16_to_f32(b[e]);
+    }
+    return __builtin_bit_cast(u32x2, b);
+}
 __device__ __forceinline__ void split3_store(float *row, int kc, f32x4 x) {
 #pragma unroll
-    for (int piece = 0; piece < 3; ++piece) {
-        bf16x4 b;
-#pragma unroll
-        for (int e = 0; e < 4; ++e) b[e] = (__bf16)x[e];
-        *reinterpret_cast<u32x2 *>(row + piece * 8 + kc / 2) = __builtin_bit_cast(u32x2, b);
-        if (piece < 2) {
-#pragma unroll
-            for (int e = 0; e < 4; ++e) x[e] = x[e] - bf16_to_f32(b[e]);
-        }
-    }
-}
+    for (int piece = 0; piece < 3; ++piece) *reinterpret_cast<u32x2 *>(row + piece * 8 + kc / 2) = split3_piece(x, piece);
+}
+__device__ __forceinline__ u32x4 split3_piece8(f32x4 &x0, f32x4 &x1, int piece) {
+    const u32x2 p0 = split3_piece(x0, piece), p1 = split3_piece(x1, piece);
+    return u32x4{p0[0], p0[1], p1[0], p1[1]};
+}
+
+constexpr int WIMG_ROWS = 128;
+constexpr int WIMG_BLOCK_BYTES = 3 * WIMG_ROWS * SPLIT_BK * 2;
+constexpr int SPLIT_LD_SW = 32;
+__device__ __forceinline__ int split_swizzle(int row) { return 2 * ((row & 3) ^ ((row >> 2) & 3)) + ((row >> 3) & 1); }
+__device__ __forceinline__ int split_sw_offset(int row, int s) { return row * SPLIT_LD_SW + 4 * (s ^ split_swizzle(row)); }
 template <int TM, int TN, int NS, typename Restage>
 __device__ __forceinline__ void split3_step(f32x16 (&acc)[TM][TN], const float *As, const float *Bs, Restage &&restage) {
     bf16x8 a[TM][3], b[TN][3];
@@ -204,6 +216,34 @@
                 for (int q = slot_before; q < slot_after; ++q) restage(q);
                 __builtin_amdgcn_sched_barrier(0);
             }
+        }
+    }
+}
+template <int TM, int TN, int NS, typename Restage>
+__device__ __forceinline__ void split3_step_sw(f32x16 (&acc)[TM][TN], const float *As, const float *Bs, const int (&poff)[3],
+                                               Restage &&restage) {
+    bf16x8 a[TM][3], b[TN][3];
+#pragma unroll
+    for (int o = 0; o < 3; ++o) {
+        const int pa = SPLIT_TERM_A[o], pb = SPLIT_TERM_W[o];
+#pragma unroll
+        for (int i = 0; i < TM; ++i) a[i][pa] = *reinterpret_cast<const bf16x8 *>(As + i * 32 * SPLIT_LD_SW + poff[pa]);
+#pragma unroll
+        for (int j = 0; j < TN; ++j) b[j][pb] = *reinterpret_cast<const bf16x8 *>(Bs + j * 32 * SPLIT_LD_SW + poff[pb]);
+    }
+    __builtin_amdgcn_sched_barrier(0);
+    constexpr int NM = 6 * TM * TN;
+    static_assert(NS <= NM, "one restage slot per matrix instruction at most");
+#pragma unroll
+    for (int idx = 0; idx < NM; ++idx) {
+        const int t = idx / (TM * TN), i = (idx / TN) % TM, j = idx % TN;
+        acc[i][j] = __builtin_amdgcn_mfma_f32_32x32x16_bf16(a[i][SPLIT_TERM_A[t]], b[j][SPLIT_TERM_W[t]], acc[i][j], 0, 0, 0);
+        const int slot_before = (idx * NS + NM - 1) / NM, slot_after = ((idx + 1) * NS + NM - 1) / NM;
+        if (slot_after > slot_before) {
+            __builtin_amdgcn_sched_barrier(0);
+#pragma unroll
+            for (int q = slot_before; q < slot_after; ++q) restage(q);
+            __builtin_amdgcn_sched_barrier(0);
         }
     }
 }
diff --git a/vision-transformer-opencl_amd/csrc/vit_gemm_persistent.hip b/vision-transformer-opencl_amd/csrc/vit_gemm_persistent.hip
--- a/vision-transformer-opencl_amd/csrc/vit_gemm_persistent.hip
+++ b/vision-transformer-opencl_amd/csrc/vit_gemm_persistent.hip
@@ -6,12 +6,14 @@
 constexpr int PLD = PBK + 4;
 constexpr int SK_HEADER_BYTES = 4096, SK_MAX_OWNERS = 1000, SK_STAT_TAKEN = 1016, SK_STAT_RECOMPUTED = 1017;
 
-template <int BM, int BN, int WM, int WN, int EPI, bool STAMP = false, bool SK = false, int DBG = 0, int ARITH = ARITH_F32>
+template <int BM, int BN, int WM, int WN, int EPI, bool STAMP = false, bool SK = false, int DBG = 0, int ARITH = ARITH_F32,
+          bool WIMG = false>
 __global__ __launch_bounds__(256, 2) void gemm_f32_nt_persistent_kernel(const GemmParams p) {
     constexpr bool SPLIT = ARITH == ARITH_SPLIT3;
     static_assert(!SPLIT || DBG == 0, "switch-off builds are fp32 only");
+    static_assert(!WIMG || (SPLIT && BM == WIMG_ROWS && BN == WIMG_ROWS && !STAMP), "the weight image feeds the 128x128 split walk");
     constexpr int PBK = SPLIT ? SPLIT_BK : vitgemm::PBK;
-    constexpr int PLD = SPLIT ? SPLIT_LD : vitgemm::PLD;
+    constexpr int PLD = WIMG ? SPLIT_LD_SW : SPLIT ? SPLIT_LD : vitgemm::PLD;
     constexpr int ROWS_PER_PASS = 256 / (PBK / 4);
     constexpr int WGN = BN / WN;
     constexpr int TM = WM / 32, TN = WN / 32;
@@ -19,6 +21,10 @@
     constexpr int B_CHUNKS = BN * (PBK / 4) / 256;
     constexpr int NC = PBK / 8;
     constexpr int NS = A_CHUNKS + B_CHUNKS;
+    constexpr int W_CHUNKS = 3;
+    constexpr int NL = WIMG ? A_CHUNKS + W_CHUNKS : NS;
+    constexpr int NSL = WIMG ? 6 : NS;
+    static_assert(!WIMG || (A_CHUNKS == 2 && BM * 2 == 256 && BN * 2 == 256), "WIMG: one 8-deep half row of A and of W per thread");
     constexpr int NM = 4 * TM * TN;
     static_assert((BM / WM) * WGN == 4, "4 waves per workgroup");
 
@@ -71,15 +77,30 @@
 
     const int ld_row = tid / (PBK / 4);
     const int ld_kc = (tid % (PBK / 4)) * 4;
+    const int sw_row = tid >> 1, sw_half = tid & 1;
+    int wr_off[3];
+#pragma unroll
+    for (int pl = 0; pl < 3; ++pl) wr_off[pl] = WIMG ? split_sw_offset(sw_row, 2 * pl + sw_half) : 0;
     const __amdgpu_buffer_rsrc_t a_rsrc = __builtin_amdgcn_make_buffer_rsrc(const_cast<float *>(p.A), 0, 0x7fffffff, 0x00020000);
-    const __amdgpu_buffer_rsrc_t w_rsrc = __builtin_amdgcn_make_buffer_rsrc(const_cast<float *>(p.W), 0, 0x7fffffff, 0x00020000);
+    const __amdgpu_buffer_rsrc_t w_rsrc =
+        __builtin_amdgcn_make_buffer_rsrc(const_cast<void *>(WIMG ? p.w_split : static_cast<const void *>(p.W)), 0, 0x7fffffff, 0x00020000);
     int a_src[A_CHUNKS];
-    int b_src[B_CHUNKS];
+    int b_src[WIMG ? W_CHUNKS : B_CHUNKS];
     f32x4 a_stage[A_CHUNKS], b_stage[B_CHUNKS];
+    u32x4 w_stage[WIMG ? W_CHUNKS : 1];
 
     auto set_sources = [&](int tile) {
         int tm, tn;
         tile_coords(tile, p.tiles_m, p.tiles_n, p.group_m, tm, tn);
+        if constexpr (WIMG) {
+            int m = tm * BM + sw_row;
+            m = m < p.M ? m : p.M - 1;
+#pragma unroll
+            for (int i = 0; i < A_CHUNKS; ++i) a_src[i] = (m * p.lda + 8 * sw_half + 4 * i) * 4;
+#pragma unroll
+            for (int q = 0; q < W_CHUNKS; ++q) b_src[q] = tn * nk * WIMG_BLOCK_BYTES + (q * 256 + tid) * 16;
+            return;
+        }
 #pragma unroll
         for (int i = 0; i < A_CHUNKS; ++i) {
             int m = tm * BM + ld_row + i * ROWS_PER_PASS;
@@ -149,6 +170,11 @@
         const int k0 = k_l * PBK;
 #pragma unroll
         for (int i = 0; i < A_CHUNKS; ++i) a_stage[i] = __builtin_bit_cast(f32x4, __builtin_amdgcn_raw_buffer_load_b128(a_rsrc, a_src[i], k0 * 4, 0));
+        if constexpr (WIMG) {
+#pragma unroll
+            for (int q = 0; q < W_CHUNKS; ++q) w_stage[q] = __builtin_amdgcn_raw_buffer_load_b128(w_rsrc, b_src[q], k_l * WIMG_BLOCK_BYTES, 0);
+            return;
+        }
 #pragma unroll
         for (int i = 0; i < B_CHUNKS; ++i) b_stage[i] = __builtin_bit_cast(f32x4, __builtin_amdgcn_raw_buffer_load_b128(w_rsrc, b_src[i], k0 * 4, 0));
     };
@@ -156,14 +182,41 @@
         if constexpr (SPLIT) split3_store(row, ld_kc, v);
         else *reinterpret_cast<f32x4 *>(row + ld_kc) = v;
     };
+    auto write_a_plane = [&](float *As, int pl) __attribute__((always_inline)) {
+        *reinterpret_cast<u32x4 *>(As + wr_off[pl]) = split3_piece8(a_stage[0], a_stage[1], pl);
+    };
+    auto write_w_plane = [&](float *Bs, int pl) __attribute__((always_inline)) { *reinterpret_cast<u32x4 *>(Bs + wr_off[pl]) = w_stage[pl]; };
     auto store_step = [&](int buf) {
         float *As = As0 + buf * BM * PLD, *Bs = Bs0 + buf * BN * PLD;
+        if constexpr (WIMG) {
+#pragma unroll
+            for (int pl = 0; pl < 3; ++pl) {
+                write_a_plane(As, pl);
+                write_w_plane(Bs, pl);
+            }
+            return;
+        }
 #pragma unroll
         for (int i = 0; i < A_CHUNKS; ++i) stage_write(As + (ld_row + i * ROWS_PER_PASS) * PLD, a_stage[i]);
 #pragma unroll
         for (int i = 0; i < B_CHUNKS; ++i) stage_write(Bs + (ld_row + i * ROWS_PER_PASS) * PLD, b_stage[i]);
     };
     auto restage_slot = [&](int q, int buf, int k0) {
+        if constexpr (WIMG) {
+            const int pl = q >> 1;
+            if (q & 1) {
+                write_w_plane(Bs0 + buf * BN * PLD, pl);
+                w_stage[pl] = __builtin_amdgcn_raw_buffer_load_b128(w_rsrc, b_src[pl], (k0 / PBK) * WIMG_BLOCK_BYTES, 0);
+            } else {
+                write_a_plane(As0 + buf * BM * PLD, pl);
+                if (pl == 2) {
+#pragma unroll
+                    for (int i = 0; i < A_CHUNKS; ++i)
+                        a_stage[i] = __builtin_bit_cast(f32x4, __builtin_amdgcn_raw_buffer_load_b128(a_rsrc, a_src[i], k0 * 4, 0));
+                }
+            }
+            return;
+        }
         if (q < A_CHUNKS) {
             float *As = As0 + buf * BM * PLD;
             if (DBG != 5 && DBG != 6) stage_write(As + (ld_row + q * ROWS_PER_PASS) * PLD, a_stage[q]);
@@ -176,8 +229,11 @@
         }
     };
 
-    const int a_frag_off = (wm * WM + r) * PLD + h * 4;
-    const int b_frag_off = (wn * WN + r) * PLD + h * 4;
+    const int a_frag_off = WIMG ? (wm * WM + r) * PLD : (wm * WM + r) * PLD + h * 4;
+    const int b_frag_off = WIMG ? (wn * WN + r) * PLD : (wn * WN + r) * PLD + h * 4;
+    int frag_poff[3];
+#pragma unroll
+    for (int pc = 0; pc < 3; ++pc) frag_poff[pc] = WIMG ? split_sw_offset(r, 2 * pc + h) - r * PLD : 0;
     f32x4 af[2][TM], bf[2][TN];
     auto read_frags = [&](int buf, int c, int set) {
         if constexpr (SPLIT) return;
@@ -304,14 +360,19 @@
         const int k_ahead = k_l * PBK;
         if constexpr (FOLD) {
             if (k_c + 1 == kend_c && out_c < 0) {
-                constexpr int FOLD_WAIT = 2 * NS, FOLD_MIN_STEPS = 4;
+                constexpr int FOLD_WAIT = 2 * NL, FOLD_MIN_STEPS = 4;
                 static_assert(FOLD_WAIT <= 63, "vmcnt is a 6-bit count on gfx950");
-                static_assert((FOLD_MIN_STEPS - 1) * NS >= FOLD_WAIT + NS, "the copy must be older than the loads the wait leaves in flight");
+                static_assert((FOLD_MIN_STEPS - 1) * NL >= FOLD_WAIT + NL, "the copy must be older than the loads the wait leaves in flight");
                 if (kend_c - seg_k0 >= FOLD_MIN_STEPS) asm volatile("s_waitcnt vmcnt(%0)" ::"n"(FOLD_WAIT) : "memory");
                 else asm volatile("s_waitcnt vmcnt(0)" ::: "memory");
             }
         }
-        if constexpr (SPLIT) {
+        if constexpr (WIMG) {
+            split3_step_sw<TM, TN, NSL>(acc, As0 + cur * BM * PLD + a_frag_off, Bs0 + cur * BN * PLD + b_frag_off, frag_poff,
+                                        [&](int q) __attribute__((always_inline)) { restage_slot(q, cur ^ 1, k_ahead); });
+            advance_load_cursor();
+            __syncthreads();
+        } else if constexpr (SPLIT) {
             split3_step<TM, TN, NS>(acc, As0 + cur * BM * PLD + a_frag_off, Bs0 + cur * BN * PLD + b_frag_off,
                                     [&](int q) __attribute__((always_inline)) { restage_slot(q, cur ^ 1, k_ahead); });
             advance_load_cursor();
@@ -383,7 +444,7 @@
     return (x >= 4 && nk - c * x >= 8) ? x * (PBK / kstep) : 0;
 }
 
-template <int BM, int BN, int WM, int WN, int ARITH = ARITH_F32>
+template <int BM, int BN, int WM, int WN, int ARITH = ARITH_F32, bool WIMG = false>
 int launch_persistent_tile(hipStream_t stream, GemmParams &p, int epilogue, int group_m) {
     const int wgs = persistent_wgs();
     if (wgs <= 0) return static_cast<int>(hipErrorInvalidDevice);
@@ -396,22 +457,22 @@
     if (p.sk_x > 0) {
         switch (epilogue) {
             case VITHIP_EPI_BIAS:
-                hipLaunchKernelGGL((gemm_f32_nt_persistent_kernel<BM, BN, WM, WN, VITHIP_EPI_BIAS, false, true, 0, ARITH>), grid, block, 0, stream, p);
+                hipLaunchKernelGGL((gemm_f32_nt_persistent_kernel<BM, BN, WM, WN, VITHIP_EPI_BIAS, false, true, 0, ARITH, WIMG>), grid, block, 0, stream, p);
                 break;
             case VITHIP_EPI_BIAS_GELU:
-                hipLaunchKernelGGL((gemm_f32_nt_persistent_kernel<BM, BN, WM, WN, VITHIP_EPI_BIAS_GELU, false, true, 0, ARITH>), grid, block, 0, stream, p);
+                hipLaunchKernelGGL((gemm_f32_nt_persistent_kernel<BM, BN, WM, WN, VITHIP_EPI_BIAS_GELU, false, true, 0, ARITH, WIMG>), grid, block, 0, stream, p);
                 break;
             case VITHIP_EPI_BIAS_RESIDUAL:
-                hipLaunchKernelGGL((gemm_f32_nt_persistent_kernel<BM, BN, WM, WN, VITHIP_EPI_BIAS_RESIDUAL, false, true, 0, ARITH>), grid, block, 0, stream, p);
+                hipLaunchKernelGGL((gemm_f32_nt_persistent_kernel<BM, BN, WM, WN, VITHIP_EPI_BIAS_RESIDUAL, false, true, 0, ARITH, WIMG>), grid, block, 0, stream, p);
                 break;
             case EPI_BIAS_LN:
-                hipLaunchKernelGGL((gemm_f32_nt_persistent_kernel<BM, BN, WM, WN, EPI_BIAS_LN, false, true, 0, ARITH>), grid, block, 0, stream, p);
+                hipLaunchKernelGGL((gemm_f32_nt_persistent_kernel<BM, BN, WM, WN, EPI_BIAS_LN, false, true, 0, ARITH, WIMG>), grid, block, 0, stream, p);
                 break;
             case EPI_BIAS_GELU_LN:
-                hipLaunchKernelGGL((gemm_f32_nt_persistent_kernel<BM, BN, WM, WN, EPI_BIAS_GELU_LN, false, true, 0, ARITH>), grid, block, 0, stream, p);
+                hipLaunchKernelGGL((gemm_f32_nt_persistent_kernel<BM, BN, WM, WN, EPI_BIAS_GELU_LN, false, true, 0, ARITH, WIMG>), grid, block, 0, stream, p);
                 break;
             case EPI_RESIDUAL_STATS:
-                hipLaunchKernelGGL((gemm_f32_nt_persistent_kernel<BM, BN, WM, WN, EPI_RESIDUAL_STATS, false, true, 0, ARITH>), grid, block, 0, stream, p);
+                hipLaunchKernelGGL((gemm_f32_nt_persistent_kernel<BM, BN, WM, WN, EPI_RESIDUAL_STATS, false, true, 0, ARITH, WIMG>), grid, block, 0, stream, p);
                 break;
             default:
                 return static_cast<int>(hipErrorInvalidValue);
@@ -420,22 +481,22 @@
     }
     switch (epilogue) {
         case VITHIP_EPI_BIAS:
-            hipLaunchKernelGGL((gemm_f32_nt_persistent_kernel<BM, BN, WM, WN, VITHIP_EPI_BIAS, false, false, 0, ARITH>), grid, block, 0, stream, p);
+            hipLaunchKernelGGL((gemm_f32_nt_persistent_kernel<BM, BN, WM, WN, VITHIP_EPI_BIAS, false, false, 0, ARITH, WIMG>), grid, block, 0, stream, p);
             break;
         case VITHIP_EPI_BIAS_GELU:
-            hipLaunchKernelGGL((gemm_f32_nt_persistent_kernel<BM, BN, WM, WN, VITHIP_EPI_BIAS_GELU, false, false, 0, ARITH>), grid, block, 0, stream, p);
+            hipLaunchKernelGGL((gemm_f32_nt_persistent_kernel<BM, BN, WM, WN, VITHIP_EPI_BIAS_GELU, false, false, 0, ARITH, WIMG>), grid, block, 0, stream, p);
             break;
         case VITHIP_EPI_BIAS_RESIDUAL:
-            hipLaunchKernelGGL((gemm_f32_nt_persistent_kernel<BM, BN, WM, WN, VITHIP_EPI_BIAS_RESIDUAL, false, false, 0, ARITH>), grid, block, 0, stream, p);
+            hipLaunchKernelGGL((gemm_f32_nt_persistent_kernel<BM, BN, WM, WN, VITHIP_EPI_BIAS_RESIDUAL, false, false, 0, ARITH, WIMG>), grid, block, 0, stream, p);
             break;
         case EPI_BIAS_LN:
-            hipLaunchKernelGGL((gemm_f32_nt_persistent_kernel<BM, BN, WM, WN, EPI_BIAS_LN, false, false, 0, ARITH>), grid, block, 0, stream, p);
+            hipLaunchKernelGGL((gemm_f32_nt_persistent_kernel<BM, BN, WM, WN, EPI_BIAS_LN, false, false, 0, ARITH, WIMG>), grid, block, 0, stream, p);
             break;
         case EPI_BIAS_GELU_LN:
-            hipLaunchKernelGGL((gemm_f32_nt_persistent_kernel<BM, BN, WM, WN, EPI_BIAS_GELU_LN, false, false, 0, ARITH>), grid, block, 0, stream, p);
+            hipLaunchKernelGGL((gemm_f32_nt_persistent_kernel<BM, BN, WM, WN, EPI_BIAS_GELU_LN, false, false, 0, ARITH, WIMG>), grid, block, 0, stream, p);
             break;
         case EPI_RESIDUAL_STATS:
-            hipLaunchKernelGGL((gemm_f32_nt_persistent_kernel<BM, BN, WM, WN, EPI_RESIDUAL_STATS, false, false, 0, ARITH>), grid, block, 0, stream, p);
+            hipLaunchKernelGGL((gemm_f32_nt_persistent_kernel<BM, BN, WM, WN, EPI_RESIDUAL_STATS, false, false, 0, ARITH, WIMG>), grid, block, 0, stream, p);
             break;
         default:
             return static_cast<int>(hipErrorInvalidValue);
@@ -500,7 +561,10 @@
         epilogue = EPI_RESIDUAL_STATS;
         p.stats_in_epilogue = 1;
     }
-    if (arith == ARITH_SPLIT3) return launch_persistent_tile<128, 128, 64, 64, ARITH_SPLIT3>(stream, p, epilogue, group_m);
+    if (arith == ARITH_SPLIT3) {
+        if (p.w_split) return launch_persistent_tile<128, 128, 64, 64, ARITH_SPLIT3, true>(stream, p, epilogue, group_m);
+        return launch_persistent_tile<128, 128, 64, 64, ARITH_SPLIT3>(stream, p, epilogue, group_m);
+    }
     return launch_persistent_tile<128, 128, 64, 64>(stream, p, epilogue, group_m);
 }
 
diff --git a/vision-transformer-opencl_amd/csrc/vit_split_weights.hip b/vision-transformer-opencl_amd/csrc/vit_split_weights.hip
--- /dev/null
+++ b/vision-transformer-opencl_amd/csrc/vit_split_weights.hip
@@ -0,0 +1,43 @@
+#include "vit_gemm_common.hpp"
+
+namespace {
+
+using namespace vitgemm;
+
+__global__ __launch_bounds__(256) void split3_weights_kernel(const float *__restrict__ W, int ldw, int N, int nk,
+                                                             unsigned char *__restrict__ out) {
+    const size_t blk = blockIdx.x;
+    const int t = threadIdx.x, row = t >> 1, half = t & 1;
+    const int panel = (int)(blk / nk), step = (int)(blk - (size_t)panel * nk);
+    const int n = panel * WIMG_ROWS + row;
+    f32x4 x0 = {0.f, 0.f, 0.f, 0.f}, x1 = {0.f, 0.f, 0.f, 0.f};
+    if (n < N) {
+        const float *src = W + (size_t)n * ldw + step * SPLIT_BK + 8 * half;
+        x0 = *reinterpret_cast<const f32x4 *>(src);
+        x1 = *reinterpret_cast<const f32x4 *>(src + 4);
+    }
+    unsigned char *dst = out + blk * WIMG_BLOCK_BYTES + (size_t)t * 16;
+#pragma unroll
+    for (int pl = 0; pl < 3; ++pl) *reinterpret_cast<u32x4 *>(dst + pl * 256 * 16) = split3_piece8(x0, x1, pl);
+}
+
+}
+
+extern "C" {
+
+size_t vithip_split3_weights_bytes(int N, int K) {
+    if (N <= 0 || K <= 0 || K % KALIGN) return 0;
+    return (size_t)((N + WIMG_ROWS - 1) / WIMG_ROWS) * WIMG_ROWS * (size_t)K * 6;
+}
+
+int vithip_split3_weights_f32(vithip_stream_t stream, const float *W, int ldw, int N, int K, void *out) {
+    if (!W || !out || N <= 0 || K <= 0 || K % KALIGN || ldw < K || ldw % 4) return static_cast<int>(hipErrorInvalidValue);
+    if ((reinterpret_cast<size_t>(W) & 15) || (reinterpret_cast<size_t>(out) & 15)) return static_cast<int>(hipErrorInvalidValue);
+    if (vithip_split3_weights_bytes(N, K) >= 0x7fffffffull) return static_cast<int>(hipErrorInvalidValue);
+    const int panels = (N + WIMG_ROWS - 1) / WIMG_ROWS, nk = K / SPLIT_BK;
+    hipLaunchKernelGGL(split3_weights_kernel, dim3((unsigned)((size_t)panels * nk)), dim3(256), 0, static_cast<hipStream_t>(stream), W, ldw,
+                       N, nk, static_cast<unsigned char *>(out));
+    return static_cast<int>(hipGetLastError());
+}
+
+}
diff --git a/vision-transformer-opencl_amd/host/vit_engine.c b/vision-transformer-opencl_amd/host/vit_engine.c
--- a/vision-transformer-opencl_amd/host/vit_engine.c
+++ b/vision-transformer-opencl_amd/host/vit_engine.c
@@ -38,6 +38,8 @@
     int split;
     unsigned short *wfold16;
     float *wfold32;
+    unsigned char *wsplit;
+    size_t wsplit_off[4], wsplit_layer;
     float *wfoldf;
     float *ln_rows32;
     float *ln_part32;
@@ -255,6 +257,15 @@
             HIP_TRY(e, vithip_malloc((void **)&e->ln_part32, (D / 64) * B * T * 2 * sizeof(float)));
         }
     }
+    if (e->split) {
+        const size_t b[4] = {vithip_split3_weights_bytes((int)(3 * D), (int)D), vithip_split3_weights_bytes((int)D, (int)D),
+                             vithip_split3_weights_bytes((int)H, (int)D), vithip_split3_weights_bytes((int)D, (int)H)};
+        if (b[0] && b[1] && b[2] && b[3]) {
+            e->wsplit_layer = 0;
+            for (int i = 0; i < 4; ++i) { e->wsplit_off[i] = e->wsplit_layer; e->wsplit_layer += b[i]; }
+            HIP_TRY(e, vithip_malloc((void **)&e->wsplit, (size_t)e->cfg.depth * e->wsplit_layer));
+        }
+    }
     HIP_TRY(e, vithip_stream_create(&e->copy_stream));
     for (int b = 0; b < 2; ++b) {
         HIP_TRY(e, vithip_malloc((void **)&e->in_stage[b], B * img * sizeof(float)));
@@ -298,6 +309,7 @@
     vithip_free(e->wblob);
     vithip_free(e->wfold16);
     vithip_free(e->wfold32);
+    vithip_free(e->wsplit);
     vithip_free(e->ln_rows32);
     vithip_free(e->ln_part32);
     vithip_free(e->wfoldf);
@@ -376,6 +388,25 @@
     return VIT_OK;
 }
 
+static int split_weights(vit_engine *e) {
+    if (!e->wsplit) return VIT_OK;
+    const size_t D = (size_t)e->cfg.embed_dim, H = (size_t)e->cfg.hidden_dim;
+    for (int l = 0; l < e->cfg.depth; ++l) {
+        float **lw = e->w + 4 + VIT_WEIGHTS_PER_LAYER * l;
+        const float *w_qkv = lw[2], *w_fc1 = lw[8];
+        if (e->fold) {
+            w_qkv = e->wfold32 + (size_t)l * (3 * D * D + H * D);
+            w_fc1 = w_qkv + 3 * D * D;
+        }
+        unsigned char *img = e->wsplit + (size_t)l * e->wsplit_layer;
+        HIP_TRY(e, vithip_split3_weights_f32(e->stream, w_qkv, (int)D, (int)(3 * D), (int)D, img + e->wsplit_off[0]));
+        HIP_TRY(e, vithip_split3_weights_f32(e->stream, lw[4], (int)D, (int)D, (int)D, img + e->wsplit_off[1]));
+        HIP_TRY(e, vithip_split3_weights_f32(e->stream, w_fc1, (int)D, (int)H, (int)D, img + e->wsplit_off[2]));
+        HIP_TRY(e, vithip_split3_weights_f32(e->stream, lw[10], (int)H, (int)D, (int)H, img + e->wsplit_off[3]));
+    }
+    return VIT_OK;
+}
+
 int vit_engine_load_weight_image(vit_engine *e, const vit_weight_image *img) {
     if (!e || !img || !img->f32) return e ? fail(e, VIT_ERR_ARG, "null weight image") : VIT_ERR_ARG;
     if (memcmp(&img->cfg, &e->cfg, sizeof(vit_config)) != 0 || img->count != e->n_weights)
@@ -388,6 +419,7 @@
     if (bf16 && !img->bf16_elems)
         HIP_TRY(e, vithip_f32_to_bf16(e->stream, e->wblob, e->wblob16, img->gemm_floats));
     if ((rc = fold_ln_weights(e))) return rc;
+    if ((rc = split_weights(e))) return rc;
     HIP_TRY(e, vithip_stream_sync(e->stream));
     e->weights_loaded = 1;
     return VIT_OK;
@@ -425,6 +457,7 @@
     if (rc) return rc;
     HIP_TRY(dst, vithip_memcpy_peer(dst->wblob, dst->opt.device, src->wblob, src->opt.device, dst->wblob_bytes, dst->stream));
     if ((rc = fold_ln_weights(dst))) return rc;
+    if ((rc = split_weights(dst))) return rc;
     HIP_TRY(dst, vithip_stream_sync(dst->stream));
     dst->weights_loaded = 1;
     return VIT_OK;
@@ -478,6 +511,7 @@
     const float *ln_rows, *ln_colsum;
     float *stats_rows, *stats_part;
     unsigned short *x16;
+    const void *w_split;
 } gemm_desc;
 
 static int gemm(vit_engine *e, vithip_stream_t s, const gemm_desc *g, int *stats_ready) {
@@ -503,6 +537,7 @@
             if (s == e->aux_stream[j]) a.workspace = e->gemm_ws[j + 1];
         a.handover_test = e->opt.gemm_handover_test; a.tile = e->opt.gemm_tile;
         a.arith = e->split && g->stage != VIT_STAGE_HEAD;
+        a.w_split = a.arith ? g->w_split : NULL;
         a.A = g->A; a.lda = g->lda; a.W = g->W; a.ldw = g->K; a.bias = g->bias; a.residual = res; a.ldr = ldr;
         a.C = g->C; a.ldc = g->ldc; a.M = g->M; a.N = g->N; a.K = g->K; a.epilogue = g->role;
         a.ln_rows = g->ln_rows; a.ln_colsum = g->ln_colsum;
@@ -616,6 +651,9 @@
     const void *w_qkv = bf16 ? (const void *)lw16[2] : lw[2], *w_out = bf16 ? (const void *)lw16[4] : lw[4],
                *w_fc1 = bf16 ? (const void *)lw16[8] : lw[8], *w_fc2 = bf16 ? (const void *)lw16[10] : lw[10];
     const float *b_qkv = lw[3], *b_fc1 = lw[9], *cs_qkv = NULL, *cs_fc1 = NULL;
+    const unsigned char *ws = e->wsplit ? e->wsplit + (size_t)l * e->wsplit_layer : NULL;
+    const void *ws_qkv = ws ? ws + e->wsplit_off[0] : NULL, *ws_out = ws ? ws + e->wsplit_off[1] : NULL,
+               *ws_fc1 = ws ? ws + e->wsplit_off[2] : NULL, *ws_fc2 = ws ? ws + e->wsplit_off[3] : NULL;
     if (fold) {
         const size_t wl = (size_t)l * (3 * (size_t)D * D + (size_t)H * D);
         const float *ff = e->wfoldf + (size_t)l * (6 * D + 2 * H);
@@ -641,11 +679,12 @@
         vit_lane *ln = &c->lane[j];
         gemm_desc g = {.stage = VIT_STAGE_QKV, .bf16 = bf16, .A = fold ? ln->xa : ln->y, .lda = D, .W = w_qkv, .bias = b_qkv,
                        .C = ln->qkv, .ldc = 3 * D, .M = ln->n * T, .N = 3 * D, .K = D, .role = VITHIP_EPI_BIAS,
-                       .ln_rows = ln->tok_pairs, .ln_colsum = cs_qkv};
+                       .ln_rows = ln->tok_pairs, .ln_colsum = cs_qkv, .w_split = ws_qkv};
         if (pruned) {
             gemm_desc kv = g;
             kv.W = at(w_qkv, (size_t)D * D, esz); kv.bias = b_qkv + D; kv.C = at(ln->qkv, D, esz); kv.N = 2 * D;
             kv.ln_colsum = cs_qkv ? cs_qkv + D : NULL;
+            kv.w_split = ws_qkv && D % 128 == 0 ? at(ws_qkv, (size_t)D * D * 6, 1) : NULL;
             RUN(gemm(e, ln->s, &kv, NULL));
             if (fold) {
                 HIP_TRY(e, stage_begin(e, ln->s, VIT_STAGE_LN));
@@ -669,7 +708,7 @@
     for (int j = 0; j < c->L; ++j) {
         vit_lane *ln = &c->lane[j];
         gemm_desc g = {.stage = VIT_STAGE_OUTPROJ, .bf16 = bf16, .A = ln->y, .lda = r * D, .W = w_out, .bias = lw[5],
-                       .C = ln->x, .ldc = r * D, .M = rows[j], .N = D, .K = D, .role = VITHIP_EPI_BIAS_RESIDUAL};
+                       .C = ln->x, .ldc = r * D, .M = rows[j], .N = D, .K = D, .role = VITHIP_EPI_BIAS_RESIDUAL, .w_split = ws_out};
         if (fold && (bf16 || !pruned)) { g.stats_rows = pairs[j]; g.stats_part = ln->partials; g.x16 = bf16 ? ln->xa : NULL; }
         RUN(gemm(e, ln->s, &g, &ln2_ready[j]));
     }
@@ -681,14 +720,14 @@
     for (int j = 0; j < c->L; ++j) {
         const vit_lane *ln = &c->lane[j];
         gemm_desc g = {.stage = VIT_STAGE_FC1, .bf16 = bf16, .A = ln->y, .lda = D, .W = w_fc1, .bias = b_fc1, .C = ln->h, .ldc = H,
-                       .M = rows[j], .N = H, .K = D, .role = VITHIP_EPI_BIAS_GELU};
+                       .M = rows[j], .N = H, .K = D, .role = VITHIP_EPI_BIAS_GELU, .w_split = ws_fc1};
         if (fold) { g.A = ln->xa; g.lda = r * D; g.ln_rows = pairs[j]; g.ln_colsum = cs_fc1; }
         RUN(gemm(e, ln->s, &g, NULL));
     }
     for (int j = 0; j < c->L; ++j) {
         vit_lane *ln = &c->lane[j];
         gemm_desc g = {.stage = VIT_STAGE_FC2, .bf16 = bf16, .A = ln->h, .lda = H, .W = w_fc2, .bias = lw[11], .C = ln->x,
-                       .ldc = r * D, .M = rows[j], .N = D, .K = H, .role = VITHIP_EPI_BIAS_RESIDUAL};
+                       .ldc = r * D, .M = rows[j], .N = D, .K = H, .role = VITHIP_EPI_BIAS_RESIDUAL, .w_split = ws_fc2};
         if (fold && feeds_next) { g.stats_rows = ln->tok_pairs; g.stats_part = ln->partials; g.x16 = bf16 ? ln->xa : NULL; }
         RUN(gemm(e, ln->s, &g, &ln->stats_ready));
     }
```

Result: faster. 5237 images/sec (median of 6 runs) (+9.6%).
